# e-c-k-e-r/tortoise-tts

Measured on AMD Instinct MI355X. Metric: audio-sec/wall-sec (RTF^-1), 16 AR candidates x 80 DDIM steps, higher is better.
Workload: dtype bf16; 1 GPU; configs[1]: 1 utterance/GPU, 64 text tokens, 16 AR candidates x 250 mel tokens (KV-cached decode), latent pass on 16 candidates, 80 DDIM steps with cond-free guidance at T=1088 (11.6 s audio); candidates=16, ddim_steps=80, mel_frames=1088, parallelism=single GPU, small_models=False, vocoder_in_step=False

## Files before the change

### tortoise_tts_amd/csrc/diff.hip

```cpp
#include <stdlib.h>

#include "ttk_common.h"
#include "ttk_host.h"

using namespace ttk;

namespace {
struct AttnBlk { float *gn_g, *gn_b; Mat qkv, proj; float* relbias; };
struct ResBlk { float *gn1_g, *gn1_b, *gn2_g, *gn2_b; Mat in, out3; int emb_slot; };
struct DLayer { ResBlk res; AttnBlk attn; };
struct Lane {
	WsBuf a, hf, qkv, ao, ms;
	const void* ms_owner = nullptr;
};
struct Segs { int n, K, rows_per_batch; GemmSeg s[3]; };
struct Epi { int gn_T = 0; const float* residual = nullptr; float* ms = nullptr; int act = ACT_NONE; int transpose = 0; };
struct Gn {
	const float *gamma, *beta; int act; const Mat* next = nullptr; const float* mod = nullptr; int64_t mod_stride = 0; const float* ms = nullptr;
	void* out = nullptr; int out_f32 = 0; const int* row_idx = nullptr; int Tout = 0;
};
struct StepPlan {
	const ttk_step* st; int nb; const float* emb; const float* noise; bool layout, stage_next; const ttk_step_ext* ext = nullptr; float* pred_xstart = nullptr;
	const ttk_step_ms* ms = nullptr; float* x0_hist = nullptr;
};
}

struct ttk_diff {
	ttk_diff_config cfg;
	int dt, wdt;
	size_t es;
	Arena arena;
	AttnBlk lat_attn[4];
	Mat lat_conv, inp_block, integ, out_conv, time0, time2, emb_cat;
	float *code_g, *code_b, *out_g, *out_b, *uncond, *time_freqs;
	void* code_table = nullptr; int in_tokens = 0;
	AttnBlk code_attn[3];
	Mat mel_head;
	DLayer integrator[3];
	std::vector<DLayer> layers;
	ResBlk tail[3];
	int n_emb;
	int in_pad;
	Lane lane[2];
	Lane* L = &lane[0];
	WsBuf cs, cs2, xs, h0, csT, xcl, outb, ecl, ms_ecl, temb, e1, e2, se, emb_all, lat_T;
	WsBuf x0h;
	WsBuf hf0, ms_hf0;
	hipStream_t side = nullptr;
	hipEvent_t ev_fork = nullptr, ev_int[2] = {nullptr, nullptr}, ev_free[2] = {nullptr, nullptr};
	int pipe = 1;
	int cur_b = 0, cur_T = 0, staged = 0;
	int fuse_stats = 1;
	int* d_tlen = nullptr; int* d_need = nullptr;
	const int* tlen = nullptr; const int* need = nullptr;
	~ttk_diff() {
		if (side) (void)hipStreamDestroy(side);
		for (hipEvent_t e : {ev_fork, ev_int[0], ev_int[1], ev_free[0], ev_free[1]}) if (e) (void)hipEventDestroy(e);
	}
};

static Segs rows_of(const void* A, const Mat& m) { return {1, m.Kpad, 0, {{A, m.Kpad, 0, 0}}}; }
static Segs taps3(const void* A, int64_t lda, const Mat& m, int Tper) {
	const int64_t tap = (int64_t)m.Npad * m.Kpad;
	return {3, m.Kpad, Tper, {{A, lda, -1, 0}, {A, lda, 0, tap}, {A, lda, 1, 2 * tap}}};
}

static void gemm(ttk_diff* h, const Mat& m, const Segs& a, int M, void* C, int64_t ldc, int out_f32, hipStream_t s, const Epi& e = {}) {
	GemmParams g = {};
	g.nseg = a.n;
	for (int j = 0; j < a.n; ++j) g.seg[j] = a.s[j];
	g.W = m.w; g.ldw = m.Kpad; g.M = M; g.N = m.N; g.K = a.K; g.rows_per_batch = a.rows_per_batch; g.bias = m.bias;
	g.residual = e.residual; g.ldr = ldc; g.C = C; g.ldc = ldc; g.out_f32 = out_f32; g.act = e.act; g.transpose_out = e.transpose;
	if (m.wes == 1) g.out_scale = m.wscale;
	h->L->ms_owner = nullptr;
	if (h->fuse_stats && e.gn_T > 0 && out_f32 && !e.transpose && gemm_fuses_gn_stats(M, m.N, h->cfg.model_channels, e.gn_T)) {
		g.gn_part = e.ms ? e.ms : (float*)h->L->ms.p; g.gn_T = e.gn_T; h->L->ms_owner = C;
	}
	launch_gemm(m.wes == 1 ? DT_FP8 : h->dt, g, s);
}

static const float* stats_of(ttk_diff* h, const float* x, int nb, int T, hipStream_t s, float* ms = nullptr) {
	if (!ms) ms = (float*)h->L->ms.p;
	const bool fused = h->L->ms_owner == (const void*)x;
	h->L->ms_owner = nullptr;
	if (!fused || h->need) launch_gn_stats(x, nb, T, h->cfg.model_channels, ms, s, h->tlen, fused ? h->need : nullptr);
	return ms;
}

static void gn(ttk_diff* h, const float* x, int nb, int T, const Gn& d, hipStream_t s) {
	const int C = h->cfg.model_channels;
	GnApplyParams p = {};
	p.row_idx = d.row_idx; p.nb = nb; p.T = T; p.Tout = d.row_idx ? d.Tout : T; p.C = C; p.nchunks = gn_num_chunks(T, C);
	if (h->tlen && !d.row_idx) { p.tlen = h->tlen; p.chunk_rows = gn_rows_per_chunk(C); }
	p.x = x; p.ms = d.ms ? d.ms : stats_of(h, x, nb, T, s); p.gamma = d.gamma; p.beta = d.beta; p.act = d.act;
	if (d.mod) { p.scale = d.mod; p.shift = d.mod + C; p.ss_stride = d.mod_stride; }
	p.out = d.out ? d.out : h->L->a.p; p.out_f32 = d.out_f32;
	if (d.next) { p.pf = d.next->w; p.pf_bytes = (int64_t)d.next->Npad * d.next->Kpad * d.next->wes; p.pf_taps = d.next->ntap; p.out_f8 = d.next->wes == 1; }
	launch_gn_apply(h->dt, p, s);
}

static void attn_block(ttk_diff* h, const AttnBlk& A, float* x, int nb, int T, hipStream_t s) {
	const int C = h->cfg.model_channels, rows = nb * T;
	gn(h, x, nb, T, {A.gn_g, A.gn_b, ACT_NONE, &A.qkv}, s);
	gemm(h, A.qkv, rows_of(h->L->a.p, A.qkv), rows, h->L->qkv.p, 3 * C, 0, s);
	AttnParams a = {};
	a.qkv = h->L->qkv.p; a.ld = 3 * C; a.q_off = 0; a.k_off = 64; a.v_off = 128; a.head_stride = 192;
	a.out = h->L->ao.p; a.ldo = C; a.nb = nb; a.T = T; a.H = h->cfg.num_heads; a.causal = 0; a.bias = A.relbias; a.scale = 0.125f; a.tlen = h->tlen;
	a.pf = A.proj.w; a.pf_bytes = (int64_t)A.proj.Npad * A.proj.Kpad * A.proj.wes; a.pf_taps = 1;
	a.out_f8 = A.proj.wes == 1;
	launch_attn_fwd(h->dt, a, s);
	gemm(h, A.proj, rows_of(h->L->ao.p, A.proj), rows, x, C, 1, s, {T, x});
}

static void res_in(ttk_diff* h, const ResBlk& R, const float* x, int nb, int T, hipStream_t s, float* hf, const float* ms_x = nullptr, float* ms_hf = nullptr) {
	gn(h, x, nb, T, {R.gn1_g, R.gn1_b, ACT_SILU, &R.in, nullptr, 0, ms_x}, s);
	gemm(h, R.in, rows_of(h->L->a.p, R.in), nb * T, hf, h->cfg.model_channels, 1, s, {T, nullptr, ms_hf});
}
static void res_out(ttk_diff* h, const ResBlk& R, const float* hf, const float* ms_hf, const float* res, float* x, int nb, int T, const float* emb_all,
					int64_t emb_stride, hipStream_t s) {
	const int C = h->cfg.model_channels;
	gn(h, hf, nb, T, {R.gn2_g, R.gn2_b, ACT_SILU, &R.out3, emb_all + (int64_t)R.emb_slot * 2 * C, emb_stride, ms_hf}, s);
	gemm(h, R.out3, taps3(h->L->a.p, C, R.out3, T), nb * T, x, C, 1, s, {T, res});
}
static void res_block(ttk_diff* h, const ResBlk& R, float* x, int nb, int T, const float* emb_all, int64_t emb_stride, hipStream_t s) {
	res_in(h, R, x, nb, T, s, (float*)h->L->hf.p);
	res_out(h, R, (const float*)h->L->hf.p, nullptr, x, x, nb, T, emb_all, emb_stride, s);
}

static int reserve_lane(ttk_diff* h, Lane& L, int nb, int T) {
	const size_t rows = (size_t)nb * T, C = h->cfg.model_channels, es = h->es;
	TTK_TRY(L.hf.reserve(rows * C * 4)); TTK_TRY(L.a.reserve(rows * C * es)); TTK_TRY(L.qkv.reserve(rows * 3 * C * es)); TTK_TRY(L.ao.reserve(rows * C * es));
	TTK_TRY(L.ms.reserve((size_t)nb * 32 * gn_num_chunks(T, (int)C) * 3 * 4));
	return TTK_OK;
}
static int reserve_ws(ttk_diff* h, int nb, int T) {
	TTK_REQUIRE(gn_num_chunks(T, h->cfg.model_channels) <= 64, TTK_E_ARG, "%d frames exceed the GroupNorm chunk table (64 chunks)", T);
	const size_t rows = (size_t)nb * T, C = h->cfg.model_channels, es = h->es;
	h->L = &h->lane[0];
	TTK_TRY(reserve_lane(h, h->lane[0], nb, T));
	TTK_TRY(h->cs.reserve(rows * C * 4)); TTK_TRY(h->xs.reserve(rows * C * 4));
	TTK_TRY(h->h0.reserve(rows * C * es)); TTK_TRY(h->csT.reserve(rows * C * es)); TTK_TRY(h->xcl.reserve(rows * h->in_pad * es));
	TTK_TRY(h->outb.reserve(rows * h->cfg.out_channels * 4)); TTK_TRY(h->ecl.reserve(rows * C * 4));
	return TTK_OK;
}

static int time_path(ttk_diff* h, const int64_t* t_dev, const int64_t* t_host, int n, hipStream_t s) {
	const int C = h->cfg.model_channels;
	const size_t es = h->es;
	TTK_TRY(h->temb.reserve((size_t)n * C * es)); TTK_TRY(h->e1.reserve((size_t)n * C * es)); TTK_TRY(h->e2.reserve((size_t)n * C * 4));
	TTK_TRY(h->se.reserve((size_t)n * C * es)); TTK_TRY(h->emb_all.reserve((size_t)n * h->n_emb * 2 * C * 4));
	if (t_dev) launch_timestep_embedding(h->dt, t_dev, 0, n, C, h->time_freqs, h->temb.p, s);
	else for (int i = 0; i < n; ++i) launch_timestep_embedding(h->dt, nullptr, t_host[i], 1, C, h->time_freqs, (char*)h->temb.p + (size_t)i * C * es, s);
	Epi silu; silu.act = ACT_SILU;
	gemm(h, h->time0, rows_of(h->temb.p, h->time0), n, h->e1.p, C, 0, s, silu);
	gemm(h, h->time2, rows_of(h->e1.p, h->time2), n, h->e2.p, C, 1, s);
	launch_silu_cast(h->dt, (const float*)h->e2.p, h->se.p, (int64_t)n * C, s);
	gemm(h, h->emb_cat, rows_of(h->se.p, h->emb_cat), n, h->emb_all.p, (int64_t)h->n_emb * 2 * C, 1, s);
	return TTK_OK;
}

static void integrator(ttk_diff* h, int nb, int T, const float* emb_all, int64_t emb_stride, float* cs, hipStream_t s, bool staged) {
	for (int i = 0; i < 3; ++i) {
		const ResBlk& R = h->integrator[i].res;
		if (i == 0 && staged) res_out(h, R, (const float*)h->hf0.p, (const float*)h->ms_hf0.p, (const float*)h->ecl.p, cs, nb, T, emb_all, emb_stride, s);
		else res_block(h, R, cs, nb, T, emb_all, emb_stride, s);
		attn_block(h, h->integrator[i].attn, cs, nb, T, s);
	}
}
static void body(ttk_diff* h, int nb, int T, const float* emb_all, int64_t emb_stride, const float* cs, float* out, hipStream_t s,
				 hipEvent_t cs_consumed = nullptr) {
	const int C = h->cfg.model_channels, rows = nb * T;
	float* x = (float*)h->xs.p;
	gemm(h, h->inp_block, taps3(h->xcl.p, h->in_pad, h->inp_block, T), rows, h->h0.p, C, 0, s);
	launch_cast(h->dt, cs, h->csT.p, (int64_t)rows * C, s);
	if (cs_consumed) (void)hipEventRecord(cs_consumed, s);
	gemm(h, h->integ, {2, C, 0, {{h->h0.p, C, 0, 0}, {h->csT.p, C, 0, C}}}, rows, x, C, 1, s, {T});
	for (size_t i = 0; i < h->layers.size(); ++i) {
		res_block(h, h->layers[i].res, x, nb, T, emb_all, emb_stride, s);
		attn_block(h, h->layers[i].attn, x, nb, T, s);
	}
	for (int i = 0; i < 3; ++i) res_block(h, h->tail[i], x, nb, T, emb_all, emb_stride, s);
	gn(h, x, nb, T, {h->out_g, h->out_b, ACT_SILU}, s);
	Epi t; t.transpose = 1;
	gemm(h, h->out_conv, taps3(h->L->a.p, C, h->out_conv, T), rows, out, 0, 1, s, t);
}

static int load_attn(ttk_diff* h, const WeightMap& wm, const std::string& p, AttnBlk* A) {
	const int C = h->cfg.model_channels;
	TTK_TRY(upload_f32(h->arena, wm, p + "norm.weight", C, &A->gn_g));
	TTK_TRY(upload_f32(h->arena, wm, p + "norm.bias", C, &A->gn_b));
	TTK_TRY(upload_mat(h->arena, wm, h->dt, p + "qkv.weight", p + "qkv.bias", PK_NK, 3 * C, C, false, &A->qkv));
	TTK_TRY(upload_mat(h->arena, wm, h->wdt, p + "proj_out.weight", p + "proj_out.bias", PK_NK, C, C, false, &A->proj));
	TTK_TRY(upload_f32(h->arena, wm, p + "__relbias", (int64_t)h->cfg.num_heads * 129, &A->relbias));
	return TTK_OK;
}
static int load_res(ttk_diff* h, const WeightMap& wm, const std::string& p, ResBlk* R, int slot) {
	const int C = h->cfg.model_channels;
	TTK_TRY(upload_f32(h->arena, wm, p + "in_layers.0.weight", C, &R->gn1_g));
	TTK_TRY(upload_f32(h->arena, wm, p + "in_layers.0.bias", C, &R->gn1_b));
	TTK_TRY(upload_f32(h->arena, wm, p + "out_layers.0.weight", C, &R->gn2_g));
	TTK_TRY(upload_f32(h->arena, wm, p + "out_layers.0.bias", C, &R->gn2_b));
	TTK_TRY(upload_mat(h->arena, wm, h->wdt, p + "in_layers.2.weight", p + "in_layers.2.bias", PK_NK, C, C, false, &R->in));
	TTK_TRY(upload_mat(h->arena, wm, h->wdt, p + "out_layers.3.weight", p + "out_layers.3.bias", PK_CONV3, C, C, false, &R->out3));
	R->emb_slot = slot;
	return TTK_OK;
}

static void precompute_tail(ttk_diff* h, const float* x, const float* cond, const int32_t* interp_idx, int b, int M, int T, float* E_out, hipStream_t s) {
	const int C = h->cfg.model_channels;
	Gn d = {h->code_g, h->code_b, ACT_NONE, nullptr, cond, 2 * C};
	d.out = h->ecl.p; d.out_f32 = 1; d.row_idx = interp_idx; d.Tout = T;
	gn(h, x, b, M, d, s);
	launch_cl_to_cf((const float*)h->ecl.p, b, C, T, E_out, s);
}
static void mel_head_of(ttk_diff* h, int b, int T, float* out, hipStream_t s, bool from_ecl) {
	const int C = h->cfg.model_channels;
	if (from_ecl) launch_cast(h->dt, (const float*)h->ecl.p, h->csT.p, (int64_t)b * T * C, s);
	Epi t; t.transpose = 1;
	gemm(h, h->mel_head, taps3(h->csT.p, C, h->mel_head, T), b * T, out, 0, 1, s, t);
}

extern "C" {

int ttk_diff_create(ttk_diff** out, const ttk_diff_config* cfg, const ttk_weight_view* w, int n_w) {
	TTK_REQUIRE(out && cfg && w, TTK_E_ARG, "ttk_diff_create: null argument");
	gemm_roles_refresh();
	TTK_REQUIRE(cfg->model_channels % 64 == 0 && cfg->num_heads * 64 == cfg->model_channels, TTK_E_ARG,
				"ttk_diff_create: head_dim must be 64 (channels %d, heads %d)", cfg->model_channels, cfg->num_heads);
	TTK_REQUIRE(cfg->in_latent_channels % 64 == 0, TTK_E_ARG, "ttk_diff_create: in_latent_channels %% 64 != 0");
	TTK_REQUIRE(cfg->model_channels % 128 == 0 && cfg->model_channels <= 1024 && 1024 % cfg->model_channels == 0, TTK_E_ARG,
				"ttk_diff_create: model_channels %d unsupported (128, 256, 512 or 1024)", cfg->model_channels);
	TTK_REQUIRE(cfg->dtype == TTK_F32 || cfg->dtype == TTK_BF16 || cfg->dtype == TTK_F16 || cfg->dtype == TTK_FP8W || cfg->dtype == TTK_FP8, TTK_E_ARG, "ttk_diff_create: bad dtype %d", cfg->dtype);
	TTK_REQUIRE(cfg->dtype != TTK_FP8 || cfg->model_channels % 128 == 0, TTK_E_ARG, "ttk_diff_create: fp8 GEMMs need channels %% 128 == 0");
	std::unique_ptr<ttk_diff> h(new ttk_diff());
	h->cfg = *cfg;
	h->wdt = cfg->dtype;
	h->dt = kernel_dtype(cfg->dtype);
	h->es = dtype_size(h->dt);
	h->in_pad = round_up(cfg->in_channels, 64);
	h->fuse_stats = getenv("TTK_NO_FUSED_GN") ? 0 : 1;
	{ const char* e = getenv("TTK_DIFF_PIPE"); h->pipe = e ? atoi(e) : 1; }
	const int C = cfg->model_channels;
	WeightMap wm(w, n_w);
	TTK_TRY(upload_f32(h->arena, wm, "unconditioned_embedding", C, &h->uncond));
	TTK_TRY(upload_f32(h->arena, wm, "__time_freqs", C / 2, &h->time_freqs));
	TTK_TRY(upload_mat(h->arena, wm, h->dt, "inp_block.weight", "inp_block.bias", PK_CONV3, C, cfg->in_channels, false, &h->inp_block));
	TTK_TRY(upload_mat(h->arena, wm, h->dt, "time_embed.0.weight", "time_embed.0.bias", PK_NK, C, C, false, &h->time0));
	TTK_TRY(upload_mat(h->arena, wm, h->dt, "time_embed.2.weight", "time_embed.2.bias", PK_NK, C, C, false, &h->time2));
	TTK_TRY(upload_f32(h->arena, wm, "code_norm.weight", C, &h->code_g));
	TTK_TRY(upload_f32(h->arena, wm, "code_norm.bias", C, &h->code_b));
	TTK_TRY(upload_mat(h->arena, wm, h->dt, "latent_conditioner.0.weight", "latent_conditioner.0.bias", PK_CONV3, C, cfg->in_latent_channels, false, &h->lat_conv));
	for (int i = 0; i < 4; ++i) TTK_TRY(load_attn(h.get(), wm, "latent_conditioner." + std::to_string(i + 1) + ".", &h->lat_attn[i]));
	TTK_TRY(upload_mat(h->arena, wm, h->dt, "integrating_conv.weight", "integrating_conv.bias", PK_NK, C, 2 * C, false, &h->integ));
	TTK_TRY(upload_f32(h->arena, wm, "out.0.weight", C, &h->out_g));
	TTK_TRY(upload_f32(h->arena, wm, "out.0.bias", C, &h->out_b));
	TTK_TRY(upload_mat(h->arena, wm, h->dt, "out.2.weight", "out.2.bias", PK_CONV3, cfg->out_channels, C, false, &h->out_conv));
	int slot = 0;
	for (int i = 0; i < 3; ++i) {
		const std::string p = "conditioning_timestep_integrator." + std::to_string(i) + ".";
		TTK_TRY(load_res(h.get(), wm, p + "resblk.", &h->integrator[i].res, slot++));
		TTK_TRY(load_attn(h.get(), wm, p + "attn.", &h->integrator[i].attn));
	}
	h->layers.resize(cfg->num_layers);
	for (int i = 0; i < cfg->num_layers; ++i) {
		const std::string p = "layers." + std::to_string(i) + ".";
		TTK_TRY(load_res(h.get(), wm, p + "resblk.", &h->layers[i].res, slot++));
		TTK_TRY(load_attn(h.get(), wm, p + "attn.", &h->layers[i].attn));
	}
	for (int i = 0; i < 3; ++i) TTK_TRY(load_res(h.get(), wm, "layers." + std::to_string(cfg->num_layers + i) + ".", &h->tail[i], slot++));
	h->n_emb = slot;
	if (const ttk_weight_view* tv = wm.find("code_embedding.weight")) {
		TTK_REQUIRE(tv->ndim == 2 && tv->shape[0] >= 1 && tv->shape[0] < (1LL << 31) && tv->shape[1] == C, TTK_E_WEIGHT,
					"ttk_diff_create: code_embedding.weight must be [in_tokens][%d]", C);
		h->in_tokens = (int)tv->shape[0];
		const int64_t n = (int64_t)h->in_tokens * C;
		if (h->dt == DT_F32) { float* t = nullptr; TTK_TRY(upload_f32(h->arena, wm, "code_embedding.weight", n, &t)); h->code_table = t; }
		else {
			WsBuf tmp;
			TTK_TRY(tmp.reserve((size_t)n * 4));
			TTK_HIP(hipMemcpy(tmp.p, tv->data, (size_t)n * 4, hipMemcpyDefault));
			TTK_TRY(h->arena.alloc(&h->code_table, (size_t)n * h->es));
			launch_cast(h->dt, (const float*)tmp.p, h->code_table, n, 0);
			TTK_HIP(hipDeviceSynchronize());
		}
		for (int i = 0; i < 3; ++i) TTK_TRY(load_attn(h.get(), wm, "code_converter." + std::to_string(i) + ".", &h->code_attn[i]));
		TTK_TRY(upload_mat(h->arena, wm, h->dt, "mel_head.weight", "mel_head.bias", PK_CONV3, cfg->in_channels, C, false, &h->mel_head));
	}
	TTK_TRY(h->arena.alloc((void**)&h->d_tlen, 128 * sizeof(int)));
	TTK_TRY(h->arena.alloc((void**)&h->d_need, 128 * sizeof(int)));
	TTK_TRY(upload_mat(h->arena, wm, h->dt, "__emb_cat.weight", "__emb_cat.bias", PK_NK, h->n_emb * 2 * C, C, false, &h->emb_cat));
	hipError_t e = hipDeviceSynchronize();
	if (e != hipSuccess) { set_error("ttk_diff_create: %s", hipGetErrorString(e)); return TTK_E_HIP; }
	*out = h.release();
	return TTK_OK;
}

int ttk_diff_destroy(ttk_diff* h) {
	if (!h) return TTK_OK;
	(void)hipDeviceSynchronize();
	delete h;
	return TTK_OK;
}

int ttk_diff_precompute(ttk_diff* h, const float* latents, const float* cond, const int32_t* interp_idx, int b, int M, int T,
						float* E_out, void* stream) {
	TTK_REQUIRE(h && latents && cond && interp_idx && E_out, TTK_E_ARG, "ttk_diff_precompute: null argument");
	TTK_REQUIRE(b >= 1 && M >= 1 && T >= 1, TTK_E_ARG, "ttk_diff_precompute: empty input (b=%d M=%d T=%d)", b, M, T);
	const int C = h->cfg.model_channels, Cl = h->cfg.in_latent_channels;
	hipStream_t s = (hipStream_t)stream;
	TTK_TRY(reserve_ws(h, b, M > T ? M : T));
	h->staged = 0;
	TTK_TRY(h->lat_T.reserve((size_t)b * M * Cl * h->es));
	float* x = (float*)h->xs.p;
	launch_cast(h->dt, latents, h->lat_T.p, (int64_t)b * M * Cl, s);
	gemm(h, h->lat_conv, taps3(h->lat_T.p, Cl, h->lat_conv, M), b * M, x, C, 1, s, {M});
	for (int i = 0; i < 4; ++i) attn_block(h, h->lat_attn[i], x, b, M, s);
	precompute_tail(h, x, cond, interp_idx, b, M, T, E_out, s);
	TTK_HIP(hipGetLastError());
	return TTK_OK;
}

int ttk_diff_precompute_codes(ttk_diff* h, const int64_t* codes, const float* cond, const int32_t* interp_idx, int b, int M, int T,
							  float* E_out, float* mel_pred_out, void* stream) {
	TTK_REQUIRE(h && codes && cond && interp_idx && E_out, TTK_E_ARG, "ttk_diff_precompute_codes: null argument");
	TTK_REQUIRE(h->code_table, TTK_E_STATE, "ttk_diff_precompute_codes: the handle was created without code_embedding / code_converter / mel_head");
	TTK_REQUIRE(b >= 1 && M >= 1 && T >= 1, TTK_E_ARG, "ttk_diff_precompute_codes: empty input (b=%d M=%d T=%d)", b, M, T);
	hipStream_t s = (hipStream_t)stream;
	TTK_TRY(reserve_ws(h, b, M > T ? M : T));
	h->staged = 0;
	float* x = (float*)h->xs.p;
	launch_embed_rows(h->dt, h->code_table, codes, b * M, h->cfg.model_channels, h->in_tokens, x, s);
	h->L->ms_owner = nullptr;
	for (int i = 0; i < 3; ++i) attn_block(h, h->code_attn[i], x, b, M, s);
	precompute_tail(h, x, cond, interp_idx, b, M, T, E_out, s);
	if (mel_pred_out) mel_head_of(h, b, T, mel_pred_out, s, true);
	TTK_HIP(hipGetLastError());
	return TTK_OK;
}

int ttk_diff_mel_head(ttk_diff* h, const float* E, int b, int T, float* mel_pred_out, void* stream) {
	TTK_REQUIRE(h && E && mel_pred_out, TTK_E_ARG, "ttk_diff_mel_head: null argument");
	TTK_REQUIRE(h->code_table, TTK_E_STATE, "ttk_diff_mel_head: the handle was created without code_embedding / code_converter / mel_head");
	TTK_REQUIRE(b >= 1 && T >= 1, TTK_E_ARG, "ttk_diff_mel_head: empty input");
	hipStream_t s = (hipStream_t)stream;
	TTK_TRY(reserve_ws(h, b, T));
	h->staged = 0;
	launch_cf_to_cl(h->dt, E, b, h->cfg.model_channels, T, h->csT.p, h->cfg.model_channels, 1, s);
	mel_head_of(h, b, T, mel_pred_out, s, false);
	TTK_HIP(hipGetLastError());
	return TTK_OK;
}

int ttk_diff_forward(ttk_diff* h, const float* x, const int64_t* t, const float* E, int b, int T, float* out, void* stream) {
	TTK_REQUIRE(h && x && t && out, TTK_E_ARG, "ttk_diff_forward: null argument");
	TTK_REQUIRE(b >= 1 && T >= 1, TTK_E_ARG, "ttk_diff_forward: empty input");
	const int C = h->cfg.model_channels;
	hipStream_t s = (hipStream_t)stream;
	TTK_TRY(reserve_ws(h, b, T));
	h->staged = 0;
	if (E) launch_cf_to_cl(DT_F32, E, b, C, T, h->cs.p, C, 1, s);
	else launch_bcast_rows(DT_F32, h->uncond, b * T, C, h->cs.p, s);
	launch_cf_to_cl(h->dt, x, b, h->cfg.in_channels, T, h->xcl.p, h->in_pad, 1, s);
	TTK_TRY(time_path(h, t, nullptr, b, s));
	const int64_t stride = (int64_t)h->n_emb * 2 * C;
	integrator(h, b, T, (const float*)h->emb_all.p, stride, (float*)h->cs.p, s, false);
	body(h, b, T, (const float*)h->emb_all.p, stride, (const float*)h->cs.p, out, s);
	TTK_HIP(hipGetLastError());
	return TTK_OK;
}

int ttk_diff_begin(ttk_diff* h, const float* E, int b, int T, void* stream) {
	TTK_REQUIRE(h && E, TTK_E_ARG, "ttk_diff_begin: null argument");
	TTK_REQUIRE(b >= 1 && T >= 1, TTK_E_ARG, "ttk_diff_begin: empty input");
	const int C = h->cfg.model_channels;
	hipStream_t s = (hipStream_t)stream;
	TTK_TRY(reserve_ws(h, 2 * b, T));
	float* ecl = (float*)h->ecl.p;
	launch_cf_to_cl(DT_F32, E, b, C, T, ecl, C, 1, s);
	launch_bcast_rows(DT_F32, h->uncond, b * T, C, ecl + (size_t)b * T * C, s);
	TTK_TRY(h->ms_ecl.reserve((size_t)2 * b * 32 * gn_num_chunks(T, C) * 3 * 4));
	launch_gn_stats(ecl, 2 * b, T, C, (float*)h->ms_ecl.p, s, h->tlen);
	h->cur_b = b; h->cur_T = T; h->staged = 1;
	TTK_TRY(h->hf0.reserve((size_t)2 * b * T * C * 4)); TTK_TRY(h->ms_hf0.reserve((size_t)2 * b * 32 * gn_num_chunks(T, C) * 3 * 4));
	res_in(h, h->integrator[0].res, ecl, 2 * b, T, s, (float*)h->hf0.p, (const float*)h->ms_ecl.p, (float*)h->ms_hf0.p);
	stats_of(h, (const float*)h->hf0.p, 2 * b, T, s, (float*)h->ms_hf0.p);
	TTK_HIP(hipGetLastError());
	return TTK_OK;
}

static StepCoefs coefs_of(const ttk_step& st) {
	return {st.sqrt_recip_ac, st.sqrt_recipm1_ac, st.sqrt_ac_prev, st.sqrt_1m_ac_prev, st.cfk, st.coef1, st.coef2, st.min_log, st.max_log, st.sampler, st.nonzero};
}
static_assert(sizeof(ttk_step_ext) == 24, "ttk_step_ext is mirrored by tortoise_tts_amd/_lib.py: StepExtC");
static StepExt ext_of(const ttk_step_ext& e) { return {e.sigma, e.dir, e.sqrt_ac_next, e.sqrt_1m_ac_next, e.mode, e.clip}; }
static bool ext_reads_noise(const ttk_step& st, const ttk_step_ext& e) { return st.nonzero && (e.mode == 1 || (e.mode == 0 && e.sigma != 0.f)); }
static int check_ext(const char* who, const ttk_step_ext& e, int i) {
	TTK_REQUIRE(e.mode >= 0 && e.mode <= 2, TTK_E_ARG, "%s: step %d has mode %d (0 ddim, 1 p, 2 reverse ddim)", who, i, e.mode);
	TTK_REQUIRE(e.sigma >= 0.f, TTK_E_ARG, "%s: step %d has sigma %g", who, i, (double)e.sigma);
	return TTK_OK;
}
static_assert(sizeof(ttk_step_ms) == 16, "ttk_step_ms is mirrored by tortoise_tts_amd/_lib.py: StepMsC");
static StepMs ms_of(const ttk_step_ms& m) { return {m.c_x, m.c_d0, m.c_d1, m.clip}; }
static std::vector<StepPlan> plan_steps(ttk_diff* h, const ttk_step* steps, int n, const float* emb_all, int64_t emb_stride, const float* noise, const ttk_step_ext* ext = nullptr, bool ascending = false,
									const ttk_step_ms* ms = nullptr, float* x0_hist = nullptr) {
	const size_t nz = (size_t)h->cur_b * h->cfg.in_channels * h->cur_T;
	std::vector<StepPlan> plan(n);
	for (int j = 0; j < n; ++j) {
		const int i = ascending ? j : n - 1 - j;
		const int next = ascending ? i + 1 : i - 1;
		const bool cf = steps[i].cfk >= 0.f;
		StepPlan& p = plan[j];
		p.st = &steps[i]; p.nb = cf ? 2 * h->cur_b : h->cur_b; p.emb = emb_all + i * emb_stride; p.noise = noise ? noise + j * nz : nullptr;
		p.layout = j == 0 || !plan[j - 1].stage_next;
		p.stage_next = next >= 0 && next < n && !h->tlen && (steps[next].cfk >= 0.f) == cf;
		p.ext = ext ? ext + i : nullptr;
		p.ms = ms ? ms + i : nullptr; p.x0_hist = x0_hist;
	}
	return plan;
}

static void step_body(ttk_diff* h, float* x, const StepPlan& p, const float* cs, hipEvent_t cs_consumed, hipStream_t s) {
	const int b = h->cur_b, T = h->cur_T, Cin = h->cfg.in_channels, rep = p.nb / b;
	if (p.layout) launch_cf_to_cl(h->dt, x, b, Cin, T, h->xcl.p, h->in_pad, rep, s, h->tlen);
	float* out = (float*)h->outb.p;
	body(h, p.nb, T, p.emb, 0, cs, out, s, cs_consumed);
	const float* out_u = out + (size_t)b * h->cfg.out_channels * T;
	if (p.ms) {
		if (p.stage_next) launch_diffusion_step_ms(out, out_u, x, p.x0_hist, p.pred_xstart, b, Cin, T, coefs_of(*p.st), ms_of(*p.ms), s, h->xcl.p, h->in_pad, rep, elem_kind(h->dt));
		else launch_diffusion_step_ms(out, out_u, x, p.x0_hist, p.pred_xstart, b, Cin, T, coefs_of(*p.st), ms_of(*p.ms), s);
		return;
	}
	if (p.ext) {
		if (p.stage_next) launch_diffusion_step_ext(out, out_u, x, p.noise, p.pred_xstart, b, Cin, T, coefs_of(*p.st), ext_of(*p.ext), s, h->xcl.p, h->in_pad, rep, elem_kind(h->dt));
		else launch_diffusion_step_ext(out, out_u, x, p.noise, p.pred_xstart, b, Cin, T, coefs_of(*p.st), ext_of(*p.ext), s);
		return;
	}
	if (p.stage_next) launch_diffusion_step(out, out_u, x, p.noise, b, Cin, T, coefs_of(*p.st), s, h->xcl.p, h->in_pad, rep, elem_kind(h->dt));
	else launch_diffusion_step(out, out_u, x, p.noise, b, Cin, T, coefs_of(*p.st), s);
}

int ttk_diff_step(ttk_diff* h, float* x, const ttk_step* st, const float* noise, void* stream) {
	TTK_REQUIRE(h && x && st, TTK_E_ARG, "ttk_diff_step: null argument");
	TTK_REQUIRE(h->staged, TTK_E_STATE, "ttk_diff_step: call ttk_diff_begin first");
	TTK_REQUIRE(st->sampler == 0 || noise, TTK_E_ARG, "ttk_diff_step: the p sampler needs noise");
	TTK_REQUIRE(h->cfg.out_channels == 2 * h->cfg.in_channels, TTK_E_ARG, "ttk_diff_step: learned-range output needs out = 2 * in channels");
	hipStream_t s = (hipStream_t)stream;
	TTK_TRY(time_path(h, nullptr, &st->t, 1, s));
	const StepPlan p = plan_steps(h, st, 1, (const float*)h->emb_all.p, 0, noise)[0];
	integrator(h, p.nb, h->cur_T, p.emb, 0, (float*)h->cs.p, s, true);
	step_body(h, x, p, (const float*)h->cs.p, nullptr, s);
	TTK_HIP(hipGetLastError());
	return TTK_OK;
}

static int sample_loop(ttk_diff* h, float* x, const float* E, int b, int T, const ttk_step* steps, int n_steps, const float* noise, int sampler, void* stream, const char* who,
					   const ttk_step_ext* ext = nullptr, const ttk_step_ms* ms = nullptr) {
	TTK_REQUIRE(h && x && E && steps && n_steps >= 1, TTK_E_ARG, "%s: bad argument", who);
	if (ext) {
		for (int i = 0; i < n_steps; ++i) {
			TTK_TRY(check_ext(who, ext[i], i));
			TTK_REQUIRE(ext[i].mode == ext[0].mode, TTK_E_ARG, "%s: step %d has mode %d, step 0 mode %d (one mode per loop)", who, i, ext[i].mode, ext[0].mode);
			TTK_REQUIRE(noise || !ext_reads_noise(steps[i], ext[i]), TTK_E_ARG, "%s: step %d adds noise (mode %d, sigma %g) but noise is null", who, i, ext[i].mode, (double)ext[i].sigma);
		}
	}
	else if (!ms) TTK_REQUIRE(sampler == 0 || noise, TTK_E_ARG, "%s: the p sampler needs one noise block per step", who);
	TTK_REQUIRE(h->cfg.out_channels == 2 * h->cfg.in_channels, TTK_E_ARG, "%s: learned-range output needs out = 2 * in channels", who);
	hipStream_t s = (hipStream_t)stream;
	TTK_TRY(ttk_diff_begin(h, E, b, T, stream));
	std::vector<int64_t> ts(n_steps);
	for (int i = 0; i < n_steps; ++i) { ts[i] = steps[i].t; TTK_REQUIRE(ext || ms || steps[i].sampler == sampler, TTK_E_ARG, "%s: step %d has sampler %d", who, i, steps[i].sampler); }
	TTK_TRY(time_path(h, nullptr, ts.data(), n_steps, s));
	if (ms) TTK_TRY(h->x0h.reserve((size_t)b * h->cfg.in_channels * T * 4));
	const std::vector<StepPlan> plan = plan_steps(h, steps, n_steps, (const float*)h->emb_all.p, (int64_t)h->n_emb * 2 * h->cfg.model_channels, noise, ext, ext && ext[0].mode == 2,
												  ms, ms ? (float*)h->x0h.p : nullptr);
	const bool pipe = h->pipe && n_steps >= 2;
	float* csb[2] = {(float*)h->cs.p, (float*)h->cs.p};
	if (pipe) {
		if (!h->side) {
			TTK_HIP(hipStreamCreateWithFlags(&h->side, hipStreamNonBlocking));
			TTK_HIP(hipEventCreateWithFlags(&h->ev_fork, hipEventDisableTiming));
			for (int i = 0; i < 2; ++i) {
				TTK_HIP(hipEventCreateWithFlags(&h->ev_int[i], hipEventDisableTiming));
				TTK_HIP(hipEventCreateWithFlags(&h->ev_free[i], hipEventDisableTiming));
			}
		}
		TTK_TRY(reserve_lane(h, h->lane[1], 2 * b, T));
		TTK_TRY(h->cs2.reserve((size_t)2 * b * T * h->cfg.model_channels * 4));
		csb[1] = (float*)h->cs2.p;
		TTK_HIP(hipEventRecord(h->ev_fork, s));
		TTK_HIP(hipStreamWaitEvent(h->side, h->ev_fork, 0));
	}
	auto enqueue_integrator = [&](int j) {
		if (pipe) h->L = &h->lane[1];
		integrator(h, plan[j].nb, T, plan[j].emb, 0, csb[j & 1], pipe ? h->side : s, true);
		h->L = &h->lane[0];
		if (pipe) (void)hipEventRecord(h->ev_int[j & 1], h->side);
	};
	if (pipe) enqueue_integrator(0);
	for (int j = 0; j < n_steps; ++j) {
		if (!pipe) enqueue_integrator(j);
		else {
			if (j + 1 < n_steps) {
				if (j >= 1) TTK_HIP(hipStreamWaitEvent(h->side, h->ev_free[(j - 1) & 1], 0));
				enqueue_integrator(j + 1);
			}
			TTK_HIP(hipStreamWaitEvent(s, h->ev_int[j & 1], 0));
		}
		step_body(h, x, plan[j], csb[j & 1], pipe ? h->ev_free[j & 1] : nullptr, s);
	}
	TTK_HIP(hipGetLastError());
	return TTK_OK;
}

int ttk_diff_sample_ddim(ttk_diff* h, float* x, const float* E, int b, int T, const ttk_step* steps, int n_steps, void* stream) {
	return sample_loop(h, x, E, b, T, steps, n_steps, nullptr, 0, stream, "ttk_diff_sample_ddim");
}

static int sample_lines(ttk_diff* h, float* x, const float* E, int b, int Tp, const int* tlen, const ttk_step* steps, int n_steps, void* stream, const char* who,
						const ttk_step_ms* ms = nullptr) {
	TTK_REQUIRE(h && x && E && tlen && steps, TTK_E_ARG, "%s: null argument", who);
	TTK_REQUIRE(b >= 1 && 2 * b <= 64, TTK_E_ARG, "%s: %d elements (1..32)", who, b);
	TTK_REQUIRE(Tp >= 64 && Tp % 64 == 0, TTK_E_ARG, "%s: the slot length %d must be a multiple of 64 frames", who, Tp);
	const int C = h->cfg.model_channels;
	for (int i = 0; i < n_steps; ++i) TTK_REQUIRE(steps[i].cfk >= 0.f, TTK_E_ARG, "%s: step %d has no conditioning-free evaluation (the batch is laid out as [cond | uncond])", who, i);
	int host_len[128], host_need[128], any_need = 0;
	for (int e = 0; e < b; ++e) {
		TTK_REQUIRE(tlen[e] >= 1 && tlen[e] <= Tp, TTK_E_ARG, "%s: element %d has %d frames, slot %d", who, e, tlen[e], Tp);
		const int nd = !(h->fuse_stats && gemm_fuses_gn_stats(2 * tlen[e], C, C, tlen[e]));
		host_len[e] = host_len[b + e] = tlen[e];
		host_need[e] = host_need[b + e] = nd;
		any_need |= nd;
	}
	hipStream_t s = (hipStream_t)stream;
	TTK_HIP(hipMemcpyAsync(h->d_tlen, host_len, (size_t)2 * b * sizeof(int), hipMemcpyHostToDevice, s));
	TTK_HIP(hipMemcpyAsync(h->d_need, host_need, (size_t)2 * b * sizeof(int), hipMemcpyHostToDevice, s));
	TTK_HIP(hipStreamSynchronize(s));
	h->tlen = h->d_tlen;
	h->need = any_need ? h->d_need : nullptr;
	const int rc = sample_loop(h, x, E, b, Tp, steps, n_steps, nullptr, 0, stream, who, nullptr, ms);
	h->tlen = nullptr; h->need = nullptr;
	return rc;
}
int ttk_diff_sample_ddim_lines(ttk_diff* h, float* x, const float* E, int b, int Tp, const int* tlen, const ttk_step* steps, int n_steps, void* stream) {
	return sample_lines(h, x, E, b, Tp, tlen, steps, n_steps, stream, "ttk_diff_sample_ddim_lines");
}

int ttk_diff_sample_p(ttk_diff* h, float* x, const float* E, int b, int T, const ttk_step* steps, int n_steps, const float* noise, void* stream) {
	return sample_loop(h, x, E, b, T, steps, n_steps, noise, 1, stream, "ttk_diff_sample_p");
}

int ttk_diff_sample_ext(ttk_diff* h, float* x, const float* E, int b, int T, const ttk_step* steps, const ttk_step_ext* ext, int n_steps, const float* noise, void* stream) {
	TTK_REQUIRE(ext, TTK_E_ARG, "ttk_diff_sample_ext: null argument");
	return sample_loop(h, x, E, b, T, steps, n_steps, noise, 0, stream, "ttk_diff_sample_ext", ext);
}

int ttk_diff_step_ext(ttk_diff* h, float* x, const ttk_step* st, const ttk_step_ext* ext, const float* noise, float* pred_xstart, void* stream) {
	TTK_REQUIRE(h && x && st && ext, TTK_E_ARG, "ttk_diff_step_ext: null argument");
	TTK_REQUIRE(h->staged, TTK_E_STATE, "ttk_diff_step_ext: call ttk_diff_begin first");
	TTK_TRY(check_ext("ttk_diff_step_ext", *ext, 0));
	TTK_REQUIRE(noise || !ext_reads_noise(*st, *ext), TTK_E_ARG, "ttk_diff_step_ext: the step adds noise (mode %d, sigma %g) but noise is null", ext->mode, (double)ext->sigma);
	TTK_REQUIRE(h->cfg.out_channels == 2 * h->cfg.in_channels, TTK_E_ARG, "ttk_diff_step_ext: learned-range output needs out = 2 * in channels");
	hipStream_t s = (hipStream_t)stream;
	TTK_TRY(time_path(h, nullptr, &st->t, 1, s));
	StepPlan p = plan_steps(h, st, 1, (const float*)h->emb_all.p, 0, noise, ext)[0];
	p.pred_xstart = pred_xstart;
	integrator(h, p.nb, h->cur_T, p.emb, 0, (float*)h->cs.p, s, true);
	step_body(h, x, p, (const float*)h->cs.p, nullptr, s);
	TTK_HIP(hipGetLastError());
	return TTK_OK;
}

int ttk_diffusion_step_ext_rows(const float* out_c, const float* out_u, float* x, const float* noise, float* pred_xstart, int nb, int C, int T, const ttk_step* st,
								const ttk_step_ext* ext, void* xcl, int ldo, int rep, int xcl_dtype, void* stream) {
	TTK_REQUIRE(out_c && x && st && ext, TTK_E_ARG, "ttk_diffusion_step_ext_rows: null argument");
	TTK_REQUIRE(nb >= 1 && C >= 1 && T >= 1, TTK_E_ARG, "ttk_diffusion_step_ext_rows: empty input");
	TTK_TRY(check_ext("ttk_diffusion_step_ext_rows", *ext, 0));
	TTK_REQUIRE(out_u || st->cfk < 0.f, TTK_E_ARG, "ttk_diffusion_step_ext_rows: cfk >= 0 mixes in out_u, which is null");
	TTK_REQUIRE(noise || !ext_reads_noise(*st, *ext), TTK_E_ARG, "ttk_diffusion_step_ext_rows: the step adds noise (mode %d, sigma %g) but noise is null", ext->mode, (double)ext->sigma);
	TTK_REQUIRE(!xcl || (ldo >= C && rep >= 1 && (xcl_dtype == DT_F32 || xcl_dtype == DT_BF16 || xcl_dtype == DT_F16)), TTK_E_ARG,
				"ttk_diffusion_step_ext_rows: the channels-last copy needs ldo >= C, rep >= 1 and an f32 / bf16 / f16 type (ldo %d, rep %d, type %d)", ldo, rep, xcl_dtype);
	launch_diffusion_step_ext(out_c, out_u, x, noise, pred_xstart, nb, C, T, coefs_of(*st), ext_of(*ext), (hipStream_t)stream, xcl, ldo, rep, elem_kind(xcl_dtype));
	TTK_HIP(hipGetLastError());
	return TTK_OK;
}

static int check_ms_loop(const char* who, const ttk_step_ms* ms, int n_steps) {
	TTK_REQUIRE(ms && n_steps >= 1, TTK_E_ARG, "%s: null ms, or no steps", who);
	TTK_REQUIRE(ms[n_steps - 1].c_d1 == 0.f, TTK_E_ARG, "%s: step %d, the first to run, has c_d1 = %g, but there is no history yet", who, n_steps - 1, (double)ms[n_steps - 1].c_d1);
	return TTK_OK;
}

int ttk_diff_sample_ms(ttk_diff* h, float* x, const float* E, int b, int T, const ttk_step* steps, const ttk_step_ms* ms, int n_steps, void* stream) {
	TTK_TRY(check_ms_loop("ttk_diff_sample_ms", ms, n_steps));
	return sample_loop(h, x, E, b, T, steps, n_steps, nullptr, 0, stream, "ttk_diff_sample_ms", nullptr, ms);
}

int ttk_diff_sample_ms_lines(ttk_diff* h, float* x, const float* E, int b, int Tp, const int* tlen, const ttk_step* steps, const ttk_step_ms* ms, int n_steps, void* stream) {
	TTK_TRY(check_ms_loop("ttk_diff_sample_ms_lines", ms, n_steps));
	return sample_lines(h, x, E, b, Tp, tlen, steps, n_steps, stream, "ttk_diff_sample_ms_lines", ms);
}

int ttk_diff_step_ms(ttk_diff* h, float* x, float* x0_hist, const ttk_step* st, const ttk_step_ms* ms, float* pred_xstart, void* stream) {
	TTK_REQUIRE(ms, TTK_E_ARG, "ttk_diff_step_ms: null ms");
	TTK_REQUIRE(x0_hist || ms->c_d1 == 0.f, TTK_E_ARG, "ttk_diff_step_ms: c_d1 = %g reads the x0 history, which is null", (double)ms->c_d1);
	TTK_REQUIRE(h && x && st, TTK_E_ARG, "ttk_diff_step_ms: null argument");
	TTK_REQUIRE(h->staged, TTK_E_STATE, "ttk_diff_step_ms: call ttk_diff_begin first");
	TTK_REQUIRE(h->cfg.out_channels == 2 * h->cfg.in_channels, TTK_E_ARG, "ttk_diff_step_ms: learned-range output needs out = 2 * in channels");
	hipStream_t s = (hipStream_t)stream;
	TTK_TRY(time_path(h, nullptr, &st->t, 1, s));
	StepPlan p = plan_steps(h, st, 1, (const float*)h->emb_all.p, 0, nullptr, nullptr, false, ms, x0_hist)[0];
	p.pred_xstart = pred_xstart;
	integrator(h, p.nb, h->cur_T, p.emb, 0, (float*)h->cs.p, s, true);
	step_body(h, x, p, (const float*)h->cs.p, nullptr, s);
	TTK_HIP(hipGetLastError());
	return TTK_OK;
}

int ttk_diffusion_step_ms_rows(const float* out_c, const float* out_u, float* x, float* x0_hist, float* pred_xstart, int nb, int C, int T, const ttk_step* st,
							   const ttk_step_ms* ms, void* xcl, int ldo, int rep, int xcl_dtype, void* stream) {
	TTK_REQUIRE(ms, TTK_E_ARG, "ttk_diffusion_step_ms_rows: null ms");
	TTK_REQUIRE(x0_hist || ms->c_d1 == 0.f, TTK_E_ARG, "ttk_diffusion_step_ms_rows: c_d1 = %g reads the x0 history, which is null", (double)ms->c_d1);
	TTK_REQUIRE(out_c && x && st, TTK_E_ARG, "ttk_diffusion_step_ms_rows: null argument");
	TTK_REQUIRE(nb >= 1 && C >= 1 && T >= 1, TTK_E_ARG, "ttk_diffusion_step_ms_rows: empty input");
	TTK_REQUIRE(out_u || st->cfk < 0.f, TTK_E_ARG, "ttk_diffusion_step_ms_rows: cfk >= 0 mixes in out_u, which is null");
	TTK_REQUIRE(!xcl || (ldo >= C && rep >= 1 && (xcl_dtype == DT_F32 || xcl_dtype == DT_BF16 || xcl_dtype == DT_F16)), TTK_E_ARG,
				"ttk_diffusion_step_ms_rows: the channels-last copy needs ldo >= C, rep >= 1 and an f32 / bf16 / f16 type (ldo %d, rep %d, type %d)", ldo, rep, xcl_dtype);
	launch_diffusion_step_ms(out_c, out_u, x, x0_hist, pred_xstart, nb, C, T, coefs_of(*st), ms_of(*ms), (hipStream_t)stream, xcl, ldo, rep, elem_kind(xcl_dtype));
	TTK_HIP(hipGetLastError());
	return TTK_OK;
}

}
```

### tortoise_tts_amd/csrc/elementwise.hip

```cpp
#include "ttk_common.h"
#include "ttk_kernels.h"

namespace ttk {

__global__ void k_set_int(int* p, int v) { *p = v; }
void launch_set_int(int* p, int v, hipStream_t s) { hipLaunchKernelGGL(k_set_int, dim3(1), dim3(1), 0, s, p, v); }
__global__ void k_fill_int(int* p, int v, int n) { const int i = blockIdx.x * blockDim.x + threadIdx.x; if (i < n) p[i] = v; }
void launch_fill_int(int* p, int v, int n, hipStream_t s) { if (n > 0) hipLaunchKernelGGL(k_fill_int, dim3(grid_for(n)), dim3(256), 0, s, p, v, n); }
__global__ void k_fill_int2(int* p, int a, int b, int n) { const int i = blockIdx.x * blockDim.x + threadIdx.x; if (i < n) { p[2 * i] = a; p[2 * i + 1] = b; } }
void launch_fill_int2(int* p, int a, int b, int n, hipStream_t s) { if (n > 0) hipLaunchKernelGGL(k_fill_int2, dim3(grid_for(n)), dim3(256), 0, s, p, a, b, n); }

__global__ void k_gather_add(const float* A, const int* ia, const float* Bt, const int* ib, float* out, int rows, int d) {
	const int64_t idx = (int64_t)blockIdx.x * blockDim.x + threadIdx.x;
	const int d4 = d / 4;
	if (idx >= (int64_t)rows * d4) return;
	const int r = (int)(idx / d4), c = (int)(idx - (int64_t)r * d4) * 4;
	float4 v = *(const float4*)(A + (int64_t)ia[r] * d + c);
	if (Bt) { const float4 w = *(const float4*)(Bt + (int64_t)ib[r] * d + c); v.x += w.x; v.y += w.y; v.z += w.z; v.w += w.w; }
	*(float4*)(out + (int64_t)r * d + c) = v;
}
void launch_gather_add(const float* A, const int* ia, const float* Bt, const int* ib, float* out, int rows, int d, hipStream_t s) {
	const int64_t total = (int64_t)rows * (d / 4);
	hipLaunchKernelGGL(k_gather_add, dim3(grid_for(total)), dim3(256), 0, s, A, ia, Bt, ib, out, rows, d);
}

template <typename T>
__global__ void k_embed_rows(const T* table, const int64_t* ids, int rows, int C, int n_tok, float* out) {
	const int tpr = C >> 3;
	const int r = blockIdx.x * (256 / tpr) + (int)threadIdx.x / tpr, c = ((int)threadIdx.x % tpr) * 8;
	if (r >= rows) return;
	int64_t id = ids[r];
	id = id < 0 ? 0 : (id >= n_tok ? n_tok - 1 : id);
	const typename Frag<T>::type v = *(const typename Frag<T>::type*)(table + id * C + c);
	float* o = out + (int64_t)r * C + c;
	*(float4*)o = make_float4((float)v[0], (float)v[1], (float)v[2], (float)v[3]);
	*(float4*)(o + 4) = make_float4((float)v[4], (float)v[5], (float)v[6], (float)v[7]);
}
void launch_embed_rows(int dt, const void* table, const int64_t* ids, int rows, int C, int n_tok, float* out, hipStream_t s) {
	const int rpb = 256 / (C / 8);
	const dim3 grid((unsigned)((rows + rpb - 1) / rpb));
	by_dtype(dt, [&](auto t) { using T = decltype(t); hipLaunchKernelGGL((k_embed_rows<T>), grid, dim3(256), 0, s, (const T*)table, ids, rows, C, n_tok, out); });
}

__global__ void k_decode_embed(const float* emb, const int64_t* tok, const float* pos, const int* d_pos, int pos_off, int pos_rows, float* out, int B, int d,
							   void* frag, int frag_f32) {
	const int idx = blockIdx.x * blockDim.x + threadIdx.x;
	const int d4 = d / 4;
	if (idx >= B * d4) return;
	const int b = idx / d4, c = (idx - b * d4) * 4;
	int pi = *d_pos + pos_off;
	pi = pi < 0 ? 0 : (pi >= pos_rows ? pos_rows - 1 : pi);
	const float4 e = *(const float4*)(emb + tok[b] * d + c), w = *(const float4*)(pos + (int64_t)pi * d + c);
	const float4 v = make_float4(e.x + w.x, e.y + w.y, e.z + w.z, e.w + w.w);
	*(float4*)(out + (int64_t)b * d + c) = v;
	if (frag) {
		const int64_t fi = TTK_FRAG_INDEX(b, c, d / 32);
		store4_kind(frag, fi, v, frag_f32);
	}
}
void launch_decode_embed(const float* emb, const int64_t* tok, const float* pos, const int* d_pos, int pos_off, int pos_rows, float* out, int B, int d, hipStream_t s,
						 void* frag, int frag_f32) {
	hipLaunchKernelGGL(k_decode_embed, dim3(grid_for(B * (d / 4))), dim3(256), 0, s, emb, tok, pos, d_pos, pos_off, pos_rows, out, B, d, frag, frag_f32);
}

__global__ void k_copy_rows(const float* src, int64_t lds_, float* dst, int64_t ldd, int rows, int d) {
	const int64_t idx = (int64_t)blockIdx.x * blockDim.x + threadIdx.x;
	const int d4 = d / 4;
	if (idx >= (int64_t)rows * d4) return;
	const int r = (int)(idx / d4), c = (int)(idx - (int64_t)r * d4) * 4;
	*(float4*)(dst + r * ldd + c) = *(const float4*)(src + r * lds_ + c);
}
void launch_copy_rows(const float* src, int64_t lds_, float* dst, int64_t ldd, int rows, int d, hipStream_t s) {
	const int64_t total = (int64_t)rows * (d / 4);
	hipLaunchKernelGGL(k_copy_rows, dim3(grid_for(total)), dim3(256), 0, s, src, lds_, dst, ldd, rows, d);
}

template <typename T>
__global__ void k_cast(const float* src, T* dst, int64_t n) {
	const int64_t i = ((int64_t)blockIdx.x * blockDim.x + threadIdx.x) * 4;
	if (i + 3 < n) {
		const float4 v = *(const float4*)(src + i);
		dst[i] = cvt<T>(v.x); dst[i + 1] = cvt<T>(v.y); dst[i + 2] = cvt<T>(v.z); dst[i + 3] = cvt<T>(v.w);
	} else {
		for (int64_t j = i; j < n; ++j) dst[j] = cvt<T>(src[j]);
	}
}
void launch_cast(int dt, const float* src, void* dst, int64_t n, hipStream_t s) {
	const unsigned grid = (unsigned)((n / 4 + 256) / 256);
	by_dtype(dt, [&](auto t) { using T = decltype(t); hipLaunchKernelGGL((k_cast<T>), dim3(grid), dim3(256), 0, s, src, (T*)dst, n); });
}

template <typename T>
__global__ void k_cf_to_cl(const float* src, int nb, int C, int Tn, T* dst, int64_t ldo, int rep, const int* tlen) {
	__shared__ float tile[32][33];
	const int b = blockIdx.z, c0 = blockIdx.y * 32, t0 = blockIdx.x * 32;
	const int tx = threadIdx.x & 31, ty = threadIdx.x >> 5;
	const int tl = tlen ? tlen[b] : Tn;
	for (int i = ty; i < 32; i += 8) {
		const int c = c0 + i, t = t0 + tx;
		tile[i][tx] = (c < C && t < tl) ? src[((int64_t)b * C + c) * Tn + t] : 0.f;
	}
	__syncthreads();
	for (int i = ty; i < 32; i += 8) {
		const int t = t0 + i, c = c0 + tx;
		if (t < Tn && c < ldo)
			for (int r = 0; r < rep; ++r) dst[(((int64_t)r * nb + b) * Tn + t) * ldo + c] = cvt<T>(tile[tx][i]);
	}
}
void launch_cf_to_cl(int dt, const float* src, int nb, int C, int T, void* dst, int64_t ldo, int rep, hipStream_t s, const int* tlen) {
	dim3 grid((T + 31) / 32, (unsigned)((ldo + 31) / 32), nb);
	by_dtype(dt, [&](auto t) { using E = decltype(t); hipLaunchKernelGGL((k_cf_to_cl<E>), grid, dim3(256), 0, s, src, nb, C, T, (E*)dst, ldo, rep, tlen); });
}

__global__ void k_cl_to_cf(const float* src, int nb, int C, int Tn, float* dst) {
	__shared__ float tile[32][33];
	const int b = blockIdx.z, c0 = blockIdx.y * 32, t0 = blockIdx.x * 32;
	const int tx = threadIdx.x & 31, ty = threadIdx.x >> 5;
	for (int i = ty; i < 32; i += 8) {
		const int t = t0 + i, c = c0 + tx;
		tile[i][tx] = (c < C && t < Tn) ? src[((int64_t)b * Tn + t) * C + c] : 0.f;
	}
	__syncthreads();
	for (int i = ty; i < 32; i += 8) {
		const int c = c0 + i, t = t0 + tx;
		if (c < C && t < Tn) dst[((int64_t)b * C + c) * Tn + t] = tile[tx][i];
	}
}
void launch_cl_to_cf(const float* src, int nb, int C, int T, float* dst, hipStream_t s) {
	dim3 grid((T + 31) / 32, (C + 31) / 32, nb);
	hipLaunchKernelGGL(k_cl_to_cf, grid, dim3(256), 0, s, src, nb, C, T, dst);
}

template <typename T>
__global__ void k_bcast_rows(const float* vec, int rows, int C, T* dst) {
	const int64_t idx = (int64_t)blockIdx.x * blockDim.x + threadIdx.x;
	if (idx >= (int64_t)rows * C) return;
	dst[idx] = cvt<T>(vec[idx % C]);
}
void launch_bcast_rows(int dt, const float* vec, int rows, int C, void* dst, hipStream_t s) {
	const dim3 grid(grid_for((int64_t)rows * C));
	by_dtype(dt, [&](auto t) { using T = decltype(t); hipLaunchKernelGGL((k_bcast_rows<T>), grid, dim3(256), 0, s, vec, rows, C, (T*)dst); });
}

template <typename T>
__global__ void k_timestep_embedding(const int64_t* t, int64_t t_host, int n, int C, const float* freqs, T* out) {
	const int idx = blockIdx.x * blockDim.x + threadIdx.x;
	const int half = C / 2;
	if (idx >= n * half) return;
	const int i = idx / half, j = idx - i * half;
	const float tv = (float)(t ? t[i] : t_host);
	const float a = tv * freqs[j];
	out[(int64_t)i * C + j] = cvt<T>(cosf(a));
	out[(int64_t)i * C + half + j] = cvt<T>(sinf(a));
}
void launch_timestep_embedding(int dt, const int64_t* t, int64_t t_host, int n, int C, const float* freqs, void* out, hipStream_t s) {
	const dim3 grid(grid_for(n * (C / 2)));
	by_dtype(dt, [&](auto e) { using T = decltype(e); hipLaunchKernelGGL((k_timestep_embedding<T>), grid, dim3(256), 0, s, t, t_host, n, C, freqs, (T*)out); });
}

template <typename T>
__global__ void k_silu_cast(const float* x, T* y, int64_t n) {
	const int64_t i = (int64_t)blockIdx.x * blockDim.x + threadIdx.x;
	if (i < n) y[i] = cvt<T>(silu_precise(x[i]));
}
void launch_silu_cast(int dt, const float* x, void* y, int64_t n, hipStream_t s) {
	by_dtype(dt, [&](auto t) { using T = decltype(t); hipLaunchKernelGGL((k_silu_cast<T>), dim3(grid_for(n)), dim3(256), 0, s, x, (T*)y, n); });
}

__global__ void k_diffusion_step(const float* out_c, const float* out_u, float* x, const float* noise, int nb, int C, int Tn, StepCoefs k, void* xcl, int ldo, int rep, int ekind) {
	const int64_t idx = (int64_t)blockIdx.x * blockDim.x + threadIdx.x;
	const int64_t per = (int64_t)C * Tn;
	if (idx >= nb * per) return;
	const int b = (int)(idx / per);
	const int64_t r = idx - b * per;
	float eps = out_c[(int64_t)b * 2 * per + r];
	if (k.cfk >= 0.f) {
		const float eu = out_u[(int64_t)b * 2 * per + r];
		eps = (1.0f + k.cfk) * eps - k.cfk * eu;
	}
	const float xv = x[idx];
	float x0 = k.sqrt_recip_ac * xv - k.sqrt_recipm1_ac * eps;
	x0 = fminf(fmaxf(x0, -1.0f), 1.0f);
	float xn;
	if (k.sampler == 0) {
		const float e2 = (k.sqrt_recip_ac * xv - x0) / k.sqrt_recipm1_ac;
		xn = x0 * k.sqrt_ac_prev + k.sqrt_1m_ac_prev * e2;
	} else {
		const float var = out_c[(int64_t)b * 2 * per + per + r];
		const float frac = (var + 1.0f) / 2.0f;
		const float log_var = frac * k.max_log + (1.0f - frac) * k.min_log;
		const float mean = k.coef1 * x0 + k.coef2 * xv;
		xn = mean + (k.nonzero ? expf(0.5f * log_var) * noise[idx] : 0.f);
	}
	x[idx] = xn;
	if (xcl) {
		const int c = (int)(r / Tn), t = (int)(r - (int64_t)c * Tn);
		for (int q = 0; q < rep; ++q) {
			const int64_t o = (((int64_t)q * nb + b) * Tn + t) * ldo + c;
			if (ekind == EK_F32) ((float*)xcl)[o] = xn;
			else if (ekind == EK_F16) ((f16*)xcl)[o] = cvt<f16>(xn);
			else ((bf16*)xcl)[o] = cvt<bf16>(xn);
		}
	}
}
void launch_diffusion_step(const float* out_c, const float* out_u, float* x, const float* noise, int nb, int C, int T, StepCoefs c, hipStream_t s, void* xcl, int ldo, int rep, int ekind) {
	const int64_t total = (int64_t)nb * C * T;
	hipLaunchKernelGGL(k_diffusion_step, dim3(grid_for(total)), dim3(256), 0, s, out_c, out_u, x, noise, nb, C, T, c, xcl, ldo, rep, ekind);
}

__global__ void k_diffusion_step_ext(const float* out_c, const float* out_u, float* x, const float* noise, float* pred_xstart, int nb, int C, int Tn, StepCoefs k, StepExt e,
									 void* xcl, int ldo, int rep, int ekind) {
#pragma clang fp contract(off)
	const int64_t idx = (int64_t)blockIdx.x * blockDim.x + threadIdx.x;
	const int64_t per = (int64_t)C * Tn;
	if (idx >= nb * per) return;
	const int b = (int)(idx / per);
	const int64_t r = idx - b * per;
	float eps = out_c[(int64_t)b * 2 * per + r];
	if (k.cfk >= 0.f) {
		const float eu = out_u[(int64_t)b * 2 * per + r];
		eps = (1.0f + k.cfk) * eps - k.cfk * eu;
	}
	const float xv = x[idx];
	const float rx = k.sqrt_recip_ac * xv;
	float x0 = __builtin_fmaf(-k.sqrt_recipm1_ac, eps, rx);
	if (e.clip) x0 = fminf(fmaxf(x0, -1.0f), 1.0f);
	if (pred_xstart) pred_xstart[idx] = x0;
	float xn;
	if (e.mode == 1) {
		const float var = out_c[(int64_t)b * 2 * per + per + r];
		const float frac = (var + 1.0f) / 2.0f;
		const float log_var = frac * k.max_log + (1.0f - frac) * k.min_log;
		const float mean = __builtin_fmaf(k.coef2, xv, k.coef1 * x0);
		xn = mean + (k.nonzero ? expf(0.5f * log_var) * noise[idx] : 0.f);
	} else {
		const float e2 = (rx - x0) / k.sqrt_recipm1_ac;
		if (e.mode == 0) {
			xn = x0 * k.sqrt_ac_prev + e.dir * e2;
			if (k.nonzero && e.sigma != 0.f) xn = xn + e.sigma * noise[idx];
		} else {
			xn = x0 * e.sqrt_ac_next + e.sqrt_1m_ac_next * e2;
		}
	}
	x[idx] = xn;
	if (xcl) {
		const int c = (int)(r / Tn), t = (int)(r - (int64_t)c * Tn);
		for (int q = 0; q < rep; ++q) {
			const int64_t o = (((int64_t)q * nb + b) * Tn + t) * ldo + c;
			if (ekind == EK_F32) ((float*)xcl)[o] = xn;
			else if (ekind == EK_F16) ((f16*)xcl)[o] = cvt<f16>(xn);
			else ((bf16*)xcl)[o] = cvt<bf16>(xn);
		}
	}
}
void launch_diffusion_step_ext(const float* out_c, const float* out_u, float* x, const float* noise, float* pred_xstart, int nb, int C, int T, StepCoefs c, StepExt e, hipStream_t s,
							   void* xcl, int ldo, int rep, int ekind) {
	const int64_t total = (int64_t)nb * C * T;
	hipLaunchKernelGGL(k_diffusion_step_ext, dim3(grid_for(total)), dim3(256), 0, s, out_c, out_u, x, noise, pred_xstart, nb, C, T, c, e, xcl, ldo, rep, ekind);
}

__global__ void k_diffusion_step_ms(const float* out_c, const float* out_u, float* x, float* x0_hist, float* pred_xstart, int nb, int C, int Tn, StepCoefs k, StepMs m,
									void* xcl, int ldo, int rep, int ekind) {
#pragma clang fp contract(off)
	const int64_t idx = (int64_t)blockIdx.x * blockDim.x + threadIdx.x;
	const int64_t per = (int64_t)C * Tn;
	if (idx >= nb * per) return;
	const int b = (int)(idx / per);
	const int64_t r = idx - b * per;
	float eps = out_c[(int64_t)b * 2 * per + r];
	if (k.cfk >= 0.f) {
		const float eu = out_u[(int64_t)b * 2 * per + r];
		eps = (1.0f + k.cfk) * eps - k.cfk * eu;
	}
	const float xv = x[idx];
	const float rx = k.sqrt_recip_ac * xv;
	float x0 = __builtin_fmaf(-k.sqrt_recipm1_ac, eps, rx);
	if (m.clip) x0 = fminf(fmaxf(x0, -1.0f), 1.0f);
	if (pred_xstart) pred_xstart[idx] = x0;
	float xn = __builtin_fmaf(m.c_d0, x0, m.c_x * xv);
	if (m.c_d1 != 0.f) xn = __builtin_fmaf(m.c_d1, x0_hist[idx], xn);
	if (x0_hist) x0_hist[idx] = x0;
	x[idx] = xn;
	if (xcl) {
		const int c = (int)(r / Tn), t = (int)(r - (int64_t)c * Tn);
		for (int q = 0; q < rep; ++q) {
			const int64_t o = (((int64_t)q * nb + b) * Tn + t) * ldo + c;
			if (ekind == EK_F32) ((float*)xcl)[o] = xn;
			else if (ekind == EK_F16) ((f16*)xcl)[o] = cvt<f16>(xn);
			else ((bf16*)xcl)[o] = cvt<bf16>(xn);
		}
	}
}
void launch_diffusion_step_ms(const float* out_c, const float* out_u, float* x, float* x0_hist, float* pred_xstart, int nb, int C, int T, StepCoefs c, StepMs m, hipStream_t s,
							  void* xcl, int ldo, int rep, int ekind) {
	const int64_t total = (int64_t)nb * C * T;
	hipLaunchKernelGGL(k_diffusion_step_ms, dim3(grid_for(total)), dim3(256), 0, s, out_c, out_u, x, x0_hist, pred_xstart, nb, C, T, c, m, xcl, ldo, rep, ekind);
}

}
```

### tortoise_tts_amd/csrc/gemm.hip

```cpp
#include <stdlib.h>

#include <type_traits>

#include <hip/hip_ext.h>

#include "gemm_epilogue.h"

namespace ttk {

template <typename T, int BM, int NWM, int NWN, int ROLE>
__device__ __forceinline__ void conv3_image_tile(const GemmParams& p, const int m0, const int n0, const int wave) {
	typedef GRole<ROLE> R;
	static_assert(R::on && R::CONV && R::RES && sizeof(T) == 2, "the k = 3 residual role on 16-bit operands");
	constexpr int ES = 2, BN = 64, KSTEPS = 2, NW = NWM * NWN;
	constexpr int WM = BM / NWM, WN = BN / NWN, MI = WM / 16, NI = WN / 16;
	static_assert(MI == 4 && NI == 2, "64 x 32 wave blocks");
	constexpr int IMG_ROWS = BM + 8, IMG = IMG_ROWS * 128, NPA = IMG_ROWS / 8;
	constexpr int A_PC = (NPA + NW - 1) / NW, B_PC = 8 / NW;
	constexpr int NB = 4, BT = BN * 128, OFF_B = 2 * IMG, OFF_DUMP = OFF_B + NB * BT;
	constexpr int KC = GR_K / 64, NM = KSTEPS * MI * NI, NR = KSTEPS * (MI + NI), RPG = TTK_PIPE_RPG, D0 = TTK_PIPE_D0;
	static_assert(KC % 2 == 0 && (NR + RPG - 1) / RPG <= NM && D0 + B_PC + A_PC <= NM, "reads and DMA pieces must fit the MFMA gaps");
	constexpr unsigned TAPB = (unsigned)(R::N * GR_K * ES);
	constexpr int RESN = MI * 4 * NI;
	constexpr unsigned OOR = 0x80000000u;
	extern __shared__ __attribute__((aligned(16))) char smem[];
	const int lane = threadIdx.x & 63, g = lane >> 4, l15 = lane & 15;
#ifdef TTK_STAMPS
	unsigned long long* const stamps_ = p.stamps;
#endif
	const int wm = wave / NWN, wn = wave % NWN;
	const unsigned smem_base = __builtin_amdgcn_readfirstlane(lds_addr(smem));
	const int Tb = p.rows_per_batch;
	float bias_pre[NI];
#pragma unroll
	for (int j = 0; j < NI; ++j) bias_pre[j] = p.bias[n0 + wn * WN + 16 * j + l15];

	unsigned fa[3][KSTEPS], fb[KSTEPS];
#pragma unroll
	for (int ks = 0; ks < KSTEPS; ++ks) {
#pragma unroll
		for (int sg = 0; sg < 3; ++sg) {
			const int r = wm * WM + l15 + sg;
			fa[sg][ks] = smem_base + r * 128 + (((4 * ks + g) ^ (r & 7)) << 4);
		}
		const int rowb = wn * WN + l15;
		fb[ks] = smem_base + OFF_B + rowb * 128 + (((4 * ks + g) ^ (rowb & 7)) << 4);
	}
	const int prow = lane >> 3, pslot = lane & 7;
	unsigned va[A_PC], vb[B_PC];
#pragma unroll
	for (int i = 0; i < A_PC; ++i) {
		const int q = wave + NW * i, r = 8 * q + prow, gr = m0 - 1 + r;
		const bool ok = q < NPA && r < BM + 2 && gr >= 0 && gr < p.M;
		va[i] = ok ? (unsigned)(gr * (GR_K * ES) + ((pslot ^ (r & 7)) << 4)) : OOR;
	}
#pragma unroll
	for (int i = 0; i < B_PC; ++i) {
		const int row = 8 * (wave + NW * i) + prow;
		vb[i] = (unsigned)((n0 + row) * (GR_K * ES) + ((pslot ^ (row & 7)) << 4));
	}
	const __amdgpu_buffer_rsrc_t srdB = __builtin_amdgcn_make_buffer_rsrc((void*)p.W, 0, 0x7fffffff, 0x00020000);
	const __amdgpu_buffer_rsrc_t srdA = __builtin_amdgcn_make_buffer_rsrc((void*)p.seg[0].A, 0, (unsigned)p.M * (unsigned)(GR_K * ES), 0x00020000);
	int mlo = 0, mhi = 0;
#pragma unroll
	for (int i = 0; i < MI; ++i) {
		const int x = m0 + wm * WM + 16 * i + l15;
		const int t = x - div_recip(x, Tb, p.inv_rpb) * Tb;
		mlo |= (t == 0 ? 1 : 0) << i;
		mhi |= (t == Tb - 1 ? 1 : 0) << i;
	}
	const bool any_lo = __builtin_amdgcn_ballot_w64(mlo != 0) != 0, any_hi = __builtin_amdgcn_ballot_w64(mhi != 0) != 0;

	struct PFrags { u32x4 a[KSTEPS][MI], b[KSTEPS][NI]; };
	f32x4 acc[MI][NI];
#pragma unroll
	for (int i = 0; i < MI; ++i)
#pragma unroll
		for (int j = 0; j < NI; ++j) acc[i][j] = f32x4{0.f, 0.f, 0.f, 0.f};

	auto issue_image = [&](auto i_, auto slot_, unsigned kc) {
		constexpr int i = decltype(i_)::value, slot = decltype(slot_)::value;
		const int q = wave + NW * i;
		pipe_glds16(va[i], srdA, kc * 128u, q < NPA ? smem_base + slot * IMG + q * 1024 : smem_base + OFF_DUMP);
	};
	auto issue_w = [&](auto i_, unsigned soff, unsigned slot_off) {
		constexpr int i = decltype(i_)::value;
		pipe_glds16(vb[i], srdB, soff, smem_base + OFF_B + slot_off + (wave + NW * i) * 1024);
	};
	auto read_one = [&](auto r_, auto slot_, auto s_, PFrags& fr, const unsigned (&rb)[KSTEPS]) {
		constexpr int r = decltype(r_)::value, ks = r / (MI + NI), q = r % (MI + NI), SLOT = decltype(slot_)::value, S = decltype(s_)::value;
		if constexpr (q < MI) pipe_read16<q * 2048 + SLOT * IMG>(fr.a[ks][q], fa[S][ks]);
		else pipe_read16<(q - MI) * 2048>(fr.b[ks][q - MI], rb[ks]);
	};
	auto clear_edges = [&](auto s_, PFrags& fr) {
		constexpr int S = decltype(s_)::value;
		if constexpr (S == 0 || S == 2) {
			if (S == 0 ? any_lo : any_hi) {
				const int m = S == 0 ? mlo : mhi;
#pragma unroll
				for (int i = 0; i < MI; ++i) {
					const bool z = (m >> i) & 1;
#pragma unroll
					for (int ks = 0; ks < KSTEPS; ++ks)
#pragma unroll
						for (int e = 0; e < 4; ++e) fr.a[ks][i][e] = z ? 0u : fr.a[ks][i][e];
				}
			}
			TTK_FENCE();
		}
	};
	int tb = 0;
	auto trip = [&](auto w_, auto rd_, auto slot_rd_, auto s_rd_, auto isw_, auto s_cur_, auto isi_, auto slot_w_, const PFrags& cur, PFrags& nxt, unsigned kc_w, unsigned kc_i) {
		constexpr int W = decltype(w_)::value, S_CUR = decltype(s_cur_)::value;
		constexpr bool RD = decltype(rd_)::value, ISW = decltype(isw_)::value, ISI = decltype(isi_)::value;
		constexpr int PER = (ISW ? B_PC : 0) + (ISI ? A_PC : 0);
		const unsigned rd_slot = (unsigned)((tb + 1) & 3) * BT, wr_slot = (unsigned)((tb + 3) & 3) * BT;
		unsigned rb[KSTEPS];
#pragma unroll
		for (int ks = 0; ks < KSTEPS; ++ks) rb[ks] = fb[ks] + rd_slot;
		const unsigned soffW = (unsigned)S_CUR * TAPB + kc_w * 128u;
		if constexpr (RD || PER > 0) { wait_vmcnt<W>(); pipe_barrier(); }
		static_for<0, NM>([&](auto m_) {
			constexpr int m = decltype(m_)::value, ks = m / (MI * NI), i = (m % (MI * NI)) / NI, j = m % NI;
			pipe_mfma<T>(acc[i][j], cur.a[ks][i], cur.b[ks][j]);
			if constexpr (RD) static_for<0, RPG>([&](auto q_) {
				constexpr int r = m * RPG + decltype(q_)::value;
				if constexpr (r < NR) read_one(std::integral_constant<int, r>{}, slot_rd_, s_rd_, nxt, rb);
			});
			if constexpr (PER > 0 && m >= D0 && m - D0 < PER) {
				constexpr int d = m - D0;
				if constexpr (ISW && d < B_PC) issue_w(std::integral_constant<int, d>{}, soffW, wr_slot);
				else issue_image(std::integral_constant<int, d - (ISW ? B_PC : 0)>{}, slot_w_, kc_i);
			}
		});
		if constexpr (RD) { pipe_lgkm0(); clear_edges(s_rd_, nxt); }
		tb = (tb + 1) & 3;
	};
	typedef std::integral_constant<int, 0> I0; typedef std::integral_constant<int, 1> I1; typedef std::integral_constant<int, 2> I2;
	typedef std::true_type Y; typedef std::false_type N;

	PipeScope scope = pipe_begin();
	static_for<0, A_PC>([&](auto i_) { issue_image(i_, I0{}, 0u); });
	static_for<0, 3>([&](auto t_) { static_for<0, B_PC>([&](auto i_) { issue_w(i_, (unsigned)decltype(t_)::value * TAPB, (unsigned)decltype(t_)::value * BT); }); });
	static_for<0, A_PC>([&](auto i_) { issue_image(i_, I1{}, 1u); });
	TTK_WSTAMP(stamps_, blockIdx.x, 1);
	wait_vmcnt<2 * B_PC + A_PC>();
	pipe_barrier();
	TTK_WSTAMP(stamps_, blockIdx.x, 2);
	PFrags f0, f1;
	{
		unsigned rb0[KSTEPS];
#pragma unroll
		for (int ks = 0; ks < KSTEPS; ++ks) rb0[ks] = fb[ks];
		static_for<0, NR>([&](auto r_) { read_one(r_, I0{}, I0{}, f0, rb0); });
	}
	pipe_lgkm0();
	clear_edges(I0{}, f0);
	scope.clk = kclock_start();
	typedef std::integral_constant<int, B_PC + A_PC> W01; typedef std::integral_constant<int, B_PC> W2;
	const int row0 = m0 + wm * WM, col0 = n0 + wn * WN;
	float res_pre[MI][4][NI];
	for (int kc = 0; kc < KC - 2; kc += 2) {
		trip(W01{}, Y{}, I0{}, I1{}, Y{}, I0{}, N{}, I0{}, f0, f1, (unsigned)kc + 1, 0u);
		trip(W01{}, Y{}, I0{}, I2{}, Y{}, I1{}, N{}, I0{}, f1, f0, (unsigned)kc + 1, 0u);
		trip(W2{}, Y{}, I1{}, I0{}, Y{}, I2{}, Y{}, I0{}, f0, f1, (unsigned)kc + 1, (unsigned)kc + 2);
		trip(W01{}, Y{}, I1{}, I1{}, Y{}, I0{}, N{}, I1{}, f1, f0, (unsigned)kc + 2, 0u);
		trip(W01{}, Y{}, I1{}, I2{}, Y{}, I1{}, N{}, I1{}, f0, f1, (unsigned)kc + 2, 0u);
		trip(W2{}, Y{}, I0{}, I0{}, Y{}, I2{}, Y{}, I1{}, f1, f0, (unsigned)kc + 2, (unsigned)kc + 3);
	}
	{
		constexpr unsigned kc = KC - 2;
		trip(W01{}, Y{}, I0{}, I1{}, Y{}, I0{}, N{}, I0{}, f0, f1, kc + 1, 0u);
		trip(W01{}, Y{}, I0{}, I2{}, Y{}, I1{}, N{}, I0{}, f1, f0, kc + 1, 0u);
		trip(W2{}, Y{}, I1{}, I0{}, Y{}, I2{}, N{}, I0{}, f0, f1, kc + 1, 0u);
		if (m0 + BM <= p.M) load_residual_role<ROLE, MI, NI, false>(p, res_pre, row0, col0, lane);
		else load_residual_role<ROLE, MI, NI, true>(p, res_pre, row0, col0, lane);
		asm volatile("" ::: "memory");
		TTK_FENCE();
		trip(std::integral_constant<int, B_PC + RESN>{}, Y{}, I1{}, I1{}, N{}, I0{}, N{}, I1{}, f1, f0, 0u, 0u);
		trip(std::integral_constant<int, RESN>{}, Y{}, I1{}, I2{}, N{}, I1{}, N{}, I1{}, f0, f1, 0u, 0u);
		trip(I0{}, N{}, I0{}, I0{}, N{}, I2{}, N{}, I0{}, f1, f0, 0u, 0u);
	}
	pipe_end(scope, TTK_GEMM_STAMPS(p), lane);
	TTK_WSTAMPD(stamps_, blockIdx.x, 3, acc[0][0][0]);
	if (m0 + BM <= p.M) epilogue_role<T, ROLE, false, MI, NI, true>(p, acc, res_pre, bias_pre, row0, col0, lane);
	else epilogue_role<T, ROLE, true, MI, NI, true>(p, acc, res_pre, bias_pre, row0, col0, lane);
	TTK_WSTAMP(stamps_, blockIdx.x, 4);
#if defined(TTK_STAMPS) && TTK_STAMPS == 2
	asm volatile("s_waitcnt vmcnt(0)" ::: "memory");
	TTK_WSTAMP(stamps_, blockIdx.x, 5);
#endif
}

template <typename T, int BM, int BN, int NWM, int NWN, int NSTAGE, int ROLE, bool LONGK = false>
__device__ __forceinline__ void gemm_tile(const GemmParams& p, const int m0, const int n0, const int wave) {
	typedef GRole<ROLE> R;
	static_assert(!R::on || (sizeof(T) <= 2 && R::N % BN == 0), "roles are 16-bit or fp8, N a multiple of the tile width");
	constexpr int LDS_AVAIL = NSTAGE * ((BM == 64 && NWM == 1 ? 128 : BM) + BN) * 128;
	if constexpr (TTK_CONV_IMAGE && R::on && R::CONV && sizeof(T) == 2 && BN == 64 && NWN == 2 && BM / NWM == 64 && LDS_AVAIL >= 2 * (BM + 8) * 128 + 4 * 8192 + 1024) {
		conv3_image_tile<T, BM, NWM, NWN, ROLE>(p, m0, n0, wave);
		return;
	}
	constexpr int ES = sizeof(T);
	constexpr bool F8 = ES == 1;
	constexpr int BKE = 128 / ES;
	constexpr int KSTEPS = F8 ? 2 : BKE / 32;
	constexpr int FCH = F8 ? 1 : 8 * ES / 16;
	constexpr int EPC = 16 / ES;
	constexpr int NW = NWM * NWN;
	constexpr int WM = BM / NWM, WN = BN / NWN, MI = WM / 16, NI = WN / 16;
	constexpr int A_PC = BM / 8 / NW, B_PC = BN / 8 / NW;
	static_assert(A_PC >= 1 && B_PC >= 1 && A_PC * 8 * NW == BM && B_PC * 8 * NW == BN, "tile does not split into 1-KiB pieces per wave");
	constexpr int PER_TILE = A_PC + B_PC;
	constexpr int STAGE = (BM + BN) * 128;
	typedef typename Frag<T>::type FragT;
	extern __shared__ __attribute__((aligned(16))) char smem[];
	const int tid = threadIdx.x, lane = tid & 63;
#ifdef TTK_STAMPS
	unsigned long long* const stamps_ = p.stamps;
#endif
	const int wm = wave / NWN, wn = wave % NWN;
	const int KT = R::on ? GR_K / BKE : p.K / BKE;
	const int NTILES = R::on ? R::NSEG * KT : p.nseg * KT;

	const int prow = lane >> 3, pslot = lane & 7;
	int a_gm[A_PC], a_t[A_PC];
#pragma unroll
	for (int i = 0; i < A_PC; ++i) {
		a_gm[i] = m0 + 8 * (wave + NW * i) + prow;
		if constexpr (R::on) a_t[i] = R::CONV ? a_gm[i] - div_recip(a_gm[i], p.rows_per_batch, p.inv_rpb) * p.rows_per_batch : 0;
		else a_t[i] = p.rows_per_batch > 0 ? a_gm[i] % p.rows_per_batch : 0;
	}
	const unsigned smem_base = __builtin_amdgcn_readfirstlane(lds_addr(smem));
	constexpr unsigned OOR = 0x80000000u;
	unsigned va[A_PC], vb[B_PC];
#pragma unroll
	for (int i = 0; i < B_PC; ++i) {
		const int row = 8 * (wave + NW * i) + prow;
		const int c = pslot ^ (row & 7);
		if constexpr (R::on) vb[i] = (unsigned)((n0 + row) * (GR_K * ES) + c * 16);
		else vb[i] = (unsigned)(((int64_t)(n0 + row) * p.ldw + c * EPC) * ES);
	}
	const __amdgpu_buffer_rsrc_t srdB = __builtin_amdgcn_make_buffer_rsrc((void*)p.W, 0, 0x7fffffff, 0x00020000);
	__amdgpu_buffer_rsrc_t srdA = srdB;
	unsigned b_seg_off = 0;
	int seg_i = 0, kk_i = 0;
	const bool seg_in = R::on ? R::CONV : (p.seg_inner != 0);
	const int NSEG = R::on ? R::NSEG : p.nseg;
	unsigned va3[R::CONV ? 3 : 1][A_PC];
	if constexpr (R::on && R::CONV) {
#pragma unroll
		for (int sg = 0; sg < 3; ++sg)
#pragma unroll
			for (int i = 0; i < A_PC; ++i) {
				const int row = 8 * (wave + NW * i) + prow;
				const int c = pslot ^ (row & 7);
				const int t = a_t[i] + sg - 1;
				const bool ok = a_gm[i] < p.M && t >= 0 && t < p.rows_per_batch;
				va3[sg][i] = ok ? (unsigned)((a_gm[i] + sg - 1) * (GR_K * ES) + c * 16) : OOR;
			}
		srdA = __builtin_amdgcn_make_buffer_rsrc((void*)p.seg[0].A, 0, (unsigned)p.M * (unsigned)(GR_K * ES), 0x00020000);
	}
	auto set_segment = [&](int sg) {
		if constexpr (R::on && R::CONV) {
			b_seg_off = (unsigned)sg * (unsigned)(R::N * GR_K * ES);
#pragma unroll
			for (int i = 0; i < A_PC; ++i) va[i] = sg == 0 ? va3[0][i] : (sg == 1 ? va3[1][i] : va3[2][i]);
			return;
		}
		if constexpr (R::on) {
			srdA = __builtin_amdgcn_make_buffer_rsrc((void*)p.seg[0].A, 0, (unsigned)p.M * (unsigned)(GR_K * ES), 0x00020000);
			b_seg_off = 0;
#pragma unroll
			for (int i = 0; i < A_PC; ++i) {
				const int row = 8 * (wave + NW * i) + prow;
				const int c = pslot ^ (row & 7);
				va[i] = a_gm[i] < p.M ? (unsigned)(a_gm[i] * (GR_K * ES) + c * 16) : OOR;
			}
			return;
		}
		sg = __builtin_amdgcn_readfirstlane(sg);
		const int64_t lda = p.seg[sg].lda;
		const int shift = p.seg[sg].shift;
		srdA = __builtin_amdgcn_make_buffer_rsrc((void*)p.seg[sg].A, 0, (unsigned)((int64_t)p.M * lda * ES), 0x00020000);
		b_seg_off = (unsigned)(p.seg[sg].w_off * ES);
#pragma unroll
		for (int i = 0; i < A_PC; ++i) {
			const int row = 8 * (wave + NW * i) + prow;
			const int c = pslot ^ (row & 7);
			const int t = a_t[i] + shift;
			const bool ok = a_gm[i] < p.M && (shift == 0 || (t >= 0 && t < p.rows_per_batch));
			va[i] = ok ? (unsigned)(((int64_t)(a_gm[i] + shift) * lda + c * EPC) * ES) : OOR;
		}
	};
	auto next_tile = [&] {
		if (seg_in) { if (++seg_i == NSEG) { seg_i = 0; ++kk_i; } }
		else if (++kk_i == KT) { kk_i = 0; ++seg_i; }
		seg_i = __builtin_amdgcn_readfirstlane(seg_i); kk_i = __builtin_amdgcn_readfirstlane(kk_i);
	};
	auto issue = [&](int stage) {
		if (seg_in || kk_i == 0) set_segment(seg_i);
		const unsigned As = smem_base + stage * STAGE;
		const unsigned Bs = As + BM * 128;
		const unsigned soffA = (unsigned)kk_i * 128u, soffB = b_seg_off + (unsigned)kk_i * 128u;
#pragma unroll
		for (int i = 0; i < A_PC; ++i) {
#ifdef TTK_DIAG_SKIP
			if ((TTK_DIAG_SKIP & 1) && (seg_i > 0 || kk_i > 1)) continue;
			if ((TTK_DIAG_SKIP & 16) && seg_i > 0) continue;
#endif
			glds16(va[i], srdA, soffA, As + (wave + NW * i) * 1024);
		}
#pragma unroll
		for (int i = 0; i < B_PC; ++i) {
#ifdef TTK_DIAG_SKIP
			if ((TTK_DIAG_SKIP & 2) && (seg_i > 0 || kk_i > 1)) continue;
#endif
			glds16(vb[i], srdB, soffB, Bs + (wave + NW * i) * 1024);
		}
		next_tile();
	};

	f32x4 acc[MI][NI];
#pragma unroll
	for (int i = 0; i < MI; ++i)
#pragma unroll
		for (int j = 0; j < NI; ++j) acc[i][j] = f32x4{0.f, 0.f, 0.f, 0.f};

	const int row0 = m0 + wm * WM, col0 = n0 + wn * WN;
	float res_pre[MI][4][NI];
	float bias_pre[NI];
	if constexpr (R::on) {
#pragma unroll
		for (int j = 0; j < NI; ++j) bias_pre[j] = p.bias[col0 + 16 * j + (lane & 15)];
	}
	constexpr int RESN = MI * 4 * NI;
	constexpr bool PRE_RES = R::on && R::RES && NSTAGE >= 3 && (NSTAGE - 2) * PER_TILE + RESN <= 63 && (NSTAGE == 3 || (TTK_GEMM_PIPE && ES == 2 && MI * NI <= 8));
	auto wait_tiles = [&](int tiles) {
		if (tiles <= 0) wait_vmcnt<0>();
		else if (tiles == 1) wait_vmcnt<PER_TILE>();
		else if (tiles == 2 || NSTAGE <= 4) wait_vmcnt<2 * PER_TILE>();
		else if (tiles == 3 || NSTAGE <= 5) wait_vmcnt<3 * PER_TILE>();
		else wait_vmcnt<4 * PER_TILE>();
	};
	constexpr bool PIPE = TTK_GEMM_PIPE && ES == 2 && (NSTAGE == 3 || (R::on && NSTAGE > 3 && NSTAGE <= 6)) && MI * NI <= 8;
	constexpr bool PIPE_H = TTK_GEMM_PIPE_H && ES == 2 && NSTAGE == 3 && ((R::on && !R::RES) || (!R::on && LONGK)) && MI * NI == 16 && KSTEPS == 2;
	if constexpr (PIPE_H) {
		constexpr int NM = MI * NI, NR = MI + NI, D0 = NM - PER_TILE - 1;
		static_assert(NR <= NM && D0 >= 0, "reads and DMA pieces must fit the gaps of a half-step");
		const int NT = NTILES;
		static_assert(!R::on || R::NSEG * (GR_K / BKE) > NSTAGE, "the ring is deeper than the k-loop");
		struct HFrags { u32x4 a[MI], b[NI]; };
		unsigned fa[KSTEPS], fb[KSTEPS];
#pragma unroll
		for (int ks = 0; ks < KSTEPS; ++ks) {
			const int c0 = 4 * ks + (lane >> 4), rowa = wm * WM + (lane & 15), rowb = wn * WN + (lane & 15);
			fa[ks] = smem_base + rowa * 128 + ((c0 ^ (rowa & 7)) << 4);
			fb[ks] = smem_base + BM * 128 + rowb * 128 + ((c0 ^ (rowb & 7)) << 4);
		}
		unsigned pA_dst = 0, pB_dst = 0, p_soffA = 0, p_soffB = 0;
		auto issue_prep = [&](unsigned stage_off) {
			if (seg_in || kk_i == 0) set_segment(seg_i);
			pA_dst = smem_base + stage_off; pB_dst = pA_dst + BM * 128;
			p_soffA = (unsigned)kk_i * 128u; p_soffB = b_seg_off + (unsigned)kk_i * 128u;
			next_tile();
		};
		auto issue_piece = [&](auto d_) {
			constexpr int d = decltype(d_)::value;
			if constexpr (d < A_PC) pipe_glds16(va[d], srdA, p_soffA, pA_dst + (wave + NW * d) * 1024);
			else pipe_glds16(vb[d - A_PC], srdB, p_soffB, pB_dst + (wave + NW * (d - A_PC)) * 1024);
		};
		auto read_one = [&](auto r_, HFrags& fr, unsigned ra, unsigned rb) {
			constexpr int r = decltype(r_)::value;
			if constexpr (r < MI) pipe_read16<r * 2048>(fr.a[r], ra);
			else pipe_read16<(r - MI) * 2048>(fr.b[r - MI], rb);
		};
		auto htrip = [&](auto bar_, auto w_, auto rd_, auto issue_, const HFrags& cur, HFrags& nxt, unsigned ra, unsigned rb) {
			constexpr bool BAR = decltype(bar_)::value, RD = decltype(rd_)::value, ISSUE = decltype(issue_)::value;
			if constexpr (BAR) { wait_vmcnt<decltype(w_)::value>(); pipe_barrier(); }
			static_for<0, NM>([&](auto m_) {
				constexpr int m = decltype(m_)::value, i = m / NI, j = m % NI;
				pipe_mfma<T>(acc[i][j], cur.a[i], cur.b[j]);
				if constexpr (RD && m < NR) read_one(m_, nxt, ra, rb);
				if constexpr (ISSUE && m >= D0 && m - D0 < PER_TILE) issue_piece(std::integral_constant<int, m - D0>{});
			});
			if constexpr (RD) pipe_lgkm0();
		};
		typedef std::true_type Y; typedef std::false_type N; typedef std::integral_constant<int, 0> W0;
		PipeScope scope = pipe_begin();
#pragma unroll
		for (int st = 0; st < NSTAGE; ++st) { issue_prep(st * STAGE); static_for<0, PER_TILE>(issue_piece); }
		TTK_WSTAMP(stamps_, blockIdx.x, 1);
		wait_vmcnt<(NSTAGE - 1) * PER_TILE>();
		pipe_barrier();
		TTK_WSTAMP(stamps_, blockIdx.x, 2);
		HFrags f0, f1;
		static_for<0, NR>([&](auto r_) { read_one(r_, f0, fa[0], fb[0]); });
		pipe_lgkm0();
		scope.clk = kclock_start();
		unsigned cur_off = 0, nxt_off = STAGE;
		auto advance = [&] { cur_off = nxt_off; nxt_off = nxt_off == (NSTAGE - 1) * STAGE ? 0u : nxt_off + STAGE; };
		for (int kt = 0; kt < NT - NSTAGE; ++kt) {
			htrip(N{}, W0{}, Y{}, N{}, f0, f1, fa[1] + cur_off, fb[1] + cur_off);
			issue_prep(cur_off);
			htrip(Y{}, std::integral_constant<int, (NSTAGE - 2) * PER_TILE>{}, Y{}, Y{}, f1, f0, fa[0] + nxt_off, fb[0] + nxt_off);
			advance();
		}
		static_for<0, NSTAGE - 1>([&](auto t_) {
			htrip(N{}, W0{}, Y{}, N{}, f0, f1, fa[1] + cur_off, fb[1] + cur_off);
			htrip(Y{}, std::integral_constant<int, (NSTAGE - 2 - decltype(t_)::value) * PER_TILE>{}, Y{}, N{}, f1, f0, fa[0] + nxt_off, fb[0] + nxt_off);
			advance();
		});
		htrip(N{}, W0{}, Y{}, N{}, f0, f1, fa[1] + cur_off, fb[1] + cur_off);
		htrip(N{}, W0{}, N{}, N{}, f1, f0, 0u, 0u);
		pipe_end(scope, TTK_GEMM_STAMPS(p), lane);
	} else if constexpr (PIPE) {
		constexpr int NM = KSTEPS * MI * NI, NR = KSTEPS * (MI + NI);
		constexpr int PREB = TTK_PIPE_PREB, DPG = TTK_PIPE_DPG;
		constexpr int RPG_MIN = (NR + (NM - PREB) - 1) / (NM - PREB), RPG = TTK_PIPE_RPG > RPG_MIN ? TTK_PIPE_RPG : RPG_MIN;
		constexpr int RGAPS = (NR + RPG - 1) / RPG, DGAPS = (PER_TILE + DPG - 1) / DPG;
		constexpr int D0 = TTK_PIPE_DLATE || PREB + TTK_PIPE_D0 > NM - DGAPS ? NM - DGAPS : PREB + TTK_PIPE_D0;
		static_assert(PREB + RGAPS <= NM && D0 >= PREB && D0 + DGAPS <= NM, "reads and DMA pieces must fit the gaps behind the barrier");
		struct PFrags { u32x4 a[KSTEPS][MI], b[KSTEPS][NI]; };
		unsigned fa[KSTEPS], fb[KSTEPS];
#pragma unroll
		for (int ks = 0; ks < KSTEPS; ++ks) {
			const int c0 = 4 * ks + (lane >> 4), rowa = wm * WM + (lane & 15), rowb = wn * WN + (lane & 15);
			fa[ks] = smem_base + rowa * 128 + ((c0 ^ (rowa & 7)) << 4);
			fb[ks] = smem_base + BM * 128 + rowb * 128 + ((c0 ^ (rowb & 7)) << 4);
		}
		unsigned pA_dst = 0, pB_dst = 0, p_soffA = 0, p_soffB = 0;
#ifdef TTK_DIAG_SKIP
		bool p_skipA = false, p_skipB = false;
#endif
		auto issue_prep = [&](unsigned stage_off) {
			if (seg_in || kk_i == 0) set_segment(seg_i);
#ifdef TTK_DIAG_SKIP
			p_skipA = ((TTK_DIAG_SKIP & 1) && (seg_i > 0 || kk_i > 1)) || ((TTK_DIAG_SKIP & 16) && seg_i > 0);
			p_skipB = (TTK_DIAG_SKIP & 2) && (seg_i > 0 || kk_i > 1);
#endif
			pA_dst = smem_base + stage_off; pB_dst = pA_dst + BM * 128;
			p_soffA = (unsigned)kk_i * 128u; p_soffB = b_seg_off + (unsigned)kk_i * 128u;
			next_tile();
		};
		auto issue_piece = [&](auto d_) {
			constexpr int d = decltype(d_)::value;
			if constexpr (d < A_PC) {
#ifdef TTK_DIAG_SKIP
				if (p_skipA) return;
#endif
				pipe_glds16(va[d], srdA, p_soffA, pA_dst + (wave + NW * d) * 1024);
			} else {
#ifdef TTK_DIAG_SKIP
				if (p_skipB) return;
#endif
				pipe_glds16(vb[d - A_PC], srdB, p_soffB, pB_dst + (wave + NW * (d - A_PC)) * 1024);
			}
		};
		auto read_one = [&](auto r_, PFrags& fr, const unsigned (&ra)[KSTEPS], const unsigned (&rb)[KSTEPS]) {
			constexpr int r = decltype(r_)::value, ks = r / (MI + NI), q = r % (MI + NI);
			if constexpr (q < MI) pipe_read16<q * 2048>(fr.a[ks][q], ra[ks]);
			else pipe_read16<(q - MI) * 2048>(fr.b[ks][q - MI], rb[ks]);
		};
		auto trip = [&](auto issue_, auto&& pre, const PFrags& cur, PFrags& nxt, unsigned rd_off) {
			constexpr bool ISSUE = decltype(issue_)::value;
			unsigned ra[KSTEPS], rb[KSTEPS];
#pragma unroll
			for (int ks = 0; ks < KSTEPS; ++ks) { ra[ks] = fa[ks] + rd_off; rb[ks] = fb[ks] + rd_off; }
			static_for<0, NM>([&](auto m_) {
				constexpr int m = decltype(m_)::value, ks = m / (MI * NI), i = (m % (MI * NI)) / NI, j = m % NI;
				if constexpr (m == PREB) pre();
#if !(defined(TTK_DIAG_SKIP) && (TTK_DIAG_SKIP & 8))
				pipe_mfma<T>(acc[i][j], cur.a[ks][i], cur.b[ks][j]);
#endif
#if !(defined(TTK_DIAG_SKIP) && (TTK_DIAG_SKIP & 4))
				static_for<0, RPG>([&](auto q_) {
					constexpr int r = (m - PREB) * RPG + decltype(q_)::value;
					if constexpr (m >= PREB && r < NR) read_one(std::integral_constant<int, r>{}, nxt, ra, rb);
				});
#endif
				if constexpr (ISSUE) static_for<0, DPG>([&](auto q_) {
					constexpr int d = (m - D0) * DPG + decltype(q_)::value;
					if constexpr (m >= D0 && d < PER_TILE) issue_piece(std::integral_constant<int, d>{});
				});
			});
			pipe_lgkm0();
		};

		auto barrier = [&] { TTK_FENCE(); __builtin_amdgcn_s_barrier(); asm volatile("" ::: "memory"); TTK_FENCE(); };
		const unsigned m0_keep = pipe_m0_save();
#pragma unroll
		for (int st = 0; st < NSTAGE; ++st)
			if (st < NTILES) { issue_prep(st * STAGE); static_for<0, PER_TILE>(issue_piece); }
		TTK_WSTAMP(stamps_, blockIdx.x, 1);
		wait_tiles(min(NSTAGE, NTILES) - 1);
		barrier();
		TTK_WSTAMP(stamps_, blockIdx.x, 2);
		PFrags f0, f1;
		static_for<0, NR>([&](auto r_) { read_one(r_, f0, fa, fb); });
		pipe_lgkm0();
#ifdef TTK_CLOCK_STAMPS
		const unsigned long long clk0_ = __builtin_amdgcn_s_memtime(), rt0_ = __builtin_amdgcn_s_memrealtime();
#endif
		unsigned rd_off = STAGE, wr_off = 0;
		auto advance = [&] { rd_off = rd_off == (NSTAGE - 1) * STAGE ? 0u : rd_off + STAGE; wr_off = wr_off == (NSTAGE - 1) * STAGE ? 0u : wr_off + STAGE; };
		auto mfma_last = [&](const PFrags& cur) {
			static_for<0, NM>([&](auto m_) {
				constexpr int m = decltype(m_)::value, ks = m / (MI * NI), i = (m % (MI * NI)) / NI, j = m % NI;
				pipe_mfma<T>(acc[i][j], cur.a[ks][i], cur.b[ks][j]);
			});
		};
		auto pstep_i = [&](const PFrags& cur, PFrags& nxt) {
			auto pre = [&] { wait_vmcnt<(NSTAGE - 2) * PER_TILE>(); barrier(); };
			issue_prep(wr_off); trip(std::true_type{}, pre, cur, nxt, rd_off);
			advance();
		};
		auto ptail = [&](auto wtag, const PFrags& cur, PFrags& nxt) {
			auto pre = [&] { wait_vmcnt<decltype(wtag)::value>(); barrier(); };
			trip(std::false_type{}, pre, cur, nxt, rd_off);
			advance();
		};
		if constexpr (R::on) {
			constexpr int NT = R::NSEG * (GR_K / BKE), NMAIN = NT - NSTAGE;
			static_assert(NMAIN >= 2, "the ring is deeper than the k-loop");
			for (int kt = 0; kt + 2 <= NMAIN; kt += 2) { pstep_i(f0, f1); pstep_i(f1, f0); }
			if constexpr (NMAIN & 1) pstep_i(f0, f1);
			if constexpr (PRE_RES) {
				if (m0 + BM <= p.M) load_residual_role<ROLE, MI, NI, false>(p, res_pre, row0, col0, lane);
				else load_residual_role<ROLE, MI, NI, true>(p, res_pre, row0, col0, lane);
				asm volatile("" ::: "memory");
				TTK_FENCE();
			}
			static_for<0, NSTAGE - 1>([&](auto t_) {
				constexpr int t = decltype(t_)::value, W = (NSTAGE - 2 - t) * PER_TILE + (PRE_RES ? RESN : 0);
				if constexpr (((NMAIN + t) & 1) == 0) ptail(std::integral_constant<int, W>{}, f0, f1);
				else ptail(std::integral_constant<int, W>{}, f1, f0);
			});
			if constexpr (((NT - 1) & 1) == 0) mfma_last(f0); else mfma_last(f1);
		} else {
			static_assert(R::on || NSTAGE == 3, "run-time tile counts: 3-stage ring only");
			const int nmain = NTILES > NSTAGE ? NTILES - NSTAGE : 0;
			int kt = 0;
			for (; kt + 2 <= nmain; kt += 2) { pstep_i(f0, f1); pstep_i(f1, f0); }
			if (kt < nmain) { pstep_i(f0, f1); f0 = f1; ++kt; }
			if (NTILES - kt >= 3) { ptail(std::integral_constant<int, PER_TILE>{}, f0, f1); ptail(std::integral_constant<int, 0>{}, f1, f0); mfma_last(f0); }
			else if (NTILES - kt == 2) { ptail(std::integral_constant<int, 0>{}, f0, f1); mfma_last(f1); }
			else mfma_last(f0);
		}
		pipe_m0_restore(m0_keep);
#ifdef TTK_CLOCK_STAMPS
		if (stamps_ && lane == 0) {
			unsigned long long* st_ = stamps_ + ((size_t)blockIdx.x * 16 + (threadIdx.x >> 6)) * 8;
			st_[6] = ((__builtin_amdgcn_s_memtime() - clk0_) << 32) | ((__builtin_amdgcn_s_memrealtime() - rt0_) & 0xffffffffull);
		}
#endif
	} else {
		typedef int i32x4 __attribute__((ext_vector_type(4)));
		typedef int i32x8 __attribute__((ext_vector_type(8)));
		struct Frags { uint4 a[F8 ? 1 : KSTEPS][F8 ? 1 : MI][FCH]; uint4 b[F8 ? 1 : KSTEPS][F8 ? 1 : NI][FCH]; i32x8 a8[F8 ? MI : 1], b8[F8 ? NI : 1]; };
		auto read_frags = [&](Frags& fr, int stage) {
			const char* As = smem + stage * STAGE;
			const char* Bs = As + BM * 128;
			if constexpr (F8) {
				const int g = lane >> 4;
	#pragma unroll
				for (int i = 0; i < MI; ++i) {
					const int row = wm * WM + 16 * i + (lane & 15);
					const i32x4 lo = *(const i32x4*)(As + row * 128 + ((g ^ (row & 7)) << 4)), hi = *(const i32x4*)(As + row * 128 + (((4 + g) ^ (row & 7)) << 4));
					fr.a8[i] = __builtin_shufflevector(lo, hi, 0, 1, 2, 3, 4, 5, 6, 7);
				}
	#pragma unroll
				for (int j = 0; j < NI; ++j) {
					const int row = wn * WN + 16 * j + (lane & 15);
					const i32x4 lo = *(const i32x4*)(Bs + row * 128 + ((g ^ (row & 7)) << 4)), hi = *(const i32x4*)(Bs + row * 128 + (((4 + g) ^ (row & 7)) << 4));
					fr.b8[j] = __builtin_shufflevector(lo, hi, 0, 1, 2, 3, 4, 5, 6, 7);
				}
				return;
			}
	#pragma unroll
			for (int ks = 0; ks < KSTEPS; ++ks) {
				const int c0 = F8 ? 4 * ks + (lane >> 4) : (ks * 32 + 8 * (lane >> 4)) / EPC;
	#pragma unroll
				for (int i = 0; i < MI; ++i) {
					const int row = wm * WM + 16 * i + (lane & 15);
	#pragma unroll
					for (int f = 0; f < FCH; ++f) fr.a[ks][i][f] = *(const uint4*)(As + row * 128 + (((c0 + f) ^ (row & 7)) << 4));
				}
	#pragma unroll
				for (int j = 0; j < NI; ++j) {
					const int row = wn * WN + 16 * j + (lane & 15);
	#pragma unroll
					for (int f = 0; f < FCH; ++f) fr.b[ks][j][f] = *(const uint4*)(Bs + row * 128 + (((c0 + f) ^ (row & 7)) << 4));
				}
			}
		};
		auto mfma_tile = [&](const Frags& fr) {
			if constexpr (F8) {
	#pragma unroll
				for (int i = 0; i < MI; ++i)
	#pragma unroll
					for (int j = 0; j < NI; ++j) {
	#if TTK_FP8_SCALED_MFMA
						acc[i][j] = __builtin_amdgcn_mfma_scale_f32_16x16x128_f8f6f4(fr.a8[i], fr.b8[j], acc[i][j], 0 , 0 , 0, 0x7f7f7f7f, 0, 0x7f7f7f7f);
	#else
						typedef long l64x4 __attribute__((ext_vector_type(4)));
						const l64x4 la = (l64x4)fr.a8[i], lb = (l64x4)fr.b8[j];
	#pragma unroll
						for (int q = 0; q < 4; ++q) acc[i][j] = __builtin_amdgcn_mfma_f32_16x16x32_fp8_fp8(la[q], lb[q], acc[i][j], 0, 0, 0);
	#endif
					}
				return;
			}
	#pragma unroll
			for (int ks = 0; ks < KSTEPS; ++ks)
	#pragma unroll
				for (int i = 0; i < MI; ++i)
	#pragma unroll
					for (int j = 0; j < NI; ++j) {
						if constexpr (F8) {
							union { uint4 q; long l[2]; } ua, ub;
							ua.q = fr.a[ks][i][0]; ub.q = fr.b[ks][j][0];
							acc[i][j] = __builtin_amdgcn_mfma_f32_16x16x32_fp8_fp8(ua.l[0], ub.l[0], acc[i][j], 0, 0, 0);
							acc[i][j] = __builtin_amdgcn_mfma_f32_16x16x32_fp8_fp8(ua.l[1], ub.l[1], acc[i][j], 0, 0, 0);
						} else {
							union { FragT v; uint4 q[FCH]; } ua, ub;
	#pragma unroll
							for (int f = 0; f < FCH; ++f) { ua.q[f] = fr.a[ks][i][f]; ub.q[f] = fr.b[ks][j][f]; }
							acc[i][j] = mma16<typename std::conditional<F8, bf16, T>::type>(ua.v, ub.v, acc[i][j]);
						}
					}
		};
		auto step = [&](int kt, const Frags& cur, Frags& nxt) {
			wait_tiles(min(NSTAGE - 2, NTILES - 2 - kt));
	#if !(defined(TTK_DIAG_SKIP) && (TTK_DIAG_SKIP & 32))
			asm volatile("s_waitcnt lgkmcnt(0)" ::: "memory");
	#endif
	#if !(defined(TTK_DIAG_SKIP) && (TTK_DIAG_SKIP & 64))
			__builtin_amdgcn_s_barrier();
	#endif
			asm volatile("" ::: "memory");
	#ifdef TTK_DIAG_SKIP
			if ((TTK_DIAG_SKIP & 4) && kt > 0) { if (kt + NSTAGE < NTILES) issue(kt % NSTAGE); mfma_tile(cur); return; }
			if ((TTK_DIAG_SKIP & 8) && kt > 0) { if (kt + NSTAGE < NTILES) issue(kt % NSTAGE); read_frags(nxt, (kt + 1) % NSTAGE); return; }
	#endif
			if (kt + NSTAGE < NTILES) issue(kt % NSTAGE);
			read_frags(nxt, (kt + 1) % NSTAGE);
			mfma_tile(cur);
		};

	#pragma unroll
		for (int st = 0; st < NSTAGE; ++st)
			if (st < NTILES) issue(st);
		TTK_WSTAMP(stamps_, blockIdx.x, 1);
		wait_tiles(min(NSTAGE, NTILES) - 1);
		__builtin_amdgcn_s_barrier();
		asm volatile("" ::: "memory");
		TTK_WSTAMP(stamps_, blockIdx.x, 2);
		Frags f0, f1;
		read_frags(f0, 0);
		if constexpr (PRE_RES) {
			constexpr int NT = R::NSEG * (GR_K / BKE);
			static_assert(!PRE_RES || (NT % 2 == 0 && NT >= 8), "the peeled tail assumes an even tile count");
			auto tail_step = [&](auto wtag, int stage_next, const Frags& cur, Frags& nxt) {
				wait_vmcnt<decltype(wtag)::value>();
	#if !(defined(TTK_DIAG_SKIP) && (TTK_DIAG_SKIP & 32))
				asm volatile("s_waitcnt lgkmcnt(0)" ::: "memory");
	#endif
				__builtin_amdgcn_s_barrier();
				asm volatile("" ::: "memory");
				read_frags(nxt, stage_next);
				mfma_tile(cur);
			};
			int kt = 0;
			for (; kt < NT - 4; kt += 2) {
				step(kt, f0, f1);
				step(kt + 1, f1, f0);
			}
			step(NT - 4, f0, f1);
			if (m0 + BM <= p.M) load_residual_role<ROLE, MI, NI, false>(p, res_pre, row0, col0, lane);
			else load_residual_role<ROLE, MI, NI, true>(p, res_pre, row0, col0, lane);
			asm volatile("" ::: "memory");
			tail_step(std::integral_constant<int, PER_TILE + RESN>{}, (NT - 2) % NSTAGE, f1, f0);
			tail_step(std::integral_constant<int, RESN>{}, (NT - 1) % NSTAGE, f0, f1);
			mfma_tile(f1);
		} else {
			int kt = 0;
			for (; kt + 2 < NTILES; kt += 2) {
				step(kt, f0, f1);
				step(kt + 1, f1, f0);
			}
			if (kt + 2 == NTILES) { step(kt, f0, f1); mfma_tile(f1); }
			else mfma_tile(f0);
		}
	}
	TTK_WSTAMPD(stamps_, blockIdx.x, 3, acc[0][0][0]);

	if constexpr (R::on) {
		if (m0 + BM <= p.M) epilogue_role<T, ROLE, false, MI, NI, PRE_RES>(p, acc, res_pre, bias_pre, row0, col0, lane);
		else epilogue_role<T, ROLE, true, MI, NI, PRE_RES>(p, acc, res_pre, bias_pre, row0, col0, lane);
		TTK_WSTAMP(stamps_, blockIdx.x, 4);
#if defined(TTK_STAMPS) && TTK_STAMPS == 2
		asm volatile("s_waitcnt vmcnt(0)" ::: "memory");
		TTK_WSTAMP(stamps_, blockIdx.x, 5);
#endif
		return;
	}
	const bool full = (m0 + BM <= p.M) && (n0 + BN <= p.N);
	if (p.transpose_out) { if (full) epilogue<T, 2, false, MI, NI>(p, acc, row0, col0, lane); else epilogue<T, 2, true, MI, NI>(p, acc, row0, col0, lane); }
	else if (p.out_f32) { if (full) epilogue<T, 1, false, MI, NI>(p, acc, row0, col0, lane); else epilogue<T, 1, true, MI, NI>(p, acc, row0, col0, lane); }
	else { if (full) epilogue<T, 0, false, MI, NI>(p, acc, row0, col0, lane); else epilogue<T, 0, true, MI, NI>(p, acc, row0, col0, lane); }
	TTK_WSTAMP(stamps_, blockIdx.x, 4);
#if defined(TTK_STAMPS) && TTK_STAMPS == 2
	asm volatile("s_waitcnt vmcnt(0)" ::: "memory");
	TTK_WSTAMP(stamps_, blockIdx.x, 5);
#endif
}

template <typename B> __device__ __forceinline__ int xcd_tile_id(B block, int nwg) {
	const int xcd = block & 7, q = nwg >> 3, r = nwg & 7;
	return (xcd < r ? xcd * (q + 1) : r * (q + 1) + (xcd - r) * q) + (block >> 3);
}

template <typename T, int BM, int BN, int NWM, int NWN, int NSTAGE, int ROLE = GR_NONE, bool LONGK = false>
__global__ __launch_bounds__(64 * NWM * NWN, 2) void k_gemm(GemmParams p) {
	typedef GRole<ROLE> R;

	if constexpr (R::on) {
		if constexpr (R::CONV) TTK_PIN_ARGS(TTK_S(p.M), TTK_S(p.W), TTK_S(p.seg[0].A), TTK_S(p.tiles_m), TTK_S(p.inv_tiles_m), TTK_S(p.rows_per_batch), TTK_S(p.inv_rpb));
		else TTK_PIN_ARGS(TTK_S(p.M), TTK_S(p.W), TTK_S(p.seg[0].A), TTK_S(p.tiles_m), TTK_S(p.inv_tiles_m));
	} else {
		TTK_PIN_ARGS(TTK_S(p.M), TTK_S(p.N), TTK_S(p.K), TTK_S(p.nseg), TTK_S(p.W), TTK_S(p.ldw), TTK_S(p.rows_per_batch), TTK_S(p.m_major),
					 TTK_S(p.seg[0].A), TTK_S(p.seg[0].lda), TTK_S(p.seg[0].shift), TTK_S(p.seg[0].w_off));
	}
	const int wave = __builtin_amdgcn_readfirstlane((int)threadIdx.x >> 6);
#ifdef TTK_STAMPS
	unsigned long long* const stamps_ = p.stamps;
#endif
	TTK_WSTAMP(stamps_, blockIdx.x, 0);
	const int tiles_m = R::on ? p.tiles_m : (p.M + BM - 1) / BM;
	const int tile_id = xcd_tile_id(blockIdx.x, R::on ? tiles_m * (R::N / BN) : (int)gridDim.x);
	int m0, n0;
	if constexpr (R::on) {
		const int tn = div_recip(tile_id, tiles_m, p.inv_tiles_m);
		m0 = (tile_id - tn * tiles_m) * BM; n0 = tn * BN;
	} else {
		const int tiles_n = (p.N + BN - 1) / BN;
		m0 = p.m_major ? (tile_id / tiles_n) * BM : (tile_id % tiles_m) * BM;
		n0 = p.m_major ? (tile_id % tiles_n) * BN : (tile_id / tiles_m) * BN;
	}
	gemm_tile<T, BM, BN, NWM, NWN, NSTAGE, ROLE, LONGK>(p, m0, n0, wave);
}

template <typename T, int ROLE>
__global__ __launch_bounds__(256, 2) void k_gemm_mixed(GemmParams p) {
	typedef GRole<ROLE> R;
	static_assert(R::on && R::N == 1024, "mixed grids serve the 1024-wide roles");
	if constexpr (R::CONV) TTK_PIN_ARGS(TTK_S(p.M), TTK_S(p.W), TTK_S(p.seg[0].A), TTK_S(p.mix_full), TTK_S(p.mix_fm), TTK_S(p.inv_tiles_m),
										TTK_S(p.rows_per_batch), TTK_S(p.inv_rpb));
	else TTK_PIN_ARGS(TTK_S(p.M), TTK_S(p.W), TTK_S(p.seg[0].A), TTK_S(p.mix_full), TTK_S(p.mix_fm), TTK_S(p.inv_tiles_m));
	const int wave = __builtin_amdgcn_readfirstlane((int)threadIdx.x >> 6);
#ifdef TTK_STAMPS
	unsigned long long* const stamps_ = p.stamps;
#endif
	TTK_WSTAMP(stamps_, blockIdx.x, 0);
	const int b = blockIdx.x;
	if (b < p.mix_full) {
		const int tile_id = xcd_tile_id(b, p.mix_full);
		const int tn = div_recip(tile_id, p.mix_fm, p.inv_tiles_m);
		gemm_tile<T, 128, 64, 2, 2, TTK_ROLE_STAGES, ROLE>(p, (tile_id - tn * p.mix_fm) * 128, tn * 64, wave);
	} else {
		if (wave >= 2) return;
		const int j = b - p.mix_full;
		gemm_tile<T, 64, 64, 1, 2, TTK_ROLE_STAGES, ROLE>(p, p.mix_fm * 128 + (j >> 4) * 64, (2 * (j & 7) + ((j >> 3) & 1)) * 64, wave);
	}
}

static void opt_in_lds_once(bool& done, const void* kernel, int lds) {
	if (done) return;
	if (lds > 64 * 1024) (void)hipFuncSetAttribute(kernel, hipFuncAttributeMaxDynamicSharedMemorySize, lds);
	done = true;
}
static void fill_derived(GemmParams& p, int tiles_m) {
	p.tiles_m = tiles_m;
	p.inv_tiles_m = 1.0f / (float)tiles_m;
	p.inv_rpb = p.rows_per_batch > 0 ? 1.0f / (float)p.rows_per_batch : 0.f;
	p.inv_gn_T = p.gn_T > 0 ? 1.0f / (float)p.gn_T : 0.f;
}

template <typename T, int BM, int BN, int NWM, int NWN, int NSTAGE, int ROLE = GR_NONE, bool LONGK = false>
static void launch_tile(const GemmParams& p_in, hipStream_t s, hipEvent_t ea, hipEvent_t eb) {
	constexpr int LDS = NSTAGE * (BM + BN) * 128;
	if constexpr (!LONGK && ROLE == GR_NONE && sizeof(T) == 2 && BM == 256 && BN == 128 && NSTAGE == 3) {
		if (TTK_GEMM_PIPE_H && (p_in.K / 64) * p_in.nseg > NSTAGE) return launch_tile<T, BM, BN, NWM, NWN, NSTAGE, ROLE, true>(p_in, s, ea, eb);
	}
	static bool attr_set = false;
	opt_in_lds_once(attr_set, (const void*)k_gemm<T, BM, BN, NWM, NWN, NSTAGE, ROLE, LONGK>, LDS);
	GemmParams p = p_in;
	fill_derived(p, (p.M + BM - 1) / BM);
	const int grid = p.tiles_m * ((p.N + BN - 1) / BN);
	hipExtLaunchKernelGGL((k_gemm<T, BM, BN, NWM, NWN, NSTAGE, ROLE, LONGK>), dim3(grid), dim3(64 * NWM * NWN), (unsigned)LDS, s, ea, eb, 0, p);
}

static int g_mixed_mode = -1;
static bool mixed_grid_applies(const GemmParams& p) {
	if (g_mixed_mode < 0) { const char* e = getenv("TTK_GEMM_MIXED"); g_mixed_mode = e ? atoi(e) : 1; }
	if (!g_mixed_mode || p.N != 1024 || p.M % 64 != 0) return false;
	const int tiles_m = (p.M + 127) / 128;
	return tiles_m * 16 > 256 && tiles_m * 16 <= 320;
}
template <typename T, int ROLE>
static void launch_mixed(const GemmParams& p_in, hipStream_t s, hipEvent_t ea, hipEvent_t eb) {
	constexpr int LDS = TTK_ROLE_STAGES * (128 + 64) * 128;
	static_assert(LDS > 64 * 1024, "the mixed grid's ring needs the LDS opt-in");
	static bool attr_set = false;
	opt_in_lds_once(attr_set, (const void*)k_gemm_mixed<T, ROLE>, LDS);
	GemmParams p = p_in;
	p.mix_fm = 16; p.mix_full = 256;
	fill_derived(p, p.mix_fm);
	const int blocks64 = (p.M - 128 * p.mix_fm) / 64;
	hipExtLaunchKernelGGL((k_gemm_mixed<T, ROLE>), dim3(p.mix_full + blocks64 * 16), dim3(256), (unsigned)LDS, s, ea, eb, 0, p);
}

int g_gemm_roles = -1;
void gemm_roles_refresh() {
	g_mixed_mode = -1;
	const char* e = getenv("TTK_GEMM_ROLE");
	g_gemm_roles = e ? (atoi(e) == 1 ? 0x1E : atoi(e)) : 0x1E;
}
static int gemm_role_of_unmasked(const GemmParams& p, int es);
static int gemm_role_of(const GemmParams& p, int es) {
	const int r = gemm_role_of_unmasked(p, es);
	return (g_gemm_roles >> r) & 1 ? r : GR_NONE;
}
static int gemm_role_of_unmasked(const GemmParams& p, int es) {
	if (g_gemm_roles < 0) gemm_roles_refresh();
	if ((es != 2 && es != 1) || p.K != GR_K || p.ldw != GR_K || !p.bias || p.act != ACT_NONE || (es == 2) != (p.out_scale == 0.f)) return GR_NONE;
	if (p.transpose_out || p.m_major) return GR_NONE;
	if (p.M < 1 || p.M > (1 << 19) || p.seg[0].lda != GR_K || p.seg[0].w_off != 0) return GR_NONE;
	if (p.nseg == 1 && p.seg[0].shift == 0) {
		if (p.N == 3072 && !p.out_f32 && p.ldc == 3072 && !p.residual && !p.gn_part) return GR_QKV;
		if (p.N == 1024 && p.out_f32 && p.ldc == 1024 && p.gn_part && p.gn_T > 0) return !p.residual ? GR_IN1x1 : (p.ldr == 1024 ? GR_PROJ_RES : GR_NONE);
		return GR_NONE;
	}
	if (p.nseg == 3 && p.N == 1024 && p.out_f32 && p.ldc == 1024 && p.residual && p.ldr == 1024 && p.gn_part && p.gn_T > 0 && p.rows_per_batch > 0) {
		for (int j = 0; j < 3; ++j)
			if (p.seg[j].A != p.seg[0].A || p.seg[j].lda != GR_K || p.seg[j].shift != j - 1 || p.seg[j].w_off != (int64_t)j * 1024 * GR_K) return GR_NONE;
		return GR_CONV3_RES;
	}
	return GR_NONE;
}
static bool is_stat_role(int role) { return role == GR_IN1x1 || role == GR_CONV3_RES || role == GR_PROJ_RES; }
template <typename F> static void with_stat_role(int role, F&& f) {
	if (role == GR_IN1x1) f(std::integral_constant<int, GR_IN1x1>{});
	else if (role == GR_CONV3_RES) f(std::integral_constant<int, GR_CONV3_RES>{});
	else if (role == GR_PROJ_RES) f(std::integral_constant<int, GR_PROJ_RES>{});
}
template <typename T, int BM, int BN, int NWM, int NWN, int NSTAGE>
static void launch_tile_role(int role, const GemmParams& p, hipStream_t s, hipEvent_t ea, hipEvent_t eb) {
	if constexpr (sizeof(T) <= 2) {
		if constexpr (BM == 128 && BN == 64) {
			if (is_stat_role(role) && mixed_grid_applies(p)) return with_stat_role(role, [&](auto r) { launch_mixed<T, decltype(r)::value>(p, s, ea, eb); });
		}
		constexpr int NS = (BM == 128 && BN == 64 && sizeof(T) == 2) ? TTK_ROLE_STAGES : NSTAGE;
		if constexpr (BN <= 128) {
			if (is_stat_role(role)) return with_stat_role(role, [&](auto r) { launch_tile<T, BM, BN, NWM, NWN, NS, decltype(r)::value>(p, s, ea, eb); });
		}
		if (role == GR_QKV) return launch_tile<T, BM, BN, NWM, NWN, NS, GR_QKV>(p, s, ea, eb);
	}
	launch_tile<T, BM, BN, NWM, NWN, NSTAGE>(p, s, ea, eb);
}

int g_force_tile = -1;
static void read_force_tile() { if (g_force_tile < 0) { const char* e = getenv("TTK_GEMM_TILE"); g_force_tile = e ? atoi(e) + 100 : 99; } }
static int pick_tile(int M, int N) {
	const int t128 = ((M + 127) / 128) * ((N + 127) / 128);
	const int t12864 = ((M + 127) / 128) * ((N + 63) / 64);
	return t128 >= 256 ? 0 : (t12864 >= 128 ? 1 : 2);
}
bool gemm_fuses_gn_stats(int M, int N, int C, int T) {
	read_force_tile();
	if (g_force_tile >= 100 && g_force_tile - 100 == 2) return false;
	return C == 1024 && N == C && T % 64 == 0 && M % 64 == 0 && pick_tile(M, N) != 2;
}

template <typename T>
static void launch_gemm_t(const GemmParams& p, hipStream_t s, hipEvent_t ea, hipEvent_t eb) {
	read_force_tile();
	int tile;
	if (g_force_tile >= 100) tile = g_force_tile - 100;
	else {
		tile = pick_tile(p.M, p.N);
	}
	static const int wide = [] { const char* e = getenv("TTK_GEMM_TILE_WIDE"); return e ? atoi(e) : -2; }();
	if (g_force_tile < 100 && tile == 0) {
		const int t128 = ((p.M + 127) / 128) * ((p.N + 127) / 128), t256 = ((p.M + 255) / 256) * ((p.N + 127) / 128);
		if (wide >= 0) { if (p.N >= 3072) tile = wide; }
		else if (wide == -2 && sizeof(T) <= 2 && t128 > 256) {
			const int r128 = (t128 + 255) / 256, r256 = (t256 + 255) / 256;
			if (15 * r256 <= 9 * r128) tile = 8;
		}
	}
	const int role = gemm_role_of(p, (int)sizeof(T));
	if (tile == 0) launch_tile_role<T, 128, 128, 2, 4, 3>(role, p, s, ea, eb);
	else if (tile == 1) launch_tile_role<T, 128, 64, 2, 2, 3>(role, p, s, ea, eb);
	else if (tile == 3) launch_tile<T, 128, 128, 2, 4, 4>(p, s, ea, eb);
	else if (tile == 4) launch_tile<T, 128, 64, 2, 2, 5>(p, s, ea, eb);
	else if (tile == 5) launch_tile<T, 128, 64, 4, 2, 3>(p, s, ea, eb);
	else if (tile == 6) launch_tile<T, 128, 64, 2, 4, 3>(p, s, ea, eb);
	else if (tile == 7) launch_tile<T, 256, 64, 4, 2, 3>(p, s, ea, eb);
	else if (tile == 8) launch_tile_role<T, 256, 128, 4, 2, 3>(role, p, s, ea, eb);
	else if (tile == 9) launch_tile<T, 128, 128, 2, 4, 2>(p, s, ea, eb);
	else launch_tile<T, 64, 64, 2, 2, 3>(p, s, ea, eb);
}

void launch_gemm(int dt, const GemmParams& p_in, hipStream_t s) {
	static const int order = [] { const char* e = getenv("TTK_GEMM_ORDER"); return e ? atoi(e) : 0; }();
	GemmParams p = p_in;
	if (order == 1) p.m_major = p.nseg == 1 && (int64_t)p.N < p.M;
	else if (order == 2) p.m_major = (int64_t)p.N * p.nseg < p.M;
	else if (order == 3) p.m_major = 1;
	p.seg_inner = p.nseg == 3 && p.seg[0].shift == -1 && p.seg[1].shift == 0 && p.seg[2].shift == 1 && p.seg[1].A == p.seg[0].A && p.seg[2].A == p.seg[0].A &&
				  p.seg[1].lda == p.seg[0].lda && p.seg[2].lda == p.seg[0].lda;
	hipEvent_t ea = nullptr, eb = nullptr;
	if (g_prof_on) prof_pair(PROF_GEMM, 2.0 * p.M * p.N * (double)p.K * p.nseg, &ea, &eb);
	if (dt == DT_FP8) launch_gemm_t<f8>(p, s, ea, eb);
	else if (dt == DT_BF16) launch_gemm_t<bf16>(p, s, ea, eb);
	else if (dt == DT_F16) launch_gemm_t<f16>(p, s, ea, eb);
	else launch_gemm_t<float>(p, s, ea, eb);
}

}
```

### tortoise_tts_amd/csrc/gemm_epilogue.h

```cpp
#pragma once

#include "gemm_prims.h"

namespace ttk {

template <int MI, int NI>
__device__ __forceinline__ void gn_block_stats(const f32x4 (&acc)[MI][NI], float* part, int b, int group0, int nch, int chunk, int lane) {
#pragma clang fp contract(off)
#pragma unroll
	for (int gq = 0; gq < NI / 2; ++gq) {
		float sum = 0.f;
#pragma unroll
		for (int i = 0; i < MI; ++i)
#pragma unroll
			for (int jj = 0; jj < 2; ++jj)
#pragma unroll
				for (int r = 0; r < 4; ++r) sum += acc[i][2 * gq + jj][r];
		const float mean = wave_sum(sum) * (1.0f / 2048.0f);
		float sq = 0.f;
#pragma unroll
		for (int i = 0; i < MI; ++i)
#pragma unroll
			for (int jj = 0; jj < 2; ++jj)
#pragma unroll
				for (int r = 0; r < 4; ++r) { const float d = acc[i][2 * gq + jj][r] - mean; sq = __builtin_fmaf(d, d, sq); }
		sq = wave_sum(sq);
		if (lane == 0) {
			float* o = part + (((int64_t)b * 32 + (group0 + gq)) * nch + chunk) * 3;
			o[0] = 2048.0f; o[1] = mean; o[2] = sq;
		}
	}
}

template <typename T, int MODE, bool GUARD, int MI, int NI>
__device__ __forceinline__ void epilogue(const GemmParams& p, f32x4 (&acc)[MI][NI], int row0, int col0, int lane) {
#pragma clang fp contract(off)
	const int lr = 4 * (lane >> 4), lc = lane & 15;
	typedef typename OutOf<T>::type OT;
	if (p.out_scale != 0.f) {
#pragma unroll
		for (int i = 0; i < MI; ++i)
#pragma unroll
			for (int j = 0; j < NI; ++j) acc[i][j] *= p.out_scale;
	}
	float bj[NI];
#pragma unroll
	for (int j = 0; j < NI; ++j) {
		const int gn = col0 + 16 * j + lc;
		bj[j] = (p.bias && (!GUARD || gn < p.N)) ? p.bias[gn] : 0.f;
	}
#pragma unroll
	for (int i = 0; i < MI; ++i)
#pragma unroll
		for (int j = 0; j < NI; ++j)
#pragma unroll
			for (int r = 0; r < 4; ++r) acc[i][j][r] += bj[j];
	if (p.act == ACT_GELU_NEW) {
#pragma unroll
		for (int i = 0; i < MI; ++i)
#pragma unroll
			for (int j = 0; j < NI; ++j)
#pragma unroll
				for (int r = 0; r < 4; ++r) acc[i][j][r] = gelu_new_f(acc[i][j][r]);
	} else if (p.act == ACT_SILU) {
#pragma unroll
		for (int i = 0; i < MI; ++i)
#pragma unroll
			for (int j = 0; j < NI; ++j)
#pragma unroll
				for (int r = 0; r < 4; ++r) acc[i][j][r] = silu_f(acc[i][j][r]);
	}
	float res[MI][4][NI];
	if (MODE == 1 && p.residual) {
#pragma unroll
		for (int i = 0; i < MI; ++i)
#pragma unroll
			for (int r = 0; r < 4; ++r)
#pragma unroll
				for (int j = 0; j < NI; ++j) {
					const int gm = row0 + 16 * i + lr + r, gn = col0 + 16 * j + lc;
					res[i][r][j] = (!GUARD || (gm < p.M && gn < p.N)) ? p.residual[(int64_t)gm * p.ldr + gn] : 0.f;
				}
	} else {
#pragma unroll
		for (int i = 0; i < MI; ++i)
#pragma unroll
			for (int r = 0; r < 4; ++r)
#pragma unroll
				for (int j = 0; j < NI; ++j) res[i][r][j] = 0.f;
	}
#pragma unroll
	for (int i = 0; i < MI; ++i) {
#pragma unroll
		for (int r = 0; r < 4; ++r) {
			const int gm = row0 + 16 * i + lr + r;
			int bb = 0, t = 0;
			if (MODE == 2) { bb = gm / p.rows_per_batch; t = gm - bb * p.rows_per_batch; }
#pragma unroll
			for (int j = 0; j < NI; ++j) {
				const int gn = col0 + 16 * j + lc;
				if (GUARD && (gm >= p.M || gn >= p.N)) continue;
				const float v = acc[i][j][r] + res[i][r][j];
				acc[i][j][r] = v;
				if (MODE == 2) ((float*)p.C)[((int64_t)bb * p.N + gn) * p.rows_per_batch + t] = v;
				else if (MODE == 1) ((float*)p.C)[(int64_t)gm * p.ldc + gn] = v;
				else ((OT*)p.C)[(int64_t)gm * p.ldc + gn] = cvt<OT>(v);
			}
		}
	}
	if (MODE == 1 && p.gn_part && MI == 4 && row0 < p.M) {
		const int b = row0 / p.gn_T, chunk = (row0 - b * p.gn_T) / 64, nch = p.gn_T / 64;
		gn_block_stats<MI, NI>(acc, p.gn_part, b, col0 / 32, nch, chunk, lane);
	}
}

template <int ROLE> struct GRole { static constexpr bool on = false, RES = false, GN = false, CONV = false; static constexpr int N = 0, NSEG = 1, MODE = 0; };
template <> struct GRole<GR_IN1x1> { static constexpr bool on = true, RES = false, GN = true, CONV = false; static constexpr int N = 1024, NSEG = 1, MODE = 1; };
template <> struct GRole<GR_CONV3_RES> { static constexpr bool on = true, RES = true, GN = true, CONV = true; static constexpr int N = 1024, NSEG = 3, MODE = 1; };
template <> struct GRole<GR_QKV> { static constexpr bool on = true, RES = false, GN = false, CONV = false; static constexpr int N = 3072, NSEG = 1, MODE = 0; };
template <> struct GRole<GR_PROJ_RES> { static constexpr bool on = true, RES = true, GN = true, CONV = false; static constexpr int N = 1024, NSEG = 1, MODE = 1; };
constexpr int GR_K = 1024;

__device__ __forceinline__ int div_recip(int x, int d, float inv) {
	int q = (int)((float)x * inv);
	const int r = x - q * d;
	q += (r >= d ? 1 : 0) - (r < 0 ? 1 : 0);
	return q;
}

template <int ROLE, int MI, int NI, bool GUARD>
__device__ __forceinline__ void load_residual_role(const GemmParams& p, float (&res)[MI][4][NI], int row0, int col0, int lane) {
	constexpr int N = GRole<ROLE>::N;
	const int lr = 4 * (lane >> 4), lc = lane & 15;
#pragma unroll
	for (int i = 0; i < MI; ++i)
#pragma unroll
		for (int r = 0; r < 4; ++r)
#pragma unroll
			for (int j = 0; j < NI; ++j) {
				const int gm = row0 + 16 * i + lr + r;
				const int gr = GUARD ? min(gm, p.M - 1) : gm;
				res[i][r][j] = p.residual[(unsigned)(gr * N + col0 + 16 * j + lc)];
			}
}

template <typename T, int ROLE, bool GUARD, int MI, int NI, bool PRE = false>
__device__ __forceinline__ void epilogue_role(const GemmParams& p, f32x4 (&acc)[MI][NI], float (&res)[MI][4][NI], const float (&bj)[NI], int row0, int col0, int lane) {
#pragma clang fp contract(off)
	typedef GRole<ROLE> R;
	typedef typename OutOf<T>::type OT;
	constexpr int N = R::N;
	const int lr = 4 * (lane >> 4), lc = lane & 15;
	const float os = sizeof(T) == 1 ? p.out_scale : 1.f;
	if constexpr (R::RES && !PRE) {
#pragma unroll
		for (int i = 0; i < MI; ++i)
#pragma unroll
			for (int r = 0; r < 4; ++r)
#pragma unroll
				for (int j = 0; j < NI; ++j) {
					const int gm = row0 + 16 * i + lr + r;
					res[i][r][j] = (!GUARD || gm < p.M) ? p.residual[(unsigned)(gm * N + col0 + 16 * j + lc)] : 0.f;
				}
	}
	if constexpr (R::MODE == 0 && sizeof(OT) == 2 && !R::RES) {
		const bool odd = lc & 1;
#pragma unroll
		for (int i = 0; i < MI; ++i)
#pragma unroll
			for (int j = 0; j < NI; ++j)
#pragma unroll
				for (int rp = 0; rp < 2; ++rp) {
					float v0 = acc[i][j][2 * rp], v1 = acc[i][j][2 * rp + 1];
					if constexpr (sizeof(T) == 1) { v0 = v0 * os; v1 = v1 * os; }
					v0 = v0 + bj[j]; v1 = v1 + bj[j];
					acc[i][j][2 * rp] = v0; acc[i][j][2 * rp + 1] = v1;
					const float mine = odd ? v1 : v0, give = odd ? v0 : v1;
					const float got = __int_as_float(__builtin_amdgcn_update_dpp(0, __float_as_int(give), 0xB1, 0xF, 0xF, true));
					const uint2 pk = pack4_16<OT>(odd ? got : mine, odd ? mine : got, 0.f, 0.f);
					const int gm = row0 + 16 * i + lr + 2 * rp + (odd ? 1 : 0);
					if (GUARD && gm >= p.M) continue;
					*(unsigned*)((OT*)p.C + (unsigned)(gm * N + col0 + 16 * j + (lc & ~1))) = pk.x;
				}
	} else {
#pragma unroll
	for (int i = 0; i < MI; ++i)
#pragma unroll
		for (int r = 0; r < 4; ++r) {
			const int gm = row0 + 16 * i + lr + r;
#pragma unroll
			for (int j = 0; j < NI; ++j) {
				float v = acc[i][j][r];
				if constexpr (sizeof(T) == 1) v = v * os;
				v = v + bj[j];
				if constexpr (R::RES) v += (PRE && GUARD && gm >= p.M) ? 0.f : res[i][r][j];
				acc[i][j][r] = v;
				if (GUARD && gm >= p.M) continue;
				const unsigned o = (unsigned)(gm * N + col0 + 16 * j + lc);
				if constexpr (R::MODE == 1) ((float*)p.C)[o] = v;
				else ((OT*)p.C)[o] = cvt<OT>(v);
			}
		}
	}
	if constexpr (R::GN) {
		if (MI == 4 && row0 < p.M) {
			const int b = div_recip(row0, p.gn_T, p.inv_gn_T), chunk = (row0 - b * p.gn_T) >> 6, nch = p.gn_T >> 6;
			gn_block_stats<MI, NI>(acc, p.gn_part, b, col0 / 32, nch, chunk, lane);
		}
	}
}

}
```

### tortoise_tts_amd/csrc/ttk_kernels.h

```cpp
#pragma once
#include <hip/hip_runtime.h>
#include <stdint.h>

namespace ttk {

enum DType { DT_F32 = 0, DT_BF16 = 1, DT_FP8W = 2, DT_FP8 = 3, DT_F16 = 4 };
inline int elem_kind(int dt) { return dt == DT_F32 ? 1 : (dt == DT_F16 ? 2 : 0); }
inline size_t dtype_size(int dt) { return dt == DT_F32 ? 4 : 2; }
inline int kernel_dtype(int dt) { return (dt == DT_FP8W || dt == DT_FP8) ? DT_BF16 : dt; }
template <typename F>
auto by_dtype(int dt, F f) {
	if (dt == DT_BF16) return f(__bf16());
	if (dt == DT_F16) return f(_Float16());
	return f(float());
}
template <typename F>
auto by_f32_bf16(int dt, F f) { return dt == DT_BF16 ? f(__bf16()) : f(float()); }
inline unsigned grid_for(int64_t total) { return (unsigned)((total + 255) / 256); }

enum ProfKind { PROF_GEMM = 0, PROF_SKINNY = 1, PROF_ATTN_FWD = 2, PROF_ATTN_DECODE = 3, PROF_GN_STATS = 4, PROF_GN_APPLY = 5,
				PROF_LAYERNORM = 6, PROF_KINDS = 7 };
extern bool g_prof_on;
void prof_start(int kind, double work, hipStream_t s);
void prof_stop(hipStream_t s);
void prof_pair(int kind, double work, hipEvent_t* start, hipEvent_t* stop);
struct ProfScope {
	hipStream_t s; bool on;
	ProfScope(int kind, double work, hipStream_t s_) : s(s_), on(g_prof_on) { if (on) prof_start(kind, work, s); }
	~ProfScope() { if (on) prof_stop(s); }
};

struct GemmSeg {
	const void* A;
	int64_t lda;
	int shift;
	int64_t w_off;
};
struct GemmParams {
	int nseg;
	int M, N, K;
	const void* W;
	int64_t ldw;
	int rows_per_batch;
	int act;
	const float* bias;
	const float* residual;
	int64_t ldr;
	void* C;
	int64_t ldc;
	float out_scale;
	int out_f32;
	int transpose_out;
	int gn_T; float* gn_part;
	int seg_inner;
	int m_major;
	int tiles_m; float inv_tiles_m, inv_rpb, inv_gn_T;
	int mix_full, mix_fm;
#ifdef TTK_STAMPS
	unsigned long long* stamps;
#endif
	GemmSeg seg[12];
};
enum GemmRole { GR_NONE = 0, GR_IN1x1 = 1, GR_CONV3_RES = 2, GR_QKV = 3, GR_PROJ_RES = 4 };
void launch_gemm(int dt, const GemmParams& p, hipStream_t s);
void gemm_roles_refresh();
bool gemm_fuses_gn_stats(int M, int N, int C, int T);

enum SkinnyMode { SK_STORE_F32 = 0, SK_RESIDUAL = 1, SK_ACT_T = 2, SK_QKV = 3 };
struct SkinnyParams {
	const void* Wp;
	int N, K, M;
	const float* bias;
	int ln_count;
	const float* x;  int64_t ldx;
	const float* g1;
	union {
		const float* b1;
		int* health;
	};
	const float *g2, *b2;
	const void* a;
	int mode, act;
	float* out_f32;  int64_t ldc;
	void* out_T;
	float* qbuf; void* kcache; void* vcache; int max_ctx, H; float q_scale;
	const int* d_pos;
	float* noise; const void* rng; const int64_t* draws;
	int w8; float wscale;
#ifdef TTK_STAMPS
	unsigned long long* stamps;
#endif
};
enum SkinnyForm { SKF_PLAIN = 0, SKF_FOLD = 1, SKF_PROLOGUE = 2 };
constexpr size_t CU_LDS_BYTES = 160 * 1024;
constexpr size_t LDS_DEFAULT_LIMIT = 64 * 1024;
inline int skinny_launch_waves(int waves, bool prologue) { return waves < 4 ? 4 : (prologue && waves > 8 ? 8 : waves); }
inline size_t skinny_lds_bytes(int dt, int MT, int K, int waves, int form) {
	const size_t red = (size_t)waves * MT * 64 * 4 * sizeof(float);
	if (form == SKF_PROLOGUE) return (size_t)16 * MT * ((size_t)K * dtype_size(dt) + 16) + red;
	return form == SKF_FOLD ? red + (size_t)waves * MT * 16 * 2 * sizeof(float) : red;
}
hipError_t launch_skinny(int dt, const SkinnyParams& p, int waves, hipStream_t s);

enum GemvRole { GV_QKV = 0, GV_PROJ = 1, GV_FC = 2, GV_HEAD = 3 };
inline int decode_row_tiles(int M) { return M <= 16 ? 1 : (M <= 32 ? 2 : (M <= 48 ? 3 : 4)); }

struct GemvParams {
	const void* Wp;
	const void* a;
	const float* bias;
	const float* csum;
	float* out_f32;
	void* out_T;
	float* qbuf; void* kcache; void* vcache;
	const int* d_pos;
	float* noise; const void* rng; const int64_t* draws;
	int* health;
	int M, N, max_ctx, H, row0;
	float q_scale, wscale;
	int K, w8;
#ifdef TTK_STAMPS
	unsigned long long* stamps;
#endif
};
bool launch_gemv(int dt, int role, const GemvParams& p, hipStream_t s);
bool gemv_supported(int dt, int role, const GemvParams& p);

void launch_layernorm(int dt, const float* x, int64_t ldx, int rows, int d, const float* g1, const float* b1,
					  const float* g2, const float* b2, void* out, int64_t ldo, int out_f32, hipStream_t s, int frag = 0, float* out2 = nullptr,
					  const int64_t* out2_idx = nullptr, int64_t out2_stride = 0, const int64_t* out2_base = nullptr);
int gn_num_chunks(int T, int C);
int gn_rows_per_chunk(int C);
void launch_gn_stats(const float* x, int nb, int T, int C, float* part, hipStream_t s, const int* tlen = nullptr, const int* need = nullptr);
struct GnApplyParams {
	const float* x; const float* ms; const float* gamma; const float* beta;
	const float* scale; const float* shift; int64_t ss_stride;
	const int* row_idx; int nb, T, Tout, C; int nchunks; int act; void* out; int out_f32;
	const int* tlen; int chunk_rows;
	int out_f8;
	const void* pf; int64_t pf_bytes; int pf_taps;
#ifdef TTK_STAMPS
	unsigned long long* stamps;
#endif
};
void launch_gn_apply(int dt, const GnApplyParams& p, hipStream_t s, int form = 0);
const char* gn_apply_form_refusal(const GnApplyParams& p, int form);

struct AttnParams {
	const void* qkv; int64_t ld;
	int q_off, k_off, v_off, head_stride;
	void* out; int64_t ldo;
	int out_f8;
	int nb, T, H, causal;
	const int* tlen;
	const float* bias;
	float scale;
	const void* pf; int64_t pf_bytes; int pf_taps;
#ifdef TTK_STAMPS
	unsigned long long* stamps;
#endif
};
void launch_attn_fwd(int dt, const AttnParams& p, hipStream_t s, int form = 0);
const char* attn_fwd_form_refusal(const AttnParams& p, int form);

struct AttnDecodeParams {
	const float* qbuf;
	const void* kcache; const void* vcache;
	const int* d_pos;
	int B, H, max_ctx;
	int ctx_hint;
	void* out;
	int out_frag;
	const int2* row_info;
	int pos_slot_p1;
	int shared_rows;
#ifdef TTK_STAMPS
	unsigned long long* stamps;
#endif
};
void launch_attn_decode(int dt, const AttnDecodeParams& p, hipStream_t s, int variant = 0);
int attn_pos_slot_acquire(int** words_out);
void attn_pos_slot_release(int slot);

void launch_kv_scatter(int dt, const void* qkv, int B, int S, int H, void* kcache, void* vcache, int max_ctx, hipStream_t s, int t0 = 0);

void launch_xent_rows(const float* logits, int64_t ld, int rows, int C, const int64_t* target, float* nll, float* mean, float* logits_t, int T, hipStream_t s);

void launch_set_int(int* p, int v, hipStream_t s);
void launch_fill_int(int* p, int v, int n, hipStream_t s);
void launch_fill_int2(int* p, int a, int b, int n, hipStream_t s);
void launch_gather_add(const float* A, const int* ia, const float* Bt, const int* ib, float* out, int rows, int d, hipStream_t s);
void launch_embed_rows(int dt, const void* table, const int64_t* ids, int rows, int C, int n_tok, float* out, hipStream_t s);
void launch_decode_embed(const float* emb, const int64_t* tok, const float* pos, const int* d_pos, int pos_off, int pos_rows,
						 float* out, int B, int d, hipStream_t s, void* frag = nullptr, int frag_f32 = 0);
void launch_copy_rows(const float* src, int64_t lds_, float* dst, int64_t ldd, int rows, int d, hipStream_t s);
void launch_cast(int dt, const float* src, void* dst, int64_t n, hipStream_t s);
void launch_cf_to_cl(int dt, const float* src, int nb, int C, int T, void* dst, int64_t ldo, int rep, hipStream_t s, const int* tlen = nullptr);
void launch_cl_to_cf(const float* src, int nb, int C, int T, float* dst, hipStream_t s);
void launch_bcast_rows(int dt, const float* vec, int rows, int C, void* dst, hipStream_t s);
void launch_timestep_embedding(int dt, const int64_t* t, int64_t t_host, int n, int C, const float* freqs, void* out, hipStream_t s);
void launch_silu_cast(int dt, const float* x, void* y, int64_t n, hipStream_t s);
struct StepCoefs {
	float sqrt_recip_ac, sqrt_recipm1_ac, sqrt_ac_prev, sqrt_1m_ac_prev, cfk;
	float coef1, coef2, min_log, max_log; int sampler; int nonzero;
};
void launch_diffusion_step(const float* out_c, const float* out_u, float* x, const float* noise, int nb, int C, int T,
						   StepCoefs c, hipStream_t s, void* xcl = nullptr, int ldo = 0, int rep = 0, int ekind = 0);
struct StepExt { float sigma, dir, sqrt_ac_next, sqrt_1m_ac_next; int mode, clip; };
void launch_diffusion_step_ext(const float* out_c, const float* out_u, float* x, const float* noise, float* pred_xstart, int nb, int C, int T, StepCoefs c, StepExt e,
							   hipStream_t s, void* xcl = nullptr, int ldo = 0, int rep = 0, int ekind = 0);
struct StepMs { float c_x, c_d0, c_d1; int clip; };
void launch_diffusion_step_ms(const float* out_c, const float* out_u, float* x, float* x0_hist, float* pred_xstart, int nb, int C, int T, StepCoefs c, StepMs m,
							  hipStream_t s, void* xcl = nullptr, int ldo = 0, int rep = 0, int ekind = 0);

enum PackLayout { PK_NK = 0, PK_KN = 1, PK_CONV3 = 2, PK_CONVK = 3, PK_CONVT = 4 };
int device_absmax(const float* x, int64_t n, float* out_host);
void launch_fp8_roundtrip(float* x, int64_t n, float scale, hipStream_t s);
void launch_pack_frag_fp8(const void* src_bf16, int Npad, int K, float scale, void* dst, hipStream_t s);
void launch_pack_nk_f8(const float* src, int layout, int N, int K, int Npad, int Kpad, float scale, void* dst, hipStream_t s, int ntap = 0);
float fp8_scale_for(float absmax);
void launch_pack_nk(int dt, const float* src, int layout, int N, int K, int Npad, int Kpad, void* dst, hipStream_t s, int ntap = 0);
void launch_pack_frag(int dt, const void* src, int Npad, int K, void* dst, hipStream_t s);
void launch_scale_kn(float* w, const float* gamma, int K, int N, hipStream_t s);
void launch_rowsum(int dt, const void* w, int64_t ld, int N, int K, float* out, hipStream_t s);
void launch_bias_fold(const float* w, const float* beta, const float* b, int K, int N, float* out, hipStream_t s);

void launch_lora_update(const float* W0, const float* lora_B, const float* lora_A, int K, int N, int rank, float s, float* out, hipStream_t stream);

}
```

Measured before the change: 40.23 audio-sec/wall-sec.

## Fold input conv into integrating conv and split-K the output conv

Algebraically folds the inp_block conv into the integrating_conv weights on the host, in double precision with rounding to the compute dtype. Each diffusion step then runs one GEMM over 3 shifted input taps plus the conditioning segments, with no h0 intermediate. The output conv, which has few output channels, gets split-K partitions that write separate slabs, and the diffusion step kernels sum those slabs. The timestep-embedding host path also becomes a single launch with the values passed in a by-value struct. The fold changes rounding slightly, and split-K adds extra slab reads and writes.

```diff
diff --git a/tortoise_tts_amd/csrc/diff.hip b/tortoise_tts_amd/csrc/diff.hip
--- a/tortoise_tts_amd/csrc/diff.hip
+++ b/tortoise_tts_amd/csrc/diff.hip
@@ -1,5 +1,6 @@
 #include <stdlib.h>
 
+#include "diff_fold.h"
 #include "ttk_common.h"
 #include "ttk_host.h"
 
@@ -13,8 +14,9 @@
 	WsBuf a, hf, qkv, ao, ms;
 	const void* ms_owner = nullptr;
 };
-struct Segs { int n, K, rows_per_batch; GemmSeg s[3]; };
-struct Epi { int gn_T = 0; const float* residual = nullptr; float* ms = nullptr; int act = ACT_NONE; int transpose = 0; };
+struct Segs { int n, K, rows_per_batch; GemmSeg s[12]; };
+struct Epi { int gn_T = 0; const float* residual = nullptr; float* ms = nullptr; int act = ACT_NONE; int transpose = 0; int N = 0; int k_parts = 1; int64_t part_stride = 0; };
+struct OutPlan { int N, parts; };
 struct Gn {
 	const float *gamma, *beta; int act; const Mat* next = nullptr; const float* mod = nullptr; int64_t mod_stride = 0; const float* ms = nullptr;
 	void* out = nullptr; int out_f32 = 0; const int* row_idx = nullptr; int Tout = 0;
@@ -32,6 +34,8 @@
 	Arena arena;
 	AttnBlk lat_attn[4];
 	Mat lat_conv, inp_block, integ, out_conv, time0, time2, emb_cat;
+	Mat fold;
+	bool folded = false;
 	float *code_g, *code_b, *out_g, *out_b, *uncond, *time_freqs;
 	void* code_table = nullptr; int in_tokens = 0;
 	AttnBlk code_attn[3];
@@ -69,8 +73,9 @@
 	GemmParams g = {};
 	g.nseg = a.n;
 	for (int j = 0; j < a.n; ++j) g.seg[j] = a.s[j];
-	g.W = m.w; g.ldw = m.Kpad; g.M = M; g.N = m.N; g.K = a.K; g.rows_per_batch = a.rows_per_batch; g.bias = m.bias;
+	g.W = m.w; g.ldw = m.Kpad; g.M = M; g.N = e.N ? e.N : m.N; g.K = a.K; g.rows_per_batch = a.rows_per_batch; g.bias = m.bias;
 	g.residual = e.residual; g.ldr = ldc; g.C = C; g.ldc = ldc; g.out_f32 = out_f32; g.act = e.act; g.transpose_out = e.transpose;
+	g.k_parts = e.k_parts; g.part_stride = e.part_stride;
 	if (m.wes == 1) g.out_scale = m.wscale;
 	h->L->ms_owner = nullptr;
 	if (h->fuse_stats && e.gn_T > 0 && out_f32 && !e.transpose && gemm_fuses_gn_stats(M, m.N, h->cfg.model_channels, e.gn_T)) {
@@ -127,6 +132,15 @@
 	res_out(h, R, (const float*)h->L->hf.p, nullptr, x, x, nb, T, emb_all, emb_stride, s);
 }
 
+static OutPlan out_plan(const ttk_diff* h, bool reads_var) {
+	const int N = reads_var ? h->cfg.out_channels : h->cfg.in_channels;
+	const int kt = 3 * (int)(h->out_conv.Kpad * h->es / 128), ring = 3;
+	int parts = 8 / ((N + 63) / 64);
+	if (parts > kt / ring) parts = kt / ring;
+	while (parts > 1 && kt % parts != 0) --parts;
+	return {N, parts < 1 ? 1 : parts};
+}
+
 static int reserve_lane(ttk_diff* h, Lane& L, int nb, int T) {
 	const size_t rows = (size_t)nb * T, C = h->cfg.model_channels, es = h->es;
 	TTK_TRY(L.hf.reserve(rows * C * 4)); TTK_TRY(L.a.reserve(rows * C * es)); TTK_TRY(L.qkv.reserve(rows * 3 * C * es)); TTK_TRY(L.ao.reserve(rows * C * es));
@@ -139,8 +153,11 @@
 	h->L = &h->lane[0];
 	TTK_TRY(reserve_lane(h, h->lane[0], nb, T));
 	TTK_TRY(h->cs.reserve(rows * C * 4)); TTK_TRY(h->xs.reserve(rows * C * 4));
-	TTK_TRY(h->h0.reserve(rows * C * es)); TTK_TRY(h->csT.reserve(rows * C * es)); TTK_TRY(h->xcl.reserve(rows * h->in_pad * es));
-	TTK_TRY(h->outb.reserve(rows * h->cfg.out_channels * 4)); TTK_TRY(h->ecl.reserve(rows * C * 4));
+	if (!h->folded) TTK_TRY(h->h0.reserve(rows * C * es));
+	TTK_TRY(h->csT.reserve(rows * C * es)); TTK_TRY(h->xcl.reserve(rows * h->in_pad * es));
+	size_t out_ch = h->cfg.out_channels;
+	for (int v = 0; v < 2; ++v) { const OutPlan op = out_plan(h, v != 0); if ((size_t)op.N * op.parts > out_ch) out_ch = (size_t)op.N * op.parts; }
+	TTK_TRY(h->outb.reserve(rows * out_ch * 4)); TTK_TRY(h->ecl.reserve(rows * C * 4));
 	return TTK_OK;
 }
 
@@ -149,8 +166,8 @@
 	const size_t es = h->es;
 	TTK_TRY(h->temb.reserve((size_t)n * C * es)); TTK_TRY(h->e1.reserve((size_t)n * C * es)); TTK_TRY(h->e2.reserve((size_t)n * C * 4));
 	TTK_TRY(h->se.reserve((size_t)n * C * es)); TTK_TRY(h->emb_all.reserve((size_t)n * h->n_emb * 2 * C * 4));
-	if (t_dev) launch_timestep_embedding(h->dt, t_dev, 0, n, C, h->time_freqs, h->temb.p, s);
-	else for (int i = 0; i < n; ++i) launch_timestep_embedding(h->dt, nullptr, t_host[i], 1, C, h->time_freqs, (char*)h->temb.p + (size_t)i * C * es, s);
+	if (t_dev) launch_timestep_embedding(h->dt, t_dev, nullptr, n, C, h->time_freqs, h->temb.p, s);
+	else launch_timestep_embedding(h->dt, nullptr, t_host, n, C, h->time_freqs, h->temb.p, s);
 	Epi silu; silu.act = ACT_SILU;
 	gemm(h, h->time0, rows_of(h->temb.p, h->time0), n, h->e1.p, C, 0, s, silu);
 	gemm(h, h->time2, rows_of(h->e1.p, h->time2), n, h->e2.p, C, 1, s);
@@ -168,13 +185,20 @@
 	}
 }
 static void body(ttk_diff* h, int nb, int T, const float* emb_all, int64_t emb_stride, const float* cs, float* out, hipStream_t s,
-				 hipEvent_t cs_consumed = nullptr) {
+				 hipEvent_t cs_consumed = nullptr, const OutPlan* op = nullptr) {
 	const int C = h->cfg.model_channels, rows = nb * T;
 	float* x = (float*)h->xs.p;
-	gemm(h, h->inp_block, taps3(h->xcl.p, h->in_pad, h->inp_block, T), rows, h->h0.p, C, 0, s);
+	if (!h->folded) gemm(h, h->inp_block, taps3(h->xcl.p, h->in_pad, h->inp_block, T), rows, h->h0.p, C, 0, s);
 	launch_cast(h->dt, cs, h->csT.p, (int64_t)rows * C, s);
 	if (cs_consumed) (void)hipEventRecord(cs_consumed, s);
-	gemm(h, h->integ, {2, C, 0, {{h->h0.p, C, 0, 0}, {h->csT.p, C, 0, C}}}, rows, x, C, 1, s, {T});
+	if (h->folded) {
+		const int ip = h->in_pad;
+		Segs a = {3 + C / ip, ip, T, {}};
+		for (int j = 0; j < 3; ++j) a.s[j] = {h->xcl.p, ip, j - 1, (int64_t)j * ip};
+		for (int j = 0; j < C / ip; ++j) a.s[3 + j] = {(const char*)h->csT.p + (size_t)j * ip * h->es, C, 0, (int64_t)(3 + j) * ip};
+		gemm(h, h->fold, a, rows, x, C, 1, s, {T});
+	}
+	else gemm(h, h->integ, {2, C, 0, {{h->h0.p, C, 0, 0}, {h->csT.p, C, 0, C}}}, rows, x, C, 1, s, {T});
 	for (size_t i = 0; i < h->layers.size(); ++i) {
 		res_block(h, h->layers[i].res, x, nb, T, emb_all, emb_stride, s);
 		attn_block(h, h->layers[i].attn, x, nb, T, s);
@@ -182,6 +206,7 @@
 	for (int i = 0; i < 3; ++i) res_block(h, h->tail[i], x, nb, T, emb_all, emb_stride, s);
 	gn(h, x, nb, T, {h->out_g, h->out_b, ACT_SILU}, s);
 	Epi t; t.transpose = 1;
+	if (op) { t.N = op->N; t.k_parts = op->parts; t.part_stride = (int64_t)rows * op->N; }
 	gemm(h, h->out_conv, taps3(h->L->a.p, C, h->out_conv, T), rows, out, 0, 1, s, t);
 }
 
@@ -204,6 +229,40 @@
 	TTK_TRY(upload_mat(h->arena, wm, h->wdt, p + "out_layers.3.weight", p + "out_layers.3.bias", PK_CONV3, C, C, false, &R->out3));
 	R->emb_slot = slot;
 	return TTK_OK;
+}
+
+static int upload_host_mat(Arena& ar, int dt, const float* w, const float* bias, int N, int K, Mat* out) {
+	out->N = N; out->K = K; out->ntap = 1; out->Npad = round_up(N, 128); out->Kpad = K; out->wes = (int)dtype_size(dt);
+	TTK_TRY(ar.alloc(&out->w, (size_t)out->Npad * out->Kpad * out->wes));
+	TTK_TRY(ar.alloc((void**)&out->bias, (size_t)N * sizeof(float)));
+	TTK_HIP(hipMemcpy(out->bias, bias, (size_t)N * sizeof(float), hipMemcpyHostToDevice));
+	WsBuf tmp;
+	TTK_TRY(tmp.reserve((size_t)N * K * sizeof(float)));
+	TTK_HIP(hipMemcpy(tmp.p, w, (size_t)N * K * sizeof(float), hipMemcpyHostToDevice));
+	pack_mat(dt, (const float*)tmp.p, PK_NK, *out, 0);
+	TTK_HIP(hipDeviceSynchronize());
+	return TTK_OK;
+}
+static int fetch_host(const WeightMap& wm, const std::string& name, int64_t expect_numel, std::vector<float>& out) {
+	const ttk_weight_view* v = wm.find(name);
+	TTK_REQUIRE(v != nullptr, TTK_E_WEIGHT, "missing weight '%s'", name.c_str());
+	TTK_REQUIRE(numel(v) == expect_numel, TTK_E_WEIGHT, "weight '%s' has %lld elements, expected %lld", name.c_str(), (long long)numel(v), (long long)expect_numel);
+	out.resize((size_t)expect_numel);
+	TTK_HIP(hipMemcpy(out.data(), v->data, (size_t)expect_numel * sizeof(float), hipMemcpyDefault));
+	return TTK_OK;
+}
+static int build_fold(ttk_diff* h, const WeightMap& wm) {
+	const int C = h->cfg.model_channels, in = h->cfg.in_channels, ip = h->in_pad;
+	h->folded = C % ip == 0 && 3 + C / ip <= 12;
+	if (!h->folded) return TTK_OK;
+	std::vector<float> w_integ, b_integ, w_inp, b_inp, w, b;
+	TTK_TRY(fetch_host(wm, "integrating_conv.weight", (int64_t)C * 2 * C, w_integ)); TTK_TRY(fetch_host(wm, "integrating_conv.bias", C, b_integ));
+	TTK_TRY(fetch_host(wm, "inp_block.weight", (int64_t)C * in * 3, w_inp)); TTK_TRY(fetch_host(wm, "inp_block.bias", C, b_inp));
+	const DiffFold f = diff_fold(w_integ.data(), b_integ.data(), w_inp.data(), b_inp.data(), C, in, ip);
+	if (h->dt == DT_BF16) diff_fold_round(f, 8, -126, w, b);
+	else if (h->dt == DT_F16) diff_fold_round(f, 11, -14, w, b);
+	else diff_fold_round(f, 24, -126, w, b);
+	return upload_host_mat(h->arena, h->dt, w.data(), b.data(), C, f.ld(), &h->fold);
 }
 
 static void precompute_tail(ttk_diff* h, const float* x, const float* cond, const int32_t* interp_idx, int b, int M, int T, float* E_out, hipStream_t s) {
@@ -252,6 +311,7 @@
 	TTK_TRY(upload_mat(h->arena, wm, h->dt, "latent_conditioner.0.weight", "latent_conditioner.0.bias", PK_CONV3, C, cfg->in_latent_channels, false, &h->lat_conv));
 	for (int i = 0; i < 4; ++i) TTK_TRY(load_attn(h.get(), wm, "latent_conditioner." + std::to_string(i + 1) + ".", &h->lat_attn[i]));
 	TTK_TRY(upload_mat(h->arena, wm, h->dt, "integrating_conv.weight", "integrating_conv.bias", PK_NK, C, 2 * C, false, &h->integ));
+	TTK_TRY(build_fold(h.get(), wm));
 	TTK_TRY(upload_f32(h->arena, wm, "out.0.weight", C, &h->out_g));
 	TTK_TRY(upload_f32(h->arena, wm, "out.0.bias", C, &h->out_b));
 	TTK_TRY(upload_mat(h->arena, wm, h->dt, "out.2.weight", "out.2.bias", PK_CONV3, cfg->out_channels, C, false, &h->out_conv));
@@ -423,20 +483,16 @@
 	const int b = h->cur_b, T = h->cur_T, Cin = h->cfg.in_channels, rep = p.nb / b;
 	if (p.layout) launch_cf_to_cl(h->dt, x, b, Cin, T, h->xcl.p, h->in_pad, rep, s, h->tlen);
 	float* out = (float*)h->outb.p;
-	body(h, p.nb, T, p.emb, 0, cs, out, s, cs_consumed);
-	const float* out_u = out + (size_t)b * h->cfg.out_channels * T;
-	if (p.ms) {
-		if (p.stage_next) launch_diffusion_step_ms(out, out_u, x, p.x0_hist, p.pred_xstart, b, Cin, T, coefs_of(*p.st), ms_of(*p.ms), s, h->xcl.p, h->in_pad, rep, elem_kind(h->dt));
-		else launch_diffusion_step_ms(out, out_u, x, p.x0_hist, p.pred_xstart, b, Cin, T, coefs_of(*p.st), ms_of(*p.ms), s);
-		return;
-	}
-	if (p.ext) {
-		if (p.stage_next) launch_diffusion_step_ext(out, out_u, x, p.noise, p.pred_xstart, b, Cin, T, coefs_of(*p.st), ext_of(*p.ext), s, h->xcl.p, h->in_pad, rep, elem_kind(h->dt));
-		else launch_diffusion_step_ext(out, out_u, x, p.noise, p.pred_xstart, b, Cin, T, coefs_of(*p.st), ext_of(*p.ext), s);
-		return;
-	}
-	if (p.stage_next) launch_diffusion_step(out, out_u, x, p.noise, b, Cin, T, coefs_of(*p.st), s, h->xcl.p, h->in_pad, rep, elem_kind(h->dt));
-	else launch_diffusion_step(out, out_u, x, p.noise, b, Cin, T, coefs_of(*p.st), s);
+	const bool reads_var = p.ms ? false : (p.ext ? p.ext->mode == 1 : p.st->sampler == 1);
+	const OutPlan op = out_plan(h, reads_var);
+	body(h, p.nb, T, p.emb, 0, cs, out, s, cs_consumed, &op);
+	const float* out_u = out + (size_t)b * op.N * T;
+	const StepSlabs sl = {op.parts, (int64_t)p.nb * T * op.N, (int64_t)op.N * T};
+	void* xcl = p.stage_next ? h->xcl.p : nullptr;
+	const int ldo = p.stage_next ? h->in_pad : 0, nrep = p.stage_next ? rep : 0, ek = p.stage_next ? elem_kind(h->dt) : 0;
+	if (p.ms) launch_diffusion_step_ms(out, out_u, x, p.x0_hist, p.pred_xstart, b, Cin, T, coefs_of(*p.st), ms_of(*p.ms), s, xcl, ldo, nrep, ek, sl);
+	else if (p.ext) launch_diffusion_step_ext(out, out_u, x, p.noise, p.pred_xstart, b, Cin, T, coefs_of(*p.st), ext_of(*p.ext), s, xcl, ldo, nrep, ek, sl);
+	else launch_diffusion_step(out, out_u, x, p.noise, b, Cin, T, coefs_of(*p.st), s, xcl, ldo, nrep, ek, sl);
 }
 
 int ttk_diff_step(ttk_diff* h, float* x, const ttk_step* st, const float* noise, void* stream) {
diff --git a/tortoise_tts_amd/csrc/diff_fold.h b/tortoise_tts_amd/csrc/diff_fold.h
--- /dev/null
+++ b/tortoise_tts_amd/csrc/diff_fold.h
@@ -0,0 +1,58 @@
+#pragma once
+#include <math.h>
+#include <stddef.h>
+#include <stdint.h>
+
+#include <vector>
+
+namespace ttk {
+
+inline double fold_round(double x, int sig, int emin) {
+	if (x == 0.0 || !isfinite(x)) return x;
+	int e;
+	(void)frexp(x, &e);
+	const int qmin = emin - (sig - 1);
+	const int q = e - sig > qmin ? e - sig : qmin;
+	return ldexp(nearbyint(ldexp(x, -q)), q);
+}
+
+struct DiffFold {
+	int C = 0, in = 0, in_pad = 0;
+	std::vector<double> w;
+	std::vector<double> b;
+	int ld() const { return 3 * in_pad + C; }
+};
+inline DiffFold diff_fold(const float* w_integ, const float* b_integ, const float* w_inp, const float* b_inp, int C, int in, int in_pad) {
+	DiffFold f;
+	f.C = C; f.in = in; f.in_pad = in_pad;
+	const int ld = f.ld(), ck = in * 3;
+	f.w.assign((size_t)C * ld, 0.0);
+	f.b.assign((size_t)C, 0.0);
+	std::vector<double> acc((size_t)ck);
+	for (int n = 0; n < C; ++n) {
+		const float* wi = w_integ + (size_t)n * 2 * C;
+		for (int q = 0; q < ck; ++q) acc[q] = 0.0;
+		double bacc = 0.0;
+		for (int m = 0; m < C; ++m) {
+			const double a = (double)wi[m];
+			const float* src = w_inp + (size_t)m * ck;
+			for (int q = 0; q < ck; ++q) acc[q] += a * (double)src[q];
+			bacc += a * (double)b_inp[m];
+		}
+		double* row = f.w.data() + (size_t)n * ld;
+		for (int c = 0; c < in; ++c)
+			for (int tap = 0; tap < 3; ++tap) row[(size_t)tap * in_pad + c] = acc[(size_t)c * 3 + tap];
+		for (int m = 0; m < C; ++m) row[(size_t)3 * in_pad + m] = (double)wi[C + m];
+		f.b[n] = (double)b_integ[n] + bacc;
+	}
+	return f;
+}
+
+inline void diff_fold_round(const DiffFold& f, int sig, int emin, std::vector<float>& w, std::vector<float>& b) {
+	w.resize(f.w.size());
+	b.resize(f.b.size());
+	for (size_t i = 0; i < f.w.size(); ++i) w[i] = (float)fold_round(f.w[i], sig, emin);
+	for (size_t i = 0; i < f.b.size(); ++i) b[i] = (float)f.b[i];
+}
+
+}
diff --git a/tortoise_tts_amd/csrc/elementwise.hip b/tortoise_tts_amd/csrc/elementwise.hip
--- a/tortoise_tts_amd/csrc/elementwise.hip
+++ b/tortoise_tts_amd/csrc/elementwise.hip
@@ -142,20 +142,29 @@
 	by_dtype(dt, [&](auto t) { using T = decltype(t); hipLaunchKernelGGL((k_bcast_rows<T>), grid, dim3(256), 0, s, vec, rows, C, (T*)dst); });
 }
 
-template <typename T>
-__global__ void k_timestep_embedding(const int64_t* t, int64_t t_host, int n, int C, const float* freqs, T* out) {
+struct TimestepBlock { enum { N = 256 }; int64_t v[N]; };
+template <typename T>
+__global__ void k_timestep_embedding(const int64_t* t, TimestepBlock t_host, int n, int C, const float* freqs, T* out) {
 	const int idx = blockIdx.x * blockDim.x + threadIdx.x;
 	const int half = C / 2;
 	if (idx >= n * half) return;
 	const int i = idx / half, j = idx - i * half;
-	const float tv = (float)(t ? t[i] : t_host);
+	const float tv = (float)(t ? t[i] : t_host.v[i]);
 	const float a = tv * freqs[j];
 	out[(int64_t)i * C + j] = cvt<T>(cosf(a));
 	out[(int64_t)i * C + half + j] = cvt<T>(sinf(a));
 }
-void launch_timestep_embedding(int dt, const int64_t* t, int64_t t_host, int n, int C, const float* freqs, void* out, hipStream_t s) {
-	const dim3 grid(grid_for(n * (C / 2)));
-	by_dtype(dt, [&](auto e) { using T = decltype(e); hipLaunchKernelGGL((k_timestep_embedding<T>), grid, dim3(256), 0, s, t, t_host, n, C, freqs, (T*)out); });
+void launch_timestep_embedding(int dt, const int64_t* t, const int64_t* t_host, int n, int C, const float* freqs, void* out, hipStream_t s) {
+	for (int i0 = 0; i0 < n; i0 += t ? n : (int)TimestepBlock::N) {
+		const int cnt = t ? n : (n - i0 < (int)TimestepBlock::N ? n - i0 : (int)TimestepBlock::N);
+		TimestepBlock tb = {};
+		if (!t) for (int i = 0; i < cnt; ++i) tb.v[i] = t_host[i0 + i];
+		const dim3 grid(grid_for(cnt * (C / 2)));
+		by_dtype(dt, [&](auto e) {
+			using T = decltype(e);
+			hipLaunchKernelGGL((k_timestep_embedding<T>), grid, dim3(256), 0, s, t, tb, cnt, C, freqs, (T*)out + (size_t)i0 * C);
+		});
+	}
 }
 
 template <typename T>
@@ -167,15 +176,20 @@
 	by_dtype(dt, [&](auto t) { using T = decltype(t); hipLaunchKernelGGL((k_silu_cast<T>), dim3(grid_for(n)), dim3(256), 0, s, x, (T*)y, n); });
 }
 
-__global__ void k_diffusion_step(const float* out_c, const float* out_u, float* x, const float* noise, int nb, int C, int Tn, StepCoefs k, void* xcl, int ldo, int rep, int ekind) {
+__device__ __forceinline__ float out_sum(const float* o, int64_t i, const StepSlabs& sl) {
+	float v = o[i];
+	for (int q = 1; q < sl.parts; ++q) v += o[(int64_t)q * sl.slab + i];
+	return v;
+}
+__global__ void k_diffusion_step(const float* out_c, const float* out_u, float* x, const float* noise, int nb, int C, int Tn, StepCoefs k, void* xcl, int ldo, int rep, int ekind, StepSlabs sl) {
 	const int64_t idx = (int64_t)blockIdx.x * blockDim.x + threadIdx.x;
 	const int64_t per = (int64_t)C * Tn;
 	if (idx >= nb * per) return;
 	const int b = (int)(idx / per);
 	const int64_t r = idx - b * per;
-	float eps = out_c[(int64_t)b * 2 * per + r];
+	float eps = out_sum(out_c, (int64_t)b * sl.bstride + r, sl);
 	if (k.cfk >= 0.f) {
-		const float eu = out_u[(int64_t)b * 2 * per + r];
+		const float eu = out_sum(out_u, (int64_t)b * sl.bstride + r, sl);
 		eps = (1.0f + k.cfk) * eps - k.cfk * eu;
 	}
 	const float xv = x[idx];
@@ -186,7 +200,7 @@
 		const float e2 = (k.sqrt_recip_ac * xv - x0) / k.sqrt_recipm1_ac;
 		xn = x0 * k.sqrt_ac_prev + k.sqrt_1m_ac_prev * e2;
 	} else {
-		const float var = out_c[(int64_t)b * 2 * per + per + r];
+		const float var = out_sum(out_c, (int64_t)b * sl.bstride + per + r, sl);
 		const float frac = (var + 1.0f) / 2.0f;
 		const float log_var = frac * k.max_log + (1.0f - frac) * k.min_log;
 		const float mean = k.coef1 * x0 + k.coef2 * xv;
@@ -203,22 +217,23 @@
 		}
 	}
 }
-void launch_diffusion_step(const float* out_c, const float* out_u, float* x, const float* noise, int nb, int C, int T, StepCoefs c, hipStream_t s, void* xcl, int ldo, int rep, int ekind) {
+static StepSlabs slabs_or_whole(StepSlabs sl, int C, int T) { return sl.parts > 0 ? sl : StepSlabs{1, 0, (int64_t)2 * C * T}; }
+void launch_diffusion_step(const float* out_c, const float* out_u, float* x, const float* noise, int nb, int C, int T, StepCoefs c, hipStream_t s, void* xcl, int ldo, int rep, int ekind, StepSlabs sl) {
 	const int64_t total = (int64_t)nb * C * T;
-	hipLaunchKernelGGL(k_diffusion_step, dim3(grid_for(total)), dim3(256), 0, s, out_c, out_u, x, noise, nb, C, T, c, xcl, ldo, rep, ekind);
+	hipLaunchKernelGGL(k_diffusion_step, dim3(grid_for(total)), dim3(256), 0, s, out_c, out_u, x, noise, nb, C, T, c, xcl, ldo, rep, ekind, slabs_or_whole(sl, C, T));
 }
 
 __global__ void k_diffusion_step_ext(const float* out_c, const float* out_u, float* x, const float* noise, float* pred_xstart, int nb, int C, int Tn, StepCoefs k, StepExt e,
-									 void* xcl, int ldo, int rep, int ekind) {
+									 void* xcl, int ldo, int rep, int ekind, StepSlabs sl) {
 #pragma clang fp contract(off)
 	const int64_t idx = (int64_t)blockIdx.x * blockDim.x + threadIdx.x;
 	const int64_t per = (int64_t)C * Tn;
 	if (idx >= nb * per) return;
 	const int b = (int)(idx / per);
 	const int64_t r = idx - b * per;
-	float eps = out_c[(int64_t)b * 2 * per + r];
+	float eps = out_sum(out_c, (int64_t)b * sl.bstride + r, sl);
 	if (k.cfk >= 0.f) {
-		const float eu = out_u[(int64_t)b * 2 * per + r];
+		const float eu = out_sum(out_u, (int64_t)b * sl.bstride + r, sl);
 		eps = (1.0f + k.cfk) * eps - k.cfk * eu;
 	}
 	const float xv = x[idx];
@@ -228,7 +243,7 @@
 	if (pred_xstart) pred_xstart[idx] = x0;
 	float xn;
 	if (e.mode == 1) {
-		const float var = out_c[(int64_t)b * 2 * per + per + r];
+		const float var = out_sum(out_c, (int64_t)b * sl.bstride + per + r, sl);
 		const float frac = (var + 1.0f) / 2.0f;
 		const float log_var = frac * k.max_log + (1.0f - frac) * k.min_log;
 		const float mean = __builtin_fmaf(k.coef2, xv, k.coef1 * x0);
@@ -254,22 +269,22 @@
 	}
 }
 void launch_diffusion_step_ext(const float* out_c, const float* out_u, float* x, const float* noise, float* pred_xstart, int nb, int C, int T, StepCoefs c, StepExt e, hipStream_t s,
-							   void* xcl, int ldo, int rep, int ekind) {
+							   void* xcl, int ldo, int rep, int ekind, StepSlabs sl) {
 	const int64_t total = (int64_t)nb * C * T;
-	hipLaunchKernelGGL(k_diffusion_step_ext, dim3(grid_for(total)), dim3(256), 0, s, out_c, out_u, x, noise, pred_xstart, nb, C, T, c, e, xcl, ldo, rep, ekind);
+	hipLaunchKernelGGL(k_diffusion_step_ext, dim3(grid_for(total)), dim3(256), 0, s, out_c, out_u, x, noise, pred_xstart, nb, C, T, c, e, xcl, ldo, rep, ekind, slabs_or_whole(sl, C, T));
 }
 
 __global__ void k_diffusion_step_ms(const float* out_c, const float* out_u, float* x, float* x0_hist, float* pred_xstart, int nb, int C, int Tn, StepCoefs k, StepMs m,
-									void* xcl, int ldo, int rep, int ekind) {
+									void* xcl, int ldo, int rep, int ekind, StepSlabs sl) {
 #pragma clang fp contract(off)
 	const int64_t idx = (int64_t)blockIdx.x * blockDim.x + threadIdx.x;
 	const int64_t per = (int64_t)C * Tn;
 	if (idx >= nb * per) return;
 	const int b = (int)(idx / per);
 	const int64_t r = idx - b * per;
-	float eps = out_c[(int64_t)b * 2 * per + r];
+	float eps = out_sum(out_c, (int64_t)b * sl.bstride + r, sl);
 	if (k.cfk >= 0.f) {
-		const float eu = out_u[(int64_t)b * 2 * per + r];
+		const float eu = out_sum(out_u, (int64_t)b * sl.bstride + r, sl);
 		eps = (1.0f + k.cfk) * eps - k.cfk * eu;
 	}
 	const float xv = x[idx];
@@ -292,9 +307,9 @@
 	}
 }
 void launch_diffusion_step_ms(const float* out_c, const float* out_u, float* x, float* x0_hist, float* pred_xstart, int nb, int C, int T, StepCoefs c, StepMs m, hipStream_t s,
-							  void* xcl, int ldo, int rep, int ekind) {
+							  void* xcl, int ldo, int rep, int ekind, StepSlabs sl) {
 	const int64_t total = (int64_t)nb * C * T;
-	hipLaunchKernelGGL(k_diffusion_step_ms, dim3(grid_for(total)), dim3(256), 0, s, out_c, out_u, x, x0_hist, pred_xstart, nb, C, T, c, m, xcl, ldo, rep, ekind);
-}
-
-}
+	hipLaunchKernelGGL(k_diffusion_step_ms, dim3(grid_for(total)), dim3(256), 0, s, out_c, out_u, x, x0_hist, pred_xstart, nb, C, T, c, m, xcl, ldo, rep, ekind, slabs_or_whole(sl, C, T));
+}
+
+}
diff --git a/tortoise_tts_amd/csrc/gemm.hip b/tortoise_tts_amd/csrc/gemm.hip
--- a/tortoise_tts_amd/csrc/gemm.hip
+++ b/tortoise_tts_amd/csrc/gemm.hip
@@ -193,7 +193,7 @@
 }
 
 template <typename T, int BM, int BN, int NWM, int NWN, int NSTAGE, int ROLE, bool LONGK = false>
-__device__ __forceinline__ void gemm_tile(const GemmParams& p, const int m0, const int n0, const int wave) {
+__device__ __forceinline__ void gemm_tile(const GemmParams& p, const int m0, const int n0, const int wave, const int part = 0) {
 	typedef GRole<ROLE> R;
 	static_assert(!R::on || (sizeof(T) <= 2 && R::N % BN == 0), "roles are 16-bit or fp8, N a multiple of the tile width");
 	constexpr int LDS_AVAIL = NSTAGE * ((BM == 64 && NWM == 1 ? 128 : BM) + BN) * 128;
@@ -221,7 +221,8 @@
 #endif
 	const int wm = wave / NWN, wn = wave % NWN;
 	const int KT = R::on ? GR_K / BKE : p.K / BKE;
-	const int NTILES = R::on ? R::NSEG * KT : p.nseg * KT;
+	const int NT_ALL = R::on ? R::NSEG * KT : p.nseg * KT;
+	const int NTILES = R::on || p.k_parts <= 1 ? NT_ALL : NT_ALL / p.k_parts;
 
 	const int prow = lane >> 3, pslot = lane & 7;
 	int a_gm[A_PC], a_t[A_PC];
@@ -298,6 +299,14 @@
 		else if (++kk_i == KT) { kk_i = 0; ++seg_i; }
 		seg_i = __builtin_amdgcn_readfirstlane(seg_i); kk_i = __builtin_amdgcn_readfirstlane(kk_i);
 	};
+	if constexpr (!R::on) {
+		if (part > 0) {
+			const int t0 = part * NTILES;
+			if (seg_in) { seg_i = t0 % NSEG; kk_i = t0 / NSEG; } else { seg_i = t0 / KT; kk_i = t0 - seg_i * KT; }
+			seg_i = __builtin_amdgcn_readfirstlane(seg_i); kk_i = __builtin_amdgcn_readfirstlane(kk_i);
+			if (!seg_in && kk_i != 0) set_segment(seg_i);
+		}
+	}
 	auto issue = [&](int stage) {
 		if (seg_in || kk_i == 0) set_segment(seg_i);
 		const unsigned As = smem_base + stage * STAGE;
@@ -706,7 +715,10 @@
 		return;
 	}
 	const bool full = (m0 + BM <= p.M) && (n0 + BN <= p.N);
-	if (p.transpose_out) { if (full) epilogue<T, 2, false, MI, NI>(p, acc, row0, col0, lane); else epilogue<T, 2, true, MI, NI>(p, acc, row0, col0, lane); }
+	if (p.transpose_out) {
+		const int64_t c_off = (int64_t)part * p.part_stride;
+		if (full) epilogue<T, 2, false, MI, NI>(p, acc, row0, col0, lane, c_off, part == 0); else epilogue<T, 2, true, MI, NI>(p, acc, row0, col0, lane, c_off, part == 0);
+	}
 	else if (p.out_f32) { if (full) epilogue<T, 1, false, MI, NI>(p, acc, row0, col0, lane); else epilogue<T, 1, true, MI, NI>(p, acc, row0, col0, lane); }
 	else { if (full) epilogue<T, 0, false, MI, NI>(p, acc, row0, col0, lane); else epilogue<T, 0, true, MI, NI>(p, acc, row0, col0, lane); }
 	TTK_WSTAMP(stamps_, blockIdx.x, 4);
@@ -738,7 +750,11 @@
 #endif
 	TTK_WSTAMP(stamps_, blockIdx.x, 0);
 	const int tiles_m = R::on ? p.tiles_m : (p.M + BM - 1) / BM;
-	const int tile_id = xcd_tile_id(blockIdx.x, R::on ? tiles_m * (R::N / BN) : (int)gridDim.x);
+	int part = 0, block = (int)blockIdx.x, nwg = (int)gridDim.x;
+	if constexpr (!R::on) {
+		if (p.k_parts > 1) { nwg = nwg / p.k_parts; part = block / nwg; block -= part * nwg; }
+	}
+	const int tile_id = xcd_tile_id(block, R::on ? tiles_m * (R::N / BN) : nwg);
 	int m0, n0;
 	if constexpr (R::on) {
 		const int tn = div_recip(tile_id, tiles_m, p.inv_tiles_m);
@@ -748,7 +764,7 @@
 		m0 = p.m_major ? (tile_id / tiles_n) * BM : (tile_id % tiles_m) * BM;
 		n0 = p.m_major ? (tile_id % tiles_n) * BN : (tile_id / tiles_m) * BN;
 	}
-	gemm_tile<T, BM, BN, NWM, NWN, NSTAGE, ROLE, LONGK>(p, m0, n0, wave);
+	gemm_tile<T, BM, BN, NWM, NWN, NSTAGE, ROLE, LONGK>(p, m0, n0, wave, part);
 }
 
 template <typename T, int ROLE>
@@ -791,13 +807,13 @@
 static void launch_tile(const GemmParams& p_in, hipStream_t s, hipEvent_t ea, hipEvent_t eb) {
 	constexpr int LDS = NSTAGE * (BM + BN) * 128;
 	if constexpr (!LONGK && ROLE == GR_NONE && sizeof(T) == 2 && BM == 256 && BN == 128 && NSTAGE == 3) {
-		if (TTK_GEMM_PIPE_H && (p_in.K / 64) * p_in.nseg > NSTAGE) return launch_tile<T, BM, BN, NWM, NWN, NSTAGE, ROLE, true>(p_in, s, ea, eb);
+		if (TTK_GEMM_PIPE_H && (p_in.K / 64) * p_in.nseg / (p_in.k_parts > 1 ? p_in.k_parts : 1) > NSTAGE) return launch_tile<T, BM, BN, NWM, NWN, NSTAGE, ROLE, true>(p_in, s, ea, eb);
 	}
 	static bool attr_set = false;
 	opt_in_lds_once(attr_set, (const void*)k_gemm<T, BM, BN, NWM, NWN, NSTAGE, ROLE, LONGK>, LDS);
 	GemmParams p = p_in;
 	fill_derived(p, (p.M + BM - 1) / BM);
-	const int grid = p.tiles_m * ((p.N + BN - 1) / BN);
+	const int grid = p.tiles_m * ((p.N + BN - 1) / BN) * (ROLE == GR_NONE && p.k_parts > 1 ? p.k_parts : 1);
 	hipExtLaunchKernelGGL((k_gemm<T, BM, BN, NWM, NWN, NSTAGE, ROLE, LONGK>), dim3(grid), dim3(64 * NWM * NWN), (unsigned)LDS, s, ea, eb, 0, p);
 }
 
@@ -834,6 +850,7 @@
 }
 static int gemm_role_of_unmasked(const GemmParams& p, int es) {
 	if (g_gemm_roles < 0) gemm_roles_refresh();
+	if (p.k_parts > 1) return GR_NONE;
 	if ((es != 2 && es != 1) || p.K != GR_K || p.ldw != GR_K || !p.bias || p.act != ACT_NONE || (es == 2) != (p.out_scale == 0.f)) return GR_NONE;
 	if (p.transpose_out || p.m_major) return GR_NONE;
 	if (p.M < 1 || p.M > (1 << 19) || p.seg[0].lda != GR_K || p.seg[0].w_off != 0) return GR_NONE;
@@ -921,6 +938,7 @@
 	else if (order == 3) p.m_major = 1;
 	p.seg_inner = p.nseg == 3 && p.seg[0].shift == -1 && p.seg[1].shift == 0 && p.seg[2].shift == 1 && p.seg[1].A == p.seg[0].A && p.seg[2].A == p.seg[0].A &&
 				  p.seg[1].lda == p.seg[0].lda && p.seg[2].lda == p.seg[0].lda;
+	if (p.k_parts > 1 && !(p.transpose_out && p.act == ACT_NONE && ((int64_t)p.K * (int64_t)(dt == DT_F32 ? 4 : (dt == DT_FP8 ? 1 : 2)) / 128 * p.nseg) % p.k_parts == 0)) p.k_parts = 1;
 	hipEvent_t ea = nullptr, eb = nullptr;
 	if (g_prof_on) prof_pair(PROF_GEMM, 2.0 * p.M * p.N * (double)p.K * p.nseg, &ea, &eb);
 	if (dt == DT_FP8) launch_gemm_t<f8>(p, s, ea, eb);
diff --git a/tortoise_tts_amd/csrc/gemm_epilogue.h b/tortoise_tts_amd/csrc/gemm_epilogue.h
--- a/tortoise_tts_amd/csrc/gemm_epilogue.h
+++ b/tortoise_tts_amd/csrc/gemm_epilogue.h
@@ -33,7 +33,7 @@
 }
 
 template <typename T, int MODE, bool GUARD, int MI, int NI>
-__device__ __forceinline__ void epilogue(const GemmParams& p, f32x4 (&acc)[MI][NI], int row0, int col0, int lane) {
+__device__ __forceinline__ void epilogue(const GemmParams& p, f32x4 (&acc)[MI][NI], int row0, int col0, int lane, const int64_t c_off = 0, const bool with_bias = true) {
 #pragma clang fp contract(off)
 	const int lr = 4 * (lane >> 4), lc = lane & 15;
 	typedef typename OutOf<T>::type OT;
@@ -47,7 +47,7 @@
 #pragma unroll
 	for (int j = 0; j < NI; ++j) {
 		const int gn = col0 + 16 * j + lc;
-		bj[j] = (p.bias && (!GUARD || gn < p.N)) ? p.bias[gn] : 0.f;
+		bj[j] = (p.bias && with_bias && (!GUARD || gn < p.N)) ? p.bias[gn] : 0.f;
 	}
 #pragma unroll
 	for (int i = 0; i < MI; ++i)
@@ -102,7 +102,7 @@
 				if (GUARD && (gm >= p.M || gn >= p.N)) continue;
 				const float v = acc[i][j][r] + res[i][r][j];
 				acc[i][j][r] = v;
-				if (MODE == 2) ((float*)p.C)[((int64_t)bb * p.N + gn) * p.rows_per_batch + t] = v;
+				if (MODE == 2) ((float*)p.C)[c_off + ((int64_t)bb * p.N + gn) * p.rows_per_batch + t] = v;
 				else if (MODE == 1) ((float*)p.C)[(int64_t)gm * p.ldc + gn] = v;
 				else ((OT*)p.C)[(int64_t)gm * p.ldc + gn] = cvt<OT>(v);
 			}
diff --git a/tortoise_tts_amd/csrc/ttk_kernels.h b/tortoise_tts_amd/csrc/ttk_kernels.h
--- a/tortoise_tts_amd/csrc/ttk_kernels.h
+++ b/tortoise_tts_amd/csrc/ttk_kernels.h
@@ -56,6 +56,7 @@
 	int m_major;
 	int tiles_m; float inv_tiles_m, inv_rpb, inv_gn_T;
 	int mix_full, mix_fm;
+	int k_parts; int64_t part_stride;
 #ifdef TTK_STAMPS
 	unsigned long long* stamps;
 #endif
@@ -198,20 +199,21 @@
 void launch_cf_to_cl(int dt, const float* src, int nb, int C, int T, void* dst, int64_t ldo, int rep, hipStream_t s, const int* tlen = nullptr);
 void launch_cl_to_cf(const float* src, int nb, int C, int T, float* dst, hipStream_t s);
 void launch_bcast_rows(int dt, const float* vec, int rows, int C, void* dst, hipStream_t s);
-void launch_timestep_embedding(int dt, const int64_t* t, int64_t t_host, int n, int C, const float* freqs, void* out, hipStream_t s);
+void launch_timestep_embedding(int dt, const int64_t* t, const int64_t* t_host, int n, int C, const float* freqs, void* out, hipStream_t s);
 void launch_silu_cast(int dt, const float* x, void* y, int64_t n, hipStream_t s);
 struct StepCoefs {
 	float sqrt_recip_ac, sqrt_recipm1_ac, sqrt_ac_prev, sqrt_1m_ac_prev, cfk;
 	float coef1, coef2, min_log, max_log; int sampler; int nonzero;
 };
+struct StepSlabs { int parts; int64_t slab, bstride; };
 void launch_diffusion_step(const float* out_c, const float* out_u, float* x, const float* noise, int nb, int C, int T,
-						   StepCoefs c, hipStream_t s, void* xcl = nullptr, int ldo = 0, int rep = 0, int ekind = 0);
+						   StepCoefs c, hipStream_t s, void* xcl = nullptr, int ldo = 0, int rep = 0, int ekind = 0, StepSlabs sl = {0, 0, 0});
 struct StepExt { float sigma, dir, sqrt_ac_next, sqrt_1m_ac_next; int mode, clip; };
 void launch_diffusion_step_ext(const float* out_c, const float* out_u, float* x, const float* noise, float* pred_xstart, int nb, int C, int T, StepCoefs c, StepExt e,
-							   hipStream_t s, void* xcl = nullptr, int ldo = 0, int rep = 0, int ekind = 0);
+							   hipStream_t s, void* xcl = nullptr, int ldo = 0, int rep = 0, int ekind = 0, StepSlabs sl = {0, 0, 0});
 struct StepMs { float c_x, c_d0, c_d1; int clip; };
 void launch_diffusion_step_ms(const float* out_c, const float* out_u, float* x, float* x0_hist, float* pred_xstart, int nb, int C, int T, StepCoefs c, StepMs m,
-							  hipStream_t s, void* xcl = nullptr, int ldo = 0, int rep = 0, int ekind = 0);
+							  hipStream_t s, void* xcl = nullptr, int ldo = 0, int rep = 0, int ekind = 0, StepSlabs sl = {0, 0, 0});
 
 enum PackLayout { PK_NK = 0, PK_KN = 1, PK_CONV3 = 2, PK_CONVK = 3, PK_CONVT = 4 };
 int device_absmax(const float* x, int64_t n, float* out_host);
```

Result: no change. 40.49 audio-sec/wall-sec, median of 6 (+0.6%).
